# phantomzone-org/fhe-ram

Hardware: AMD Instinct MI355X
Metric: encrypted RAM read ops/s + write ops/s at 2^18 entries; achieved HBM GB/s vs peak (higher is better)
Workload: dtype f64

## Files before the change

fhe-ram_amd/csrc/bank.hpp:

```cpp
#pragma once
#include "path.hpp"

struct fheram_regs;
struct fheram_table;

enum LastKind { LAST_LIST, LAST_SELECT, LAST_REGS, LAST_TABLE, LAST_PEEK, LAST_KINDS };
struct LastOutputs {
    int n = 0;
    ResHome home;
};

struct fheram_bank {
    fheram_ctx* c = nullptr;
    int M = 0, mws = 0;
    RamState ram[FHERAM_BANK_MAX];
    double* d_prep = nullptr;
    double* d_prep_inv = nullptr;
    DenseBufs list;
    LastOutputs last[LAST_KINDS];
    DenseBufs wl;
    int kept_alone = 0, kept_n = 0;
    unsigned kept_map = 0;
    bool wl_holds[FHERAM_BANK_MAX] = {};
    SelectBufs sel;
    SelectLaneTable lanes;
    int sel_fail_alloc = 0;
    bool has_res[FHERAM_BANK_MAX] = {};
    int wl_fail_alloc = 0;
    OneRowSet regs;
    std::vector<fheram_regs*> regfiles;
    const int32_t* regs_old = nullptr;
    const fheram_regs* regs_old_owner = nullptr;
    OneRowSet tabs;
    std::vector<fheram_table*> tables;
    MixBufs mix;
    PublicBufs pub;
    int pub_fail_alloc = 0;
};

namespace {

void regs_keys_changed(fheram_bank* b);
void regs_bank_release(fheram_bank* b);
void table_bank_release(fheram_bank* b);

static_assert(FHERAM_READ_LIST_MAX >= FHERAM_BANK_MAX && FHERAM_READ_LIST_MAX * 4 <= 32, "a member set has four bits of the map per entry");
struct MemberSet {
    int n = 0;
    int m[FHERAM_READ_LIST_MAX];
    static MemberSet range(int first, int n) { MemberSet s; s.n = n; for (int k = 0; k < n; k++) s.m[k] = first + k; return s; }
    static MemberSet list(const int* members, int n) { MemberSet s; s.n = n; for (int k = 0; k < n; k++) s.m[k] = members[k]; return s; }
    bool is_range() const { for (int k = 1; k < n; k++) if (m[k] != m[0] + k) return false; return true; }
    unsigned map() const { unsigned v = 0; for (int k = 0; k < n; k++) v |= (unsigned)m[k] << (4 * k); return v; }
};

RamView bank_view(const fheram_bank* b, int first) {
    RamView v = ctx_view(b->c);
    const size_t o1 = (size_t)first * b->mws * fheram_ctx::GLWE, oR = o1 * b->c->rows;
    for (int32_t** p : {&v.rows, &v.A, &v.B, &v.C, &v.D}) *p += oR;
    for (int32_t** p : {&v.part, &v.tmp, &v.tmp2, &v.res, &v.tree, &v.w, &v.trtop}) *p += o1;
    return v;
}
GlweRef member_slot(const fheram_bank* b, int32_t* buf, int m) { return ref(buf + (size_t)m * b->mws * fheram_ctx::GLWE, (long)fheram_ctx::GLWE, 0); }

int check_addrs(fheram_ctx* c, const fheram_addr* const* addrs, int n) {
    for (int k = 0; k < n; k++) {
        if (!addrs[k] || addrs[k]->ctx != c) return fail(c, FHERAM_ERR_INVALID_ARG, "address " + std::to_string(k) + " is null or does not belong to this bank (layout mismatch, ram.rs:404)");
        if (addrs[k]->empty) return fail(c, FHERAM_ERR_INVALID_ARG, "address " + std::to_string(k) + " is an empty address: fheram_bank_address_alloc without fheram_bank_address_derive");
    }
    return FHERAM_OK;
}
int members_ready(fheram_bank* b, const MemberSet& s, const fheram_addr* const* addrs, int want_state) {
    fheram_ctx* c = b->c;
    if (addrs) { const int rc = check_addrs(c, addrs, s.n); if (rc != FHERAM_OK) return rc; }
    for (int k = 0; k < s.n; k++)
        if (!b->ram[s.m[k]].initialized) return fail(c, FHERAM_ERR_UNINITIALIZED, "unitialized memory: self.data.len()=0 (member " + std::to_string(s.m[k]) + ")");
    if (want_state < 0) return FHERAM_OK;
    if (!c->keys_loaded) return fail(c, FHERAM_ERR_KEYS, "evaluation keys not loaded");
    for (int k = 0; k < s.n; k++) {
        if (want_state == 0 && b->ram[s.m[k]].state)
            return fail(c, FHERAM_ERR_STATE, "invalid call to Memory.read: internal state is true -> requires calling Memory.write (member " + std::to_string(s.m[k]) + ")");
        if (want_state == 1 && !b->ram[s.m[k]].state)
            return fail(c, FHERAM_ERR_STATE, "invalid call to Memory.write: internal state is false -> requires calling Memory.read_prepare_write (member " + std::to_string(s.m[k]) + ")");
    }
    return FHERAM_OK;
}
int range_check(fheram_bank* b, int first, int n, const fheram_addr* const* addrs, const char* null_args, int want_state, MemberSet* s) {
    if (!b) return FHERAM_ERR_INVALID_ARG;
    fheram_ctx* c = b->c;
    if (null_args) return fail(c, FHERAM_ERR_INVALID_ARG, null_args);
    mid_rearm(c);
    if (first < 0 || n < 1 || first > b->M - n)
        return fail(c, FHERAM_ERR_INVALID_ARG, "member range [" + std::to_string(first) + ", " + std::to_string(first) + " + " + std::to_string(n) + ") is empty or outside the bank's " + std::to_string(b->M) + " members");
    *s = MemberSet::range(first, n);
    return members_ready(b, *s, addrs, want_state);
}
int read_list_check(fheram_bank* b, const int* members, const fheram_addr* const* addrs, int n, MemberSet* s) {
    if (!b) return FHERAM_ERR_INVALID_ARG;
    fheram_ctx* c = b->c;
    mid_rearm(c);
    if (!members || !addrs) return fail(c, FHERAM_ERR_INVALID_ARG, "null member list or null address list");
    if (n < 1 || n > FHERAM_READ_LIST_MAX)
        return fail(c, FHERAM_ERR_INVALID_ARG, "n = " + std::to_string(n) + " is outside [1, FHERAM_READ_LIST_MAX = " + std::to_string(FHERAM_READ_LIST_MAX) + "]");
    if ((long)n * b->mws > 64)
        return fail(c, FHERAM_ERR_INVALID_ARG, "n * word_size = " + std::to_string((long)n * b->mws) + " exceeds 64, the ciphertext limit of the single-launch chains (k_chain_mid)");
    for (int k = 0; k < n; k++)
        if (members[k] < 0 || members[k] >= b->M)
            return fail(c, FHERAM_ERR_INVALID_ARG, "entry " + std::to_string(k) + " names member " + std::to_string(members[k]) + ", outside the bank's " + std::to_string(b->M) + " members");
    *s = MemberSet::list(members, n);
    return members_ready(b, *s, addrs, 0);
}
int write_list_members(fheram_bank* b, const int* members, const fheram_addr* const* addrs, int n, int want_state, MemberSet* s) {
    fheram_ctx* c = b->c;
    if (n < 1 || n > b->M)
        return fail(c, FHERAM_ERR_INVALID_ARG, "n = " + std::to_string(n) + " is outside [1, the bank's " + std::to_string(b->M) + " members]");
    unsigned seen = 0;
    for (int k = 0; k < n; k++) {
        if (members[k] < 0 || members[k] >= b->M)
            return fail(c, FHERAM_ERR_INVALID_ARG, "entry " + std::to_string(k) + " names member " + std::to_string(members[k]) + ", outside the bank's " + std::to_string(b->M) + " members");
        if (seen & (1u << members[k]))
            return fail(c, FHERAM_ERR_INVALID_ARG, "entry " + std::to_string(k) + " names member " + std::to_string(members[k]) + " a second time: a RAM has one pending write (ram.rs:196-294), so the members of a write list are distinct");
        seen |= 1u << members[k];
    }
    *s = MemberSet::list(members, n);
    return members_ready(b, *s, addrs, want_state);
}
int write_list_check(fheram_bank* b, const int* members, const fheram_addr* const* addrs, int n, bool null_words, int want_state, MemberSet* s) {
    if (!b) return FHERAM_ERR_INVALID_ARG;
    fheram_ctx* c = b->c;
    mid_rearm(c);
    if (!members || !addrs || null_words) return fail(c, FHERAM_ERR_INVALID_ARG, want_state ? "null member list, null address list or null words" : "null member list or null address list");
    return write_list_members(b, members, addrs, n, want_state, s);
}

RamState set_state(const fheram_bank* b, const MemberSet& s, bool dense, bool write) {
    RamState st{true, write, true, dense ? 0 : b->ram[s.m[0]].memo_alone, false};
    bool holds = dense && write && b->kept_alone > 0 && b->kept_n == s.n && b->kept_map == s.map();
    for (int k = 0; k < s.n; k++) {
        const RamState& r = b->ram[s.m[k]];
        st.memo_top = st.memo_top && r.memo_top;
        if (!dense && r.memo_alone != st.memo_alone) st.memo_alone = 0;
        holds = holds && b->wl_holds[s.m[k]];
    }
    if (holds) st.memo_alone = b->kept_alone;
    return st;
}
struct SetPlan {
    const bool dense;
    RamState st;
    const RamView v;
    const Opnds o;
    SetPlan(fheram_bank* b, const MemberSet& s, const fheram_addr* const* addrs, bool write)
        : dense(!s.is_range()), st(set_state(b, s, dense, write)), v(dense ? dense_view(b->c, b->wl) : bank_view(b, s.m[0])),
          o(s.n == 1 ? one_addr(b->c, addrs, b->mws, &st)
                     : table_opnds(b->c, &st, addrs, s.n, b->mws, b->d_prep, b->d_prep_inv, dense ? s.map() : MEMBER_MAP_IDENTITY, true)) {}
    SetPlan(const SetPlan&) = delete;
};
void set_assign(fheram_bank* b, const MemberSet& s, const RamState& st, bool dense, bool state, bool new_result) {
    for (int k = 0; k < s.n; k++) {
        RamState& r = b->ram[s.m[k]];
        r.state = state; r.memo_top = st.memo_top; r.memo_alone = dense ? 0 : st.memo_alone;
        if (new_result) { r.res_in_trtop = st.res_in_trtop; b->has_res[s.m[k]] = true; }
        b->wl_holds[s.m[k]] = dense && st.memo_alone > 0;
    }
}
int set_result(fheram_bank* b, const MemberSet& s, bool dense, int64_t* out) {
    fheram_ctx* c = b->c;
    const size_t per = (size_t)b->mws * fheram_ctx::GLWE;
    ResRun runs[FHERAM_BANK_MAX];
    int n_runs = 0;
    for (int k = 0; k < s.n; k++) {
        const int32_t* src = (b->ram[s.m[k]].res_in_trtop ? c->d_trtop : c->d_res) + (size_t)s.m[k] * per;
        if (!dense && n_runs && runs[n_runs - 1].src + runs[n_runs - 1].n == src) runs[n_runs - 1].n += per;
        else runs[n_runs++] = ResRun{src, per};
    }
    return result_export(c, runs, n_runs, c->h_res, c->d_h_res, out);
}
int bank_read_set(fheram_bank* b, const MemberSet& s, const fheram_addr* const* addrs, bool prepare_write, int64_t* out) {
    fheram_ctx* c = b->c;
    HIPCHK(c, hipSetDevice(c->device));
    if (!s.is_range()) {
        const int rc = dense_reserve(c, b->wl, s.n, b->mws, true, &b->wl_fail_alloc);
        if (rc != FHERAM_OK) return rc;
        b->kept_alone = 0;
    }
    SetPlan p(b, s, addrs, false);
    const int rc = read_impl(p.o, p.v, prepare_write);
    if (rc == FHERAM_OK && p.dense) {
        const long G = (long)fheram_ctx::GLWE;
        for (int k = 0; k < s.n; k++) {
            if (c->n2 == 2) launch_copy(c, p.o.slice(ref(p.v.tree, G, 0), k), member_slot(b, c->d_tree, s.m[k]), 1, b->mws);
            launch_copy(c, p.o.slice(ref(p.st.res_in_trtop ? p.v.trtop : p.v.res, G, 0), k), member_slot(b, p.st.res_in_trtop ? c->d_trtop : c->d_res, s.m[k]), 1, b->mws);
        }
        b->kept_alone = p.st.memo_alone; b->kept_n = s.n; b->kept_map = p.o.member_map;
    }
    set_assign(b, s, p.st, p.dense, rc == FHERAM_OK && prepare_write, true);
    if (rc != FHERAM_OK) return rc;
    HIPCHK(c, hipGetLastError());
    return out ? set_result(b, s, p.dense, out) : FHERAM_OK;
}
template <typename S>
int bank_write_set(fheram_bank* b, const MemberSet& s, const fheram_addr* const* addrs, S&& stage) {
    fheram_ctx* c = b->c;
    HIPCHK(c, hipSetDevice(c->device));
    if (!s.is_range()) {
        const int rc = dense_reserve(c, b->wl, s.n, b->mws, true, &b->wl_fail_alloc);
        if (rc != FHERAM_OK) return rc;
    }
    SetPlan p(b, s, addrs, true);
    const long G = (long)fheram_ctx::GLWE;
    if (p.dense) {
        const bool holds = p.st.memo_alone > 0;
        b->kept_alone = 0;
        if (!holds) {
            main_enqueued(c);
            for (int k = 0; k < s.n; k++) {
                if (c->n2 == 2) launch_copy(c, member_slot(b, c->d_tree, s.m[k]), p.o.slice(ref(p.v.tree, G, 0), k), 1, b->mws);
                if (p.st.memo_top) launch_copy(c, member_slot(b, c->d_trtop, s.m[k]), p.o.slice(ref(p.v.trtop, G, 0), k), 1, b->mws);
            }
        }
    }
    const int rc = write_all(p.o, p.v, stage);
    if (rc == FHERAM_OK && p.dense && c->n2 == 2)
        for (int k = 0; k < s.n; k++) launch_copy(c, p.o.slice(ref(p.v.tree, G, 0), k), member_slot(b, c->d_tree, s.m[k]), 1, b->mws);
    set_assign(b, s, p.st, p.dense, rc != FHERAM_OK, false);
    if (rc != FHERAM_OK) return rc;
    HIPCHK(c, hipGetLastError());
    return FHERAM_OK;
}
struct LastKindText {
    int src;
    const char *unit, *units;
    const char *last, *of_last;
    const char* none;
};
const LastKindText LAST_TEXT[LAST_KINDS] = {
    {FHERAM_SRC_LIST_RESULT, "entry", "entries", "read list", "list", "no read list has run"},
    {FHERAM_SRC_SELECT_RESULT, "output", "outputs", "select", "select", "no select has run"},
    {FHERAM_SRC_REGS_RESULT, "output", "outputs", "register read", "register read", "no fheram_bank_regs_read has run"},
    {FHERAM_SRC_TABLE_RESULT, "output", "outputs", "table read", "table read", "no fheram_bank_table_read has run"},
    {FHERAM_SRC_PEEK_RESULT, "output", "outputs", "peek", "peek", "no fheram_bank_peek or fheram_bank_poke has run"},
};
int last_result(fheram_bank* b, LastKind kind, int first, int n, int64_t* out) {
    fheram_ctx* c = b->c;
    const LastOutputs& L = b->last[kind];
    const LastKindText& t = LAST_TEXT[kind];
    if (!out) return fail(c, FHERAM_ERR_INVALID_ARG, "null output");
    if (!L.n) return fail(c, FHERAM_ERR_STATE, std::string(t.none) + " on this bank");
    if (first < 0 || n < 1 || first > L.n - n)
        return fail(c, FHERAM_ERR_INVALID_ARG, std::string(t.units) + " [" + std::to_string(first) + ", " + std::to_string(first) + " + " + std::to_string(n) + ") are empty or outside the last " + t.of_last + "'s " + std::to_string(L.n) + " " + t.units);
    HIPCHK(c, hipSetDevice(c->device));
    const size_t per = (size_t)b->mws * fheram_ctx::GLWE;
    const ResRun run{L.home.res + (size_t)first * per, (size_t)n * per};
    return result_export(c, &run, 1, L.home.h, L.home.d_h, out);
}
void list_done(fheram_bank* b, int n) { b->last[LAST_LIST] = LastOutputs{n, ResHome{b->list.res, b->list.h_res, b->list.d_h_res, -1}}; }

}

extern "C" {

int fheram_bank_create(const fheram_params* p, int device, int n_members, const fheram_config* cfg, fheram_bank** out) {
    if (!p || !out) return fail(nullptr, FHERAM_ERR_INVALID_ARG, "null argument");
    *out = nullptr;
    if (n_members < 1 || n_members > FHERAM_BANK_MAX)
        return fail(nullptr, FHERAM_ERR_INVALID_ARG, "n_members = " + std::to_string(n_members) + " is outside [1, FHERAM_BANK_MAX = " + std::to_string(FHERAM_BANK_MAX) + "]");
    if ((uint64_t)n_members * p->word_size > 64)
        return fail(nullptr, FHERAM_ERR_INVALID_ARG, "n_members * word_size = " + std::to_string((uint64_t)n_members * p->word_size) + " exceeds 64, the ciphertext limit of the single-launch chains (k_chain_mid)");
    fheram_params wide = *p;
    wide.word_size = (uint32_t)n_members * p->word_size;
    fheram_config asked;
    if (cfg) asked = *cfg; else fheram_config_default(&asked);
    if (n_members > 1) asked.pre_inv = 0;
    fheram_ctx* c = nullptr;
    const int rc = fheram_ctx_create_cfg(&wide, device, 0, 1, &asked, &c);
    if (rc != FHERAM_OK) return rc;
    fheram_bank* b = new fheram_bank();
    b->c = c; b->M = n_members; b->mws = (int)p->word_size;
    c->ram.initialized = true;
    if (n_members > 1) {
        const size_t bytes = (size_t)n_members * c->n_digits * fheram_ctx::GGSW * sizeof(double);
        hipError_t e = c->res.device(&b->d_prep, bytes);
        if (e == hipSuccess) e = c->res.device(&b->d_prep_inv, bytes);
        if (e != hipSuccess) {
            (void)hipGetLastError();
            fheram_bank_destroy(b);
            return fail(nullptr, FHERAM_ERR_DEVICE, std::string("operand tables of the bank: ") + hipGetErrorString(e));
        }
    }
    *out = b;
    return FHERAM_OK;
}
void fheram_bank_destroy(fheram_bank* b) {
    if (!b) return;
    if (b->c) { hipSetDevice(b->c->device); for (hipStream_t s : {b->c->stream, b->c->stream2}) if (s) hipStreamSynchronize(s); }
    dense_free(b->list);
    dense_free(b->wl);
    select_free(b->sel);
    lane_table_free(b->lanes);
    regs_bank_release(b);
    table_bank_release(b);
    mix_bufs_free(b->mix);
    public_bufs_free(b->pub);
    fheram_ctx_destroy(b->c);
    delete b;
}
const char* fheram_bank_last_error(const fheram_bank* b) { return fheram_last_error(b ? b->c : nullptr); }
int fheram_bank_size(const fheram_bank* b) { return b ? b->M : 0; }

int fheram_bank_keys_load(fheram_bank* b, const int64_t* gal_els, int n_gal, const int64_t* const* atk_glwe,
                          const int64_t* atk_ggsw_inv, int64_t atk_ggsw_inv_p, const int64_t* tsk) {
    if (!b) return FHERAM_ERR_INVALID_ARG;
    const int rc = fheram_keys_load(b->c, gal_els, n_gal, atk_glwe, atk_ggsw_inv, atk_ggsw_inv_p, tsk);
    if (rc != FHERAM_OK) return rc;
    for (int m = 0; m < b->M; m++) { b->ram[m].memo_top = false; b->ram[m].memo_alone = 0; b->wl_holds[m] = false; }
    regs_keys_changed(b);
    return FHERAM_OK;
}
int fheram_bank_ram_upload(fheram_bank* b, int member, const int64_t* rows) {
    if (!b) return FHERAM_ERR_INVALID_ARG;
    fheram_ctx* c = b->c;
    if (member < 0 || member >= b->M) return fail(c, FHERAM_ERR_INVALID_ARG, "no such member");
    if (!rows) return fail(c, FHERAM_ERR_INVALID_ARG, "null rows");
    HIPCHK(c, hipSetDevice(c->device));
    const size_t n = (size_t)b->mws * c->rows * fheram_ctx::GLWE;
    const int rc = upload_i64(c, c->d_data + (size_t)member * n, rows, n);
    if (rc != FHERAM_OK) return rc;
    RamState& r = b->ram[member];
    r.initialized = true; r.state = false; r.memo_top = false; r.memo_alone = 0;
    b->wl_holds[member] = false;
    return FHERAM_OK;
}
int fheram_bank_ram_download(fheram_bank* b, int member, int64_t* rows) {
    if (!b) return FHERAM_ERR_INVALID_ARG;
    fheram_ctx* c = b->c;
    if (member < 0 || member >= b->M || !rows) return fail(c, FHERAM_ERR_INVALID_ARG, "no such member, or null rows");
    if (!b->ram[member].initialized) return fail(c, FHERAM_ERR_UNINITIALIZED, "unitialized memory: self.data.len()=0");
    HIPCHK(c, hipSetDevice(c->device));
    const size_t n = (size_t)b->mws * c->rows * fheram_ctx::GLWE;
    const int rc = download_i64(c, rows, c->d_data + (size_t)member * n, n);
    return rc == FHERAM_OK ? check_precision(c) : rc;
}
int fheram_bank_ram_tree_download(fheram_bank* b, int member, int level, int64_t* out) {
    if (!b) return FHERAM_ERR_INVALID_ARG;
    fheram_ctx* c = b->c;
    if (member < 0 || member >= b->M || !out) return fail(c, FHERAM_ERR_INVALID_ARG, "no such member, or null output");
    if (level != 0 || c->n2 < 2) return fail(c, FHERAM_ERR_INVALID_ARG, "tree level does not exist (ram.rs:315-324)");
    HIPCHK(c, hipSetDevice(c->device));
    const size_t n = (size_t)b->mws * fheram_ctx::GLWE;
    return download_i64(c, out, c->d_tree + (size_t)member * n, n);
}
int fheram_bank_ram_state(const fheram_bank* b, int member) { return (b && member >= 0 && member < b->M) ? (int)b->ram[member].state : 0; }

int fheram_bank_address_create(fheram_bank* b, const int64_t* const* ggsw, int n_ggsw, fheram_addr** out) {
    if (!b) return FHERAM_ERR_INVALID_ARG;
    return fheram_address_create(b->c, ggsw, n_ggsw, out);
}

int fheram_bank_fheuint_create(fheram_bank* b, const int64_t* bits, int n_bits, fheram_fheuint** out) {
    if (!b) return FHERAM_ERR_INVALID_ARG;
    return fheram_fheuint_create(b->c, bits, n_bits, out);
}
int fheram_bank_address_alloc(fheram_bank* b, fheram_addr** out) {
    if (!b) return FHERAM_ERR_INVALID_ARG;
    return fheram_address_alloc(b->c, out);
}
int fheram_bank_address_derive(fheram_bank* b, const fheram_fheuint* const* fus, int n, int sign, fheram_addr* const* addrs) {
    if (!b) return FHERAM_ERR_INVALID_ARG;
    return fheram_address_derive(b->c, fus, n, sign, addrs);
}
int fheram_bank_address_derive_at(fheram_bank* b, const fheram_fheuint* const* fus, const int* first_bit, int n, int sign, fheram_addr* const* addrs) {
    if (!b) return FHERAM_ERR_INVALID_ARG;
    return fheram_address_derive_at(b->c, fus, first_bit, n, sign, addrs);
}

int fheram_bank_read(fheram_bank* b, int first, int n, const fheram_addr* const* addrs, int64_t* out) {
    MemberSet s;
    const int rc = range_check(b, first, n, addrs, addrs ? nullptr : "null address list", 0, &s);
    return rc == FHERAM_OK ? bank_read_set(b, s, addrs, false, out) : rc;
}
int fheram_bank_read_prepare_write(fheram_bank* b, int first, int n, const fheram_addr* const* addrs, int64_t* out) {
    MemberSet s;
    const int rc = range_check(b, first, n, addrs, addrs ? nullptr : "null address list", 0, &s);
    return rc == FHERAM_OK ? bank_read_set(b, s, addrs, true, out) : rc;
}
int fheram_bank_write(fheram_bank* b, int first, int n, const int64_t* w, const fheram_addr* const* addrs) {
    MemberSet s;
    const int rc = range_check(b, first, n, addrs, (addrs && w) ? nullptr : "null address list or null words", 1, &s);
    return rc == FHERAM_OK ? bank_write_set(b, s, addrs, [&](int32_t* d_w, int n_ct) { return stage_words(b->c, d_w, w, n_ct); }) : rc;
}
int fheram_bank_result_download(fheram_bank* b, int first, int n, int64_t* out) {
    if (!b) return FHERAM_ERR_INVALID_ARG;
    if (!out) return fail(b->c, FHERAM_ERR_INVALID_ARG, "null output");
    MemberSet s;
    const int rc = range_check(b, first, n, nullptr, nullptr, -1, &s);
    if (rc != FHERAM_OK) return rc;
    HIPCHK(b->c, hipSetDevice(b->c->device));
    return set_result(b, s, false, out);
}
int fheram_bank_read_list(fheram_bank* b, const int* members, const fheram_addr* const* addrs, int n, int64_t* out) {
    MemberSet s;
    int rc = read_list_check(b, members, addrs, n, &s);
    if (rc != FHERAM_OK) return rc;
    fheram_ctx* c = b->c;
    HIPCHK(c, hipSetDevice(c->device));
    const long G = (long)fheram_ctx::GLWE;
    b->last[LAST_LIST].n = 0;
    if (n == 1) {
        rc = dense_reserve(c, b->list, 1, b->mws);
        if (rc == FHERAM_OK) rc = bank_read_set(b, s, addrs, false, nullptr);
        if (rc != FHERAM_OK) return rc;
        launch_copy(c, member_slot(b, c->d_res, s.m[0]), ref(b->list.res, G, 0), 1, b->mws);
        list_done(b, 1);
        HIPCHK(c, hipGetLastError());
        return out ? last_result(b, LAST_LIST, 0, 1, out) : FHERAM_OK;
    }
    RamState st{true, false, false, 0, false};
    return read_many(c, b->list, &st, addrs, n, b->mws, s.map(), b->M > 1, out, [&](const Opnds& o) {
        set_assign(b, s, st, false, false, true);
        for (int m = 0; m < b->M; m++) {
            int last = -1;
            for (int k = 0; k < n; k++) if (s.m[k] == m) last = k;
            if (last >= 0) launch_copy(c, o.slice(ref(b->list.res, G, 0), last), member_slot(b, c->d_res, m), 1, b->mws);
        }
        list_done(b, n);
    });
}
int fheram_bank_read_prepare_write_list(fheram_bank* b, const int* members, const fheram_addr* const* addrs, int n, int64_t* out) {
    MemberSet s;
    const int rc = write_list_check(b, members, addrs, n, false, 0, &s);
    return rc == FHERAM_OK ? bank_read_set(b, s, addrs, true, out) : rc;
}
int fheram_bank_write_list(fheram_bank* b, const int* members, const fheram_addr* const* addrs, int n, const int64_t* w) {
    MemberSet s;
    const int rc = write_list_check(b, members, addrs, n, !w, 1, &s);
    return rc == FHERAM_OK ? bank_write_set(b, s, addrs, [&](int32_t* d_w, int n_ct) { return stage_words(b->c, d_w, w, n_ct); }) : rc;
}
int fheram_bank_selftest_fail_list_alloc(fheram_bank* b, int nth) {
    if (!b || nth < 0) return FHERAM_ERR_INVALID_ARG;
    b->wl_fail_alloc = nth;
    return FHERAM_OK;
}
int fheram_bank_read_list_result(fheram_bank* b, int first, int n, int64_t* out) {
    return b ? last_result(b, LAST_LIST, first, n, out) : FHERAM_ERR_INVALID_ARG;
}
int fheram_bank_sync(fheram_bank* b) { return b ? fheram_sync(b->c) : FHERAM_ERR_INVALID_ARG; }
int fheram_bank_roundoff_max(fheram_bank* b, double* max_out) { return b ? fheram_roundoff_max(b->c, max_out) : FHERAM_ERR_INVALID_ARG; }
int fheram_bank_roundoff_reset(fheram_bank* b) { return b ? fheram_roundoff_reset(b->c) : FHERAM_ERR_INVALID_ARG; }
int fheram_bank_tail_stats(fheram_bank* b, uint64_t* launches, uint64_t* fallbacks) { return b ? fheram_tail_stats(b->c, launches, fallbacks) : FHERAM_ERR_INVALID_ARG; }
int fheram_bank_mid_stats(fheram_bank* b, uint64_t* launches, uint64_t* fallbacks) { return b ? fheram_mid_stats(b->c, launches, fallbacks) : FHERAM_ERR_INVALID_ARG; }
int fheram_bank_profile_enable(fheram_bank* b, int on) { return b ? fheram_profile_enable(b->c, on) : FHERAM_ERR_INVALID_ARG; }
int fheram_bank_profile_get(fheram_bank* b, const char* cls, uint64_t* launches, uint64_t* blocks, double* total_ms) {
    return b ? fheram_profile_get(b->c, cls, launches, blocks, total_ms) : FHERAM_ERR_INVALID_ARG;
}
int fheram_bank_profile_reset(fheram_bank* b) { return b ? fheram_profile_reset(b->c) : FHERAM_ERR_INVALID_ARG; }

}
```

fhe-ram_amd/csrc/ctx.hpp:

```cpp
#pragma once
#include "../../include/fheram.h"
#include "kernels.hpp"
#include "cmux_chain.hpp"
#include "cmux_jobs.hpp"
#include "mapped_chains.hpp"
#include "tail_wait.hpp"

#include <algorithm>
#include <atomic>
#include <cstdio>
#include <cstdlib>
#include <cstring>
#include <map>
#include <string>
#include <vector>

using namespace fk;

namespace {

thread_local std::string g_create_err;


struct ProfCls {
    uint64_t launches = 0, blocks = 0;
    double ms = 0.0;
    std::vector<std::pair<hipEvent_t, hipEvent_t>> pending;
};

}

inline uint64_t next_addr_id() { static std::atomic<uint64_t> n{0}; return ++n; }

struct RamState {
    bool initialized = false, state = false;
    bool memo_top = false;
    int memo_alone = 0;
    bool res_in_trtop = false;
};

struct DenseBufs {
    int cap = 0;
    int32_t *A = nullptr, *B = nullptr, *C = nullptr, *D = nullptr;
    int32_t *part = nullptr, *tmp = nullptr, *tmp2 = nullptr, *res = nullptr, *tree = nullptr, *w = nullptr, *trtop = nullptr;
    double* prep = nullptr;
    int64_t *h_res = nullptr, *d_h_res = nullptr;
};

inline fheram_config config_builtin() {
    fheram_config d{};
    d.limb_split = 1; d.fine_split = 1; d.memo = 1; d.pre_inv = 1; d.tail = 1; d.tail_test = 0; d.mid = 2; d.mid_test = 0;
    d.chain = 1; d.chain_y = 3; d.pair_z = 1; d.fuse = 1; d.graph = 0; d.safe = 0; d.nco = 0; d.tail_ep = 1; d.monitor = 1; d.reserved = 0;
    return d;
}
inline fheram_config config_in_effect(const fheram_config& in) {
    using C = fheram_config;
    fheram_config e{};
    for (int32_t C::*on_off : {&C::limb_split, &C::fine_split, &C::memo, &C::tail, &C::tail_ep, &C::mid_test, &C::chain, &C::pair_z, &C::fuse, &C::graph, &C::safe})
        e.*on_off = in.*on_off ? 1 : 0;
    for (int32_t C::*upto2 : {&C::tail_test, &C::mid, &C::monitor}) e.*upto2 = in.*upto2 < 0 ? 0 : (in.*upto2 > 2 ? 2 : in.*upto2);
    e.chain_y = in.chain_y ? 3 : 0;
    e.nco = in.nco == 2 ? 2 : (in.nco == 1 ? 1 : 0);
    e.pre_inv = e.memo ? (in.pre_inv == 2 ? 2 : (in.pre_inv ? 1 : 0)) : 0;
    if (e.graph) e.pre_inv = 0;
    if (e.safe) { e.tail = 0; e.tail_test = 0; e.mid = 0; e.mid_test = 0; if (e.pre_inv == 1) e.pre_inv = 2; }
    if (e.safe && e.monitor == 1) e.monitor = 2;
    return e;
}

struct CtxResources {
    std::vector<void*> dev, pinned;
    std::vector<hipEvent_t> events;
    template <typename T> hipError_t device(T** p, size_t bytes) { const hipError_t e = hipMalloc((void**)p, bytes); if (e == hipSuccess) dev.push_back(*p); return e; }
    template <typename T> hipError_t host(T** p, size_t bytes, unsigned flags) { const hipError_t e = hipHostMalloc((void**)p, bytes, flags); if (e == hipSuccess) pinned.push_back(*p); return e; }
    hipError_t event(hipEvent_t* ev, bool timing = false) {
        const hipError_t e = timing ? hipEventCreate(ev) : hipEventCreateWithFlags(ev, hipEventDisableTiming);
        if (e == hipSuccess) events.push_back(*ev);
        return e;
    }
    void release() {
        for (hipEvent_t e : events) hipEventDestroy(e);
        for (void* p : dev) hipFree(p);
        for (void* p : pinned) hipHostFree(p);
        events.clear(); dev.clear(); pinned.clear();
    }
};

struct fheram_ctx {
    fheram_params p;
    int device = 0;
    int ws = 0, n2 = 0, n_digits = 0, max_digits = 0;
    size_t rows = 0;
    size_t rows_glob = 0;
    int shard = 0, n_shards = 1;
    std::vector<std::vector<int>> base2d;
    static constexpr int S_CT = 3, S_ADDR = 4, S_INV = 5, DNUM_CT = 3, DNUM_GGSW = 4;
    int s_evk = 4;
    size_t atk = 0;
    static constexpr size_t GLWE = (size_t)S_CT * 2 * N;
    static constexpr size_t GLWE4 = (size_t)S_ADDR * 2 * N;
    static constexpr size_t GGSW = (size_t)DNUM_CT * 2 * GLWE4;
    static constexpr size_t EVK5 = (size_t)DNUM_GGSW * S_INV * 2 * N;
    static constexpr size_t GGSW5 = (size_t)DNUM_GGSW * 2 * S_INV * 2 * N;
    int cus = 256;
    CtxResources res;
    hipStream_t stream = nullptr;
    hipStream_t stream2 = nullptr;
    hipStream_t cur = nullptr;
    hipEvent_t ev_fork = nullptr, ev_join = nullptr;
    hipEvent_t ev_xout = nullptr, ev_xin = nullptr;
    fheram_config cfg = config_builtin();
    bool wide = false;
    double* d_tw = nullptr;
    double ninv = 0.0;
    double* d_atk = nullptr;
    double* d_atk_inv = nullptr;
    double* d_tsk = nullptr;
    int64_t gal[LOGN];
    bool keys_loaded = false;
    unsigned* h_ro_flag = nullptr;
    int32_t* d_data = nullptr;
    int32_t* d_tree = nullptr;
    int32_t* d_scrA = nullptr;
    int32_t* d_scrB = nullptr;
    int32_t* d_scrC = nullptr;
    int32_t* d_scrD = nullptr;
    int32_t* d_res = nullptr;
    int32_t* d_tmp = nullptr;
    int32_t* d_tmp2 = nullptr;
    int32_t* d_w = nullptr;
    int32_t* d_trtop = nullptr;
    int32_t* d_part = nullptr;
    int32_t* d_gat[3] = {nullptr, nullptr, nullptr};
    RamState ram;
    DenseBufs batch;
    double* d_big = nullptr;
    double* d_big2 = nullptr;
    double* d_prep = nullptr;
    bool prep1_ready = false;
    int32_t* d_ggsw_tmp = nullptr;
    int32_t* d_ggsw_tmp2 = nullptr;
    unsigned tail_seq = 0;
    int tail_xoff = 0;
    uint64_t tail_launches = 0;
    unsigned* h_tail_fb = nullptr;
    unsigned tail_fb_mark = 0;
    uint64_t tail_launch_mark = 0;
    unsigned* d_tail_sync = nullptr;
    unsigned* h_tail_done = nullptr;
    unsigned* d_h_tail_done = nullptr;
    TailWait tail_wait;
    unsigned mid_seq = 0;
    uint64_t mid_launches = 0, mid_launch_mark = 0;
    unsigned mid_fb_mark = 0;
    int mid_bad_windows = 0, mid_saved = 0;
    uint64_t mid_window_cts = 0, mid_disabled_count = 0;
    unsigned mid_off_ops = 0;
    unsigned* h_mid_fb = nullptr;
    unsigned* d_mid_sync[2] = {nullptr, nullptr};
    double* d_mid_big[2] = {nullptr, nullptr};
    double* d_mid_y[2] = {nullptr, nullptr};
    uint64_t inv_id[2] = {0, 0};
    double* d_prep_inv = nullptr;
    int32_t* d_ggsw_inv = nullptr;
    hipEvent_t ev_inv[2] = {nullptr, nullptr};
    bool inv_pending[2] = {false, false};
    hipEvent_t ev_wdone = nullptr;
    bool wdone_pending = false;
    hipEvent_t ev_opstart = nullptr;
    bool opstart_valid = false;
    bool wide_unsynced = false;
    bool derive_unsynced = false;
    bool main_idle = false;
    int32_t* h_pin[2] = {nullptr, nullptr};
    hipEvent_t ev_pin[2] = {nullptr, nullptr};
    int64_t* h_res = nullptr;
    int64_t* d_h_res = nullptr;
    int32_t* h_w = nullptr;
    hipEvent_t ev_w = nullptr;
    bool w_busy = false;
    bool side_begun = false;
    bool trhi_in_C = false;
    bool tree_rotate_pending = false;
    bool words_staged = false;
    int profile = 0;
    std::map<std::string, ProfCls> prof;
    std::vector<hipEvent_t> ev_pool;
    hipEvent_t t0 = nullptr, t1 = nullptr;
    std::string err;
};

struct fheram_addr {
    fheram_ctx* ctx;
    int32_t* d_ggsw;
    int n_digits;
    int device;
    uint64_t id = next_addr_id();
    hipGraphExec_t graph[3] = {nullptr, nullptr, nullptr};
    unsigned graph_sig[3] = {0, 0, 0};
    bool empty = false;
};

struct fheram_fheuint {
    fheram_ctx* ctx;
    int device, n_bits;
    int32_t* d_std;
    double* d_prep;
};

struct fheram_secret {
    fheram_ctx* ctx;
    int device;
    std::vector<int32_t> sk;
    double* d_hat;
};

namespace {

int fail(fheram_ctx* c, int code, const std::string& msg) {
    if (c) c->err = msg; else g_create_err = msg;
    return code;
}
int check_precision(fheram_ctx* c) {
    if (c->h_ro_flag && __atomic_load_n(c->h_ro_flag, __ATOMIC_RELAXED))
        return fail(c, FHERAM_ERR_PRECISION, "FP64 round-off of an inverse transform exceeded 3/8 (fheram_roundoff_max): the rounded integers are no longer trustworthy");
    return FHERAM_OK;
}
#define HIPCHK(c, call)                                                                     \
    do {                                                                                    \
        hipError_t e_ = (call);                                                             \
        if (e_ != hipSuccess)                                                               \
            return fail((c), FHERAM_ERR_DEVICE, std::string(#call) + ": " + hipGetErrorString(e_)); \
    } while (0)

GlweRef ref(int32_t* p, long sy, long sx) { return GlweRef{p, sy, sx}; }

void main_waited(fheram_ctx* c) { c->wide_unsynced = c->derive_unsynced = false; c->main_idle = true; c->tail_wait.waited(); }
void main_enqueued(fheram_ctx* c) { c->main_idle = false; c->tail_wait.enqueued(); }

hipEvent_t get_event(fheram_ctx* c) {
    if (!c->ev_pool.empty()) { hipEvent_t e = c->ev_pool.back(); c->ev_pool.pop_back(); return e; }
    hipEvent_t e = nullptr; c->res.event(&e, true); return e;
}
struct ProfScope {
    fheram_ctx* c; ProfCls* cls = nullptr; hipEvent_t a = nullptr;
    ProfScope(fheram_ctx* c_, const char* name, uint64_t blocks, int steps = 1) : c(c_) {
        if (!c->profile) return;
        if (c->profile == 2 && !strstr(name, "chain_launch")) return;
        cls = &c->prof[name];
        cls->launches += steps; cls->blocks += blocks * steps;
        a = get_event(c);
        hipEventRecord(a, c->cur);
    }
    ~ProfScope() {
        if (!cls) return;
        hipEvent_t b = get_event(c);
        hipEventRecord(b, c->cur);
        cls->pending.emplace_back(a, b);
    }
};
void prof_collect(fheram_ctx* c) {
    for (auto& kv : c->prof) {
        for (auto& pr : kv.second.pending) {
            hipEventSynchronize(pr.second);
            float ms = 0.f;
            hipEventElapsedTime(&ms, pr.first, pr.second);
            kv.second.ms += ms;
            c->ev_pool.push_back(pr.first); c->ev_pool.push_back(pr.second);
        }
        kv.second.pending.clear();
    }
}

std::vector<std::vector<int>> base_2d(uint64_t max_addr, const fheram_params& p) {
    std::vector<std::vector<int>> plan;
    uint32_t x = (uint32_t)(max_addr - 1), bits = 0;
    while (x) { bits++; x >>= 1; }
    while (bits != 0) {
        std::vector<int> v;
        for (uint32_t i = 0; i < p.n_decomp; i++) {
            const uint32_t b = p.decomp_n[i];
            if (b <= bits) { v.push_back((int)b); bits -= b; }
            else { if (bits != 0) { v.push_back((int)bits); bits = 0; } break; }
        }
        plan.push_back(v);
    }
    return plan;
}
int ilog2_ceil(size_t x) { int k = 0; while (((size_t)1 << k) < x) k++; return k; }
int galois_mod(int64_t g) { const int64_t m = 2 * N; return (int)(((g % m) + m) % m); }
int galois_inv_mod(int g) {
    int64_t r = 1, b = g, e = N - 1, m = 2 * N;
    while (e) { if (e & 1) r = r * b % m; b = b * b % m; e >>= 1; }
    return (int)r;
}
int64_t galois_element(int i) {
    if (i == 0) return -1;
    int64_t g = 5, e = (int64_t)1 << (i - 1), r = 1, m = 2 * N;
    while (e) { if (e & 1) r = r * g % m; g = g * g % m; e >>= 1; }
    return r;
}

bool narrow(const int64_t* src, int32_t* dst, size_t n) {
    int64_t bad = 0;
    for (size_t i = 0; i < n; i++) {
        const int64_t v = src[i];
        bad |= (v > 65536) | (v < -65536);
        dst[i] = (int32_t)v;
    }
    return bad == 0;
}
void widen(const int32_t* src, int64_t* dst, size_t n) { for (size_t i = 0; i < n; i++) dst[i] = src[i]; }

constexpr size_t PIN_CHUNK = (size_t)1 << 21;
int pin_init(fheram_ctx* c) {
    if (c->h_pin[0]) return FHERAM_OK;
    for (int b = 0; b < 2; b++) {
        HIPCHK(c, c->res.host(&c->h_pin[b], PIN_CHUNK * sizeof(int32_t), hipHostMallocDefault));
        HIPCHK(c, c->res.event(&c->ev_pin[b]));
    }
    return FHERAM_OK;
}
int upload_i64(fheram_ctx* c, int32_t* dst, const int64_t* src, size_t n) {
    int rc = pin_init(c);
    if (rc != FHERAM_OK) return rc;
    bool ok = true;
    int k = 0;
    for (size_t off = 0; off < n && ok; off += PIN_CHUNK, k++) {
        const int b = k & 1;
        const size_t m = std::min(PIN_CHUNK, n - off);
        if (k >= 2) HIPCHK(c, hipEventSynchronize(c->ev_pin[b]));
        ok = narrow(src + off, c->h_pin[b], m);
        if (!ok) break;
        HIPCHK(c, hipMemcpyAsync(dst + off, c->h_pin[b], m * sizeof(int32_t), hipMemcpyHostToDevice, c->stream));
        HIPCHK(c, hipEventRecord(c->ev_pin[b], c->stream));
    }
    HIPCHK(c, hipStreamSynchronize(c->stream));
    if (!ok) return fail(c, FHERAM_ERR_RANGE, "limb out of the normalised range [-2^16, 2^16]");
    return FHERAM_OK;
}
int download_i64(fheram_ctx* c, int64_t* dst, const int32_t* src, size_t n) {
    int rc = pin_init(c);
    if (rc != FHERAM_OK) return rc;
    const size_t n_chunks = (n + PIN_CHUNK - 1) / PIN_CHUNK;
    for (size_t k = 0; k <= n_chunks; k++) {
        if (k < n_chunks) {
            const size_t off = k * PIN_CHUNK, m = std::min(PIN_CHUNK, n - off);
            HIPCHK(c, hipMemcpyAsync(c->h_pin[k & 1], src + off, m * sizeof(int32_t), hipMemcpyDeviceToHost, c->stream));
            HIPCHK(c, hipEventRecord(c->ev_pin[k & 1], c->stream));
        }
        if (k > 0) {
            const size_t off = (k - 1) * PIN_CHUNK, m = std::min(PIN_CHUNK, n - off);
            HIPCHK(c, hipEventSynchronize(c->ev_pin[(k - 1) & 1]));
            widen(c->h_pin[(k - 1) & 1], dst + off, m);
        }
    }
    return FHERAM_OK;
}
int stage_words(fheram_ctx* c, int32_t* d_w, const int64_t* w, int n_ct) {
    if (c->w_busy) { HIPCHK(c, hipEventSynchronize(c->ev_w)); c->w_busy = false; }
    const size_t n = (size_t)n_ct * fheram_ctx::GLWE;
    if (!narrow(w, c->h_w, n)) return fail(c, FHERAM_ERR_RANGE, "limb out of the normalised range [-2^16, 2^16]");
    main_enqueued(c);
    HIPCHK(c, hipMemcpyAsync(d_w, c->h_w, n * sizeof(int32_t), hipMemcpyHostToDevice, c->stream));
    HIPCHK(c, hipEventRecord(c->ev_w, c->stream));
    c->w_busy = true;
    return FHERAM_OK;
}

}
```

fhe-ram_amd/csrc/fheram.hip:

```cpp
#include <unistd.h>
#include <atomic>
#include "path.hpp"

extern "C" {

int fheram_params_default(fheram_params* p) {
    if (!p) return FHERAM_ERR_INVALID_ARG;
    std::memset(p, 0, sizeof(*p));
    p->log_n = 12; p->base2k = 17; p->rank = 1;
    p->k_glwe_pt = 3; p->k_glwe_ct = 51; p->k_ggsw_addr = 68; p->k_evk_trace = 68; p->k_evk_ggsw_inv = 85;
    p->word_size = 4; p->n_decomp = 4;
    p->decomp_n[0] = p->decomp_n[1] = p->decomp_n[2] = p->decomp_n[3] = 3;
    p->max_addr = (uint64_t)1 << 14;
    return FHERAM_OK;
}

const char* fheram_last_error(const fheram_ctx* c) { return c ? c->err.c_str() : g_create_err.c_str(); }

void fheram_config_default(fheram_config* cfg) {
    if (!cfg) return;
    fheram_config d = config_builtin();
    auto env = [](const char* n) { const char* v = getenv(n); return (v && v[0]) ? v[0] : '\0'; };
    if (env("FHERAM_LIMB_SPLIT") == '0') d.limb_split = 0;
    if (env("FHERAM_FINE_SPLIT") == '0') d.fine_split = 0;
    if (env("FHERAM_MEMO") == '0') d.memo = 0;
    if (env("FHERAM_PRE_INV") == '0') d.pre_inv = 0; else if (env("FHERAM_PRE_INV") == '2') d.pre_inv = 2;
    const char tl = env("FHERAM_TAIL");
    if (tl == '0') d.tail = 0;
    d.tail_test = tl == '2' ? 1 : (tl == '3' ? 2 : 0);
    const char md = env("FHERAM_MID");
    d.mid = md == '0' ? 0 : (md == '1' ? 1 : 2);
    d.mid_test = md == '2' ? 1 : 0;
    if (env("FHERAM_CHAIN") == '0') d.chain = 0;
    if (env("FHERAM_CHAIN_Y") == '0') d.chain_y = 0;
    if (env("FHERAM_PAIR_Z") == '0') d.pair_z = 0;
    if (env("FHERAM_FUSE") == '0') d.fuse = 0;
    if (env("FHERAM_GRAPH") == '1') d.graph = 1;
    if (env("FHERAM_SAFE") == '1') d.safe = 1;
    const char nc = env("FHERAM_NCO");
    d.nco = nc == '2' ? 2 : (nc == '1' ? 1 : 0);
    if (env("FHERAM_TAIL_EP") == '0') d.tail_ep = 0;
    const char mo = env("FHERAM_MONITOR");
    if (mo == '0') d.monitor = 0; else if (mo == '2') d.monitor = 2;
    *cfg = d;
}

int fheram_ctx_create(const fheram_params* p, int device, fheram_ctx** out) {
    return fheram_ctx_create_cfg(p, device, 0, 1, nullptr, out);
}

int fheram_ctx_create_sharded(const fheram_params* p, int device, int shard, int n_shards, fheram_ctx** out) {
    return fheram_ctx_create_cfg(p, device, shard, n_shards, nullptr, out);
}

int fheram_ctx_create_cfg(const fheram_params* p, int device, int shard, int n_shards, const fheram_config* user_cfg, fheram_ctx** out) {
    if (!p || !out) return fail(nullptr, FHERAM_ERR_INVALID_ARG, "null argument");
    *out = nullptr;
    if (n_shards < 1 || shard < 0 || shard >= n_shards || (n_shards & (n_shards - 1)) != 0)
        return fail(nullptr, FHERAM_ERR_INVALID_ARG, "n_shards must be a power of two and 0 <= shard < n_shards");
    auto limbs = [&](uint32_t k) { return (k + p->base2k - 1) / (p->base2k ? p->base2k : 1); };
    if (p->log_n != 12 || p->base2k != 17 || p->rank != 1 || p->k_glwe_ct == 0 || limbs(p->k_glwe_ct) != 3 || limbs(p->k_ggsw_addr) != 4 ||
        (limbs(p->k_evk_trace) != 4 && limbs(p->k_evk_trace) != 5) || limbs(p->k_evk_ggsw_inv) != 5)
        return fail(nullptr, FHERAM_ERR_UNSUPPORTED, "kernels are built for LOG_N=12, BASE2K=17, RANK=1 and limb counts K_CT: 3, K_ADDR: 4, K_EVK_TRACE: 4 or 5, K_EVK_GGSW_INV: 5");
    if (p->k_glwe_pt == 0 || p->k_glwe_pt > p->k_glwe_ct)
        return fail(nullptr, FHERAM_ERR_INVALID_ARG, "k_glwe_pt must be in [1, k_glwe_ct]");
    if (p->word_size == 0 || p->word_size > 64 || p->n_decomp == 0 || p->n_decomp > 16 || p->max_addr < 2)
        return fail(nullptr, FHERAM_ERR_INVALID_ARG, "bad word_size / decomp_n / max_addr");
    unsigned sum = 0;
    for (uint32_t i = 0; i < p->n_decomp; i++) { if (p->decomp_n[i] == 0) return fail(nullptr, FHERAM_ERR_INVALID_ARG, "zero digit width"); sum += p->decomp_n[i]; }
    if (sum != p->log_n) return fail(nullptr, FHERAM_ERR_INVALID_ARG, "DECOMP_N must sum to LOG_N (parameters.rs:168)");
    if (p->max_addr > ((uint64_t)N * N)) return fail(nullptr, FHERAM_ERR_UNSUPPORTED, "max_addr > N^2 is not supported by the reference either (SURVEY.md 3.1)");
    if (user_cfg && user_cfg->reserved != 0)
        return fail(nullptr, FHERAM_ERR_INVALID_ARG, "fheram_config.reserved must be 0 (start from fheram_config_default())");

    int ndev = 0;
    if (hipGetDeviceCount(&ndev) != hipSuccess || ndev <= 0)
        return fail(nullptr, FHERAM_ERR_DEVICE, "no HIP device: the FHE-RAM evaluator has no CPU path");
    if (device < 0 || device >= ndev) return fail(nullptr, FHERAM_ERR_INVALID_ARG, "bad device index");

    fheram_ctx* c = new fheram_ctx();
    c->p = *p; c->device = device; c->ws = (int)p->word_size;
    c->s_evk = (int)limbs(p->k_evk_trace);
    c->atk = (size_t)fheram_ctx::DNUM_CT * c->s_evk * 2 * N;
    c->rows_glob = (size_t)((p->max_addr + N - 1) / N);
    c->shard = shard; c->n_shards = n_shards;
    if (n_shards > 1 && ((c->rows_glob & (c->rows_glob - 1)) != 0 || c->rows_glob < (size_t)n_shards)) {
        delete c;
        return fail(nullptr, FHERAM_ERR_INVALID_ARG, "row sharding needs a power-of-two number of rows >= n_shards (else: replicas only)");
    }
    c->rows = c->rows_glob / (size_t)n_shards;
    c->base2d = base_2d(p->max_addr, *p);
    c->n2 = (int)c->base2d.size();
    for (auto& v : c->base2d) { c->n_digits += (int)v.size(); c->max_digits = std::max(c->max_digits, (int)v.size()); }
    for (int i = 0; i < LOGN; i++) c->gal[i] = galois_element(i);

#define CCHK(call)                                                                  \
    do {                                                                            \
        hipError_t e_ = (call);                                                     \
        if (e_ != hipSuccess) {                                                     \
            g_create_err = std::string(#call) + ": " + hipGetErrorString(e_);       \
            fheram_ctx_destroy(c);                                                  \
            return FHERAM_ERR_DEVICE;                                               \
        }                                                                           \
    } while (0)
    CCHK(hipSetDevice(device));
    CCHK(hipStreamCreateWithFlags(&c->stream, hipStreamNonBlocking));
    {
        int lo = 0, hi = 0;
        CCHK(hipDeviceGetStreamPriorityRange(&lo, &hi));
        CCHK(hipStreamCreateWithPriority(&c->stream2, hipStreamNonBlocking, lo));
    }
    c->cur = c->stream;
    for (hipEvent_t* ev : {&c->ev_fork, &c->ev_join, &c->ev_xout, &c->ev_xin}) CCHK(c->res.event(ev));
    for (hipEvent_t* ev : {&c->t0, &c->t1}) CCHK(c->res.event(ev, true));
    fheram_config asked;
    if (user_cfg) asked = *user_cfg; else fheram_config_default(&asked);
    c->cfg = config_in_effect(asked);
    static std::atomic<int> serial{0};
    c->tail_xoff = ((serial++ + (int)getpid()) & 1) * (TAIL_GROUPS / 2);
    hipDeviceProp_t prop;
    if (hipGetDeviceProperties(&prop, device) == hipSuccess && prop.multiProcessorCount > 0) c->cus = prop.multiProcessorCount;
#define LDSATTR(k) CCHK(hipFuncSetAttribute(reinterpret_cast<const void*>(k), hipFuncAttributeMaxDynamicSharedMemorySize, (int)LDS_BYTES))
    LDSATTR(k_prepare);
    LDSATTR((&k_ext_product<3, 4, 1>));
    LDSATTR((&k_ext_product<3, 4, 2>));
    LDSATTR((&k_ext_product<3, 4, 1, 1>));
    LDSATTR((&k_ext_product_fine<3, 4>));
    LDSATTR((&k_ext_product_fine<4, 5>));
    LDSATTR((&k_ext_product_chain<3, 4>));
    LDSATTR((&k_ext_product_chain_r<4>));
    LDSATTR((&k_pair_z<4>)); LDSATTR((&k_pair_z<5>));
    LDSATTR((&k_read_chain<4, 4>)); LDSATTR((&k_read_chain<5, 4>)); LDSATTR((&k_write_chain<4, 4>)); LDSATTR((&k_write_chain<5, 4>));
    LDSATTR((&k_write_chain_t<4, 4>)); LDSATTR((&k_write_chain_t<5, 4>));
    LDSATTR((&k_read_chain_w<4, 4>)); LDSATTR((&k_read_chain_w<5, 4>));
    LDSATTR((&k_read_chain_t<4, 4>)); LDSATTR((&k_read_chain_t<5, 4>));
    LDSATTR((&k_trace_tail_t<3, 4, 3>)); LDSATTR((&k_trace_tail_t<3, 5, 3>));
    LDSATTR((&k_keyswitch_chain_w<3, 4, 3, 3>)); LDSATTR((&k_keyswitch_chain_w<3, 5, 3, 3>));
    LDSATTR((&k_keyswitch_chain<3, 4, 3>));
    LDSATTR((&k_keyswitch_chain<3, 4, 3, 3>));
    LDSATTR((&k_keyswitch_chain<3, 5, 3, 3>));
    LDSATTR((&k_trace_tail<3, 4, 3>));
    LDSATTR((&k_chain_mid<false, 4, 3, 2>)); LDSATTR((&k_chain_mid<false, 5, 3, 2>)); LDSATTR((&k_chain_mid<true, 4, 3, 2>));
    LDSATTR((&k_chain_mid<false, 4, 1, 1>)); LDSATTR((&k_chain_mid<false, 5, 1, 1>));
    LDSATTR((&k_chain_mid<false, 4, 1, 2>)); LDSATTR((&k_chain_mid<false, 5, 1, 2>));
#define LDSATTR_KS4(M, SX, SK, SO) LDSATTR((&k_keyswitch<M, SX, SK, SO, 1>)); LDSATTR((&k_keyswitch<M, SX, SK, SO, 1, 1>)); LDSATTR((&k_keyswitch_fine<M, SX, SK>))
#define LDSATTR_KS(M, SX, SK, SO) LDSATTR_KS4(M, SX, SK, SO); LDSATTR((&k_keyswitch<M, SX, SK, SO, 2>))
    LDSATTR_KS(KS_AUTO, 3, 4, 3);
    LDSATTR_KS(KS_TRACE, 3, 4, 3);
    LDSATTR_KS4(KS_PAIR, 3, 4, 3);
    LDSATTR_KS(KS_ADD, 3, 4, 3);
    LDSATTR_KS(KS_SUBNEG, 3, 4, 3);
    LDSATTR((&k_keyswitch_chain<3, 5, 3>));
    LDSATTR((&k_trace_tail<3, 5, 3>));
    LDSATTR_KS(KS_AUTO, 3, 5, 3);
    LDSATTR_KS(KS_TRACE, 3, 5, 3);
    LDSATTR_KS4(KS_PAIR, 3, 5, 3);
    LDSATTR_KS(KS_ADD, 3, 5, 3);
    LDSATTR_KS(KS_SUBNEG, 3, 5, 3);
    LDSATTR_KS4(KS_AUTO, 4, 5, 4);
    LDSATTR_KS4(KS_TENSOR, 4, 5, 4);
    LDSATTR((&k_encrypt_sk<1, 1>));
    LDSATTR((&k_encrypt_sk<3, 0>)); LDSATTR((&k_encrypt_sk<3, 1>));
    LDSATTR((&k_encrypt_sk<4, 0>)); LDSATTR((&k_encrypt_sk<4, 1>));
    LDSATTR((&k_encrypt_sk<5, 0>)); LDSATTR((&k_encrypt_sk<5, 1>));
    CCHK(cmux_chain_register());
    CCHK(cmux_jobs_register());
    CCHK(mapped_chains_register());
#undef LDSATTR_KS
#undef LDSATTR_KS4
#undef LDSATTR

    std::vector<double> tw = make_fft_twiddles();
    c->ninv = 1.0 / (double)NC;
    {
        CCHK(c->res.host(&c->h_ro_flag, 64, hipHostMallocDefault));
        *c->h_ro_flag = 0;
        const uint64_t mode = (uint64_t)c->cfg.monitor, flag_addr = (uint64_t)(size_t)c->h_ro_flag;
        std::memcpy(&tw[0], &mode, 8);
        std::memcpy(&tw[N + 1], &flag_addr, 8);
    }
    CCHK(c->res.device(&c->d_tw, TW_GLOBAL * sizeof(double)));
    CCHK(hipMemcpy(c->d_tw, tw.data(), TW_GLOBAL * sizeof(double), hipMemcpyHostToDevice));
    const size_t G = fheram_ctx::GLWE, nrow = (size_t)c->ws * c->rows;
    CCHK(c->res.device(&c->d_atk, (size_t)LOGN * c->atk * sizeof(double)));
    for (double** key : {&c->d_atk_inv, &c->d_tsk}) CCHK(c->res.device(key, fheram_ctx::EVK5 * sizeof(double)));
    for (int32_t** arena : {&c->d_data, &c->d_scrA, &c->d_scrB, &c->d_scrC, &c->d_scrD}) CCHK(c->res.device(arena, nrow * G * sizeof(int32_t)));
    CCHK(c->res.device(&c->d_ggsw_tmp2, (size_t)c->max_digits * fheram_ctx::GGSW * sizeof(int32_t)));
    for (int32_t** ct : {&c->d_tmp2, &c->d_part}) CCHK(c->res.device(ct, (size_t)c->ws * G * sizeof(int32_t)));
    for (double** big : {&c->d_big, &c->d_big2}) CCHK(c->res.device(big, (size_t)LIMB_SPLIT_MAX * BIG_STRIDE * sizeof(double)));
    if (n_shards > 1) for (int i = 0; i < 3; i++) CCHK(c->res.device(&c->d_gat[i], (size_t)n_shards * c->ws * G * sizeof(int32_t)));
    for (int32_t** ct : {&c->d_tree, &c->d_res, &c->d_tmp, &c->d_w, &c->d_trtop}) CCHK(c->res.device(ct, (size_t)c->ws * G * sizeof(int32_t)));
    CCHK(c->res.device(&c->d_prep, (size_t)std::max(c->n_digits, c->max_digits) * fheram_ctx::GGSW * sizeof(double)));
    CCHK(c->res.device(&c->d_ggsw_tmp, (size_t)c->max_digits * fheram_ctx::GGSW * sizeof(int32_t)));
    CCHK(hipMemset(c->d_tree, 0, (size_t)c->ws * G * sizeof(int32_t)));
    CCHK(c->res.device(&c->d_prep_inv, (size_t)c->n_digits * fheram_ctx::GGSW * sizeof(double)));
    CCHK(c->res.device(&c->d_ggsw_inv, (size_t)c->n_digits * fheram_ctx::GGSW * sizeof(int32_t)));
    for (hipEvent_t* ev : {&c->ev_inv[0], &c->ev_inv[1], &c->ev_wdone, &c->ev_opstart}) CCHK(c->res.event(ev));
    CCHK(c->res.device(&c->d_tail_sync, (size_t)(TAIL_GROUPS + 1) * 32 * sizeof(unsigned)));
    CCHK(hipMemset(c->d_tail_sync, 0, (size_t)(TAIL_GROUPS + 1) * 32 * sizeof(unsigned)));
    for (int i = 0; i < 2; i++) {
        CCHK(c->res.device(&c->d_mid_sync[i], (size_t)(MID_GROUPS_MAX + 1) * 32 * sizeof(unsigned)));
        CCHK(hipMemset(c->d_mid_sync[i], 0, (size_t)(MID_GROUPS_MAX + 1) * 32 * sizeof(unsigned)));
        CCHK(c->res.device(&c->d_mid_y[i], (size_t)2 * MID_GROUPS_MAX * 2 * N * sizeof(double)));
        CCHK(c->res.device(&c->d_mid_big[i], (size_t)2 * MID_GROUPS_MAX * BIG_STRIDE * sizeof(double)));
    }
    CCHK(c->res.host(&c->h_tail_fb, 64, hipHostMallocDefault));
    *c->h_tail_fb = 0;
    CCHK(c->res.host(&c->h_tail_done, 128, hipHostMallocMapped));
    memset(c->h_tail_done, 0, 128);
    CCHK(hipHostGetDevicePointer((void**)&c->d_h_tail_done, c->h_tail_done, 0));
    c->tail_wait.done = c->h_tail_done; c->tail_wait.gave_up = c->h_tail_done + 16;
    if (const char* e = std::getenv("FHERAM_TAIL_POLL_US")) c->tail_wait.bound_us = std::atol(e);
    CCHK(c->res.host(&c->h_mid_fb, 128, hipHostMallocDefault));
    memset(c->h_mid_fb, 0, 128);
    CCHK(c->res.host(&c->h_res, ((size_t)c->ws * G + 1) * sizeof(int64_t), hipHostMallocMapped));
    CCHK(hipHostGetDevicePointer((void**)&c->d_h_res, c->h_res, 0));
    CCHK(c->res.host(&c->h_w, (size_t)c->ws * G * sizeof(int32_t), hipHostMallocDefault));
    CCHK(c->res.event(&c->ev_w));
#undef CCHK
    *out = c;
    return FHERAM_OK;
}

void fheram_ctx_destroy(fheram_ctx* c) {
    if (!c) return;
    hipSetDevice(c->device);
    for (hipStream_t s : {c->stream, c->stream2}) if (s) hipStreamSynchronize(s);
    prof_collect(c);
    dense_free(c->batch);
    c->res.release();
    for (hipStream_t s : {c->stream2, c->stream}) if (s) hipStreamDestroy(s);
    delete c;
}

int fheram_ctx_config(const fheram_ctx* c, fheram_config* out) {
    if (!c || !out) return FHERAM_ERR_INVALID_ARG;
    *out = c->cfg;
    out->reserved = 0;
    return FHERAM_OK;
}

size_t fheram_glwe_len(const fheram_ctx*) { return fheram_ctx::GLWE; }
size_t fheram_ggsw_len(const fheram_ctx*) { return fheram_ctx::GGSW; }
size_t fheram_atk_len(const fheram_ctx* c) { return c ? c->atk : 0; }
size_t fheram_evk_inv_len(const fheram_ctx*) { return fheram_ctx::EVK5; }
size_t fheram_rows(const fheram_ctx* c) { return c ? c->rows : 0; }
int fheram_n_digits(const fheram_ctx* c) { return c ? c->n_digits : 0; }
int fheram_n_coordinates(const fheram_ctx* c) { return c ? c->n2 : 0; }

int fheram_keys_load(fheram_ctx* c, const int64_t* gal_els, int n_gal, const int64_t* const* atk_glwe,
                     const int64_t* atk_ggsw_inv, int64_t atk_ggsw_inv_p, const int64_t* tsk) {
    if (!c) return FHERAM_ERR_INVALID_ARG;
    if (!gal_els || !atk_glwe || !atk_ggsw_inv || !tsk) return fail(c, FHERAM_ERR_INVALID_ARG, "null key pointer");
    if (n_gal != LOGN) return fail(c, FHERAM_ERR_KEYS, "expected log2(N) trace keys (keys.rs:39)");
    if (atk_ggsw_inv_p != -1) return fail(c, FHERAM_ERR_KEYS, "auto_key.p() != -1 (coordinate_prepared.rs:134)");
    HIPCHK(c, hipSetDevice(c->device));
    HIPCHK(c, hipStreamSynchronize(c->stream));
    HIPCHK(c, hipStreamSynchronize(c->stream2));
    int order[LOGN];
    for (int i = 0; i < LOGN; i++) {
        order[i] = -1;
        for (int j = 0; j < n_gal; j++) if (gal_els[j] == c->gal[i]) order[i] = j;
        if (order[i] < 0) return fail(c, FHERAM_ERR_KEYS, "missing trace key for a Galois element of GLWE::trace_galois_elements");
    }
    int32_t* d_stage = nullptr;
    const size_t stage_n = std::max(c->atk, fheram_ctx::EVK5);
    HIPCHK(c, hipMalloc(&d_stage, stage_n * sizeof(int32_t)));
    int rc = FHERAM_OK;
    for (int i = 0; i < LOGN && rc == FHERAM_OK; i++) {
        rc = upload_i64(c, d_stage, atk_glwe[order[i]], c->atk);
        if (rc == FHERAM_OK) launch_prepare(c, d_stage, c->d_atk + (size_t)i * c->atk, (int)(c->atk / N), c->gal[i]);
        hipStreamSynchronize(c->stream);
    }
    if (rc == FHERAM_OK) rc = upload_i64(c, d_stage, atk_ggsw_inv, fheram_ctx::EVK5);
    if (rc == FHERAM_OK) { launch_prepare(c, d_stage, c->d_atk_inv, (int)(fheram_ctx::EVK5 / N), -1); hipStreamSynchronize(c->stream); }
    if (rc == FHERAM_OK) rc = upload_i64(c, d_stage, tsk, fheram_ctx::EVK5);
    if (rc == FHERAM_OK) { launch_prepare(c, d_stage, c->d_tsk, (int)(fheram_ctx::EVK5 / N)); hipStreamSynchronize(c->stream); }
    hipFree(d_stage);
    if (rc != FHERAM_OK) return rc;
    HIPCHK(c, hipGetLastError());
    c->keys_loaded = true;
    c->inv_id[0] = c->inv_id[1] = 0;
    c->inv_pending[0] = c->inv_pending[1] = false;
    c->ram.memo_top = false; c->ram.memo_alone = 0;
    return FHERAM_OK;
}

int fheram_ram_upload(fheram_ctx* c, const int64_t* rows) {
    if (!c) return FHERAM_ERR_INVALID_ARG;
    if (!rows) return fail(c, FHERAM_ERR_INVALID_ARG, "null rows");
    HIPCHK(c, hipSetDevice(c->device));
    int rc = upload_i64(c, c->d_data, rows, (size_t)c->ws * c->rows * fheram_ctx::GLWE);
    if (rc != FHERAM_OK) return rc;
    c->ram.initialized = true; c->ram.state = false; c->ram.memo_top = false; c->ram.memo_alone = 0;
    return FHERAM_OK;
}
int fheram_ram_download(fheram_ctx* c, int64_t* rows) {
    if (!c || !rows) return FHERAM_ERR_INVALID_ARG;
    if (!c->ram.initialized) return fail(c, FHERAM_ERR_UNINITIALIZED, "unitialized memory: self.data.len()=0");
    HIPCHK(c, hipSetDevice(c->device));
    const int rc = download_i64(c, rows, c->d_data, (size_t)c->ws * c->rows * fheram_ctx::GLWE);
    return rc == FHERAM_OK ? check_precision(c) : rc;
}
int fheram_ram_tree_download(fheram_ctx* c, int level, int64_t* out) {
    if (!c || !out) return FHERAM_ERR_INVALID_ARG;
    if (level != 0 || c->n2 < 2) return fail(c, FHERAM_ERR_INVALID_ARG, "tree level does not exist (ram.rs:315-324)");
    HIPCHK(c, hipSetDevice(c->device));
    return download_i64(c, out, c->d_tree, (size_t)c->ws * fheram_ctx::GLWE);
}
int fheram_ram_state(const fheram_ctx* c) { return c ? (int)c->ram.state : 0; }

int fheram_address_create(fheram_ctx* c, const int64_t* const* ggsw, int n_ggsw, fheram_addr** out) {
    if (!c || !out) return FHERAM_ERR_INVALID_ARG;
    *out = nullptr;
    if (!ggsw) return fail(c, FHERAM_ERR_INVALID_ARG, "null ggsw");
    if (n_ggsw != c->n_digits) return fail(c, FHERAM_ERR_INVALID_ARG, "address digit count does not match the context's Base2D (ram.rs:404)");
    HIPCHK(c, hipSetDevice(c->device));
    fheram_addr* a = new fheram_addr{c, nullptr, n_ggsw, c->device};
    hipError_t e = hipMalloc(&a->d_ggsw, (size_t)n_ggsw * fheram_ctx::GGSW * sizeof(int32_t));
    if (e != hipSuccess) { delete a; return fail(c, FHERAM_ERR_DEVICE, std::string("hipMalloc: ") + hipGetErrorString(e)); }
    for (int i = 0; i < n_ggsw; i++) {
        if (!ggsw[i]) { fheram_address_destroy(a); return fail(c, FHERAM_ERR_INVALID_ARG, "null ggsw digit"); }
        int rc = upload_i64(c, a->d_ggsw + (size_t)i * fheram_ctx::GGSW, ggsw[i], fheram_ctx::GGSW);
        if (rc != FHERAM_OK) { fheram_address_destroy(a); return rc; }
    }
    *out = a;
    return FHERAM_OK;
}
void fheram_address_destroy(fheram_addr* a) {
    if (!a) return;
    hipSetDevice(a->device);
    for (auto& g : a->graph) if (g) { hipGraphExecDestroy(g); g = nullptr; }
    if (a->d_ggsw) hipFree(a->d_ggsw);
    delete a;
}

int fheram_result_map(fheram_ctx* c, const int64_t** out) {
    if (!c || !out) return FHERAM_ERR_INVALID_ARG;
    HIPCHK(c, hipSetDevice(c->device));
    const ResRun run{c->ram.res_in_trtop ? c->d_trtop : c->d_res, (size_t)c->ws * fheram_ctx::GLWE};
    *out = c->h_res;
    return result_export(c, &run, 1, c->h_res, c->d_h_res, nullptr);
}
int fheram_result_download(fheram_ctx* c, int64_t* out) {
    if (!c || !out) return FHERAM_ERR_INVALID_ARG;
    const int64_t* src = nullptr;
    const int rc = fheram_result_map(c, &src);
    if (rc != FHERAM_OK) return rc;
    std::memcpy(out, src, (size_t)c->ws * fheram_ctx::GLWE * sizeof(int64_t));
    return FHERAM_OK;
}
int fheram_sync(fheram_ctx* c) {
    if (!c) return FHERAM_ERR_INVALID_ARG;
    HIPCHK(c, hipSetDevice(c->device));
    if (!c->tail_wait.poll()) HIPCHK(c, hipStreamSynchronize(c->stream));
    HIPCHK(c, hipGetLastError());
    main_waited(c);
    return check_precision(c);
}
int fheram_roundoff_max(fheram_ctx* c, double* max_out) {
    if (!c || !max_out) return FHERAM_ERR_INVALID_ARG;
    HIPCHK(c, hipSetDevice(c->device));
    HIPCHK(c, hipStreamSynchronize(c->stream));
    HIPCHK(c, hipStreamSynchronize(c->stream2));
    double m = 0.0;
    HIPCHK(c, hipMemcpy(&m, c->d_tw + N, sizeof(double), hipMemcpyDeviceToHost));
    *max_out = m;
    if (c->cfg.monitor && m > MON_LIMIT) __atomic_store_n(c->h_ro_flag, 1u, __ATOMIC_RELAXED);
    return check_precision(c);
}
int fheram_roundoff_reset(fheram_ctx* c) {
    if (!c) return FHERAM_ERR_INVALID_ARG;
    HIPCHK(c, hipSetDevice(c->device));
    HIPCHK(c, hipStreamSynchronize(c->stream));
    HIPCHK(c, hipStreamSynchronize(c->stream2));
    HIPCHK(c, hipMemset(c->d_tw + N, 0, sizeof(double)));
    __atomic_store_n(c->h_ro_flag, 0u, __ATOMIC_RELAXED);
    return FHERAM_OK;
}

int fheram_read(fheram_ctx* c, const fheram_addr* addr, int64_t* out) {
    int rc = check_common(c, addr);
    if (rc != FHERAM_OK) return rc;
    if (c->n_shards != 1) return fail(c, FHERAM_ERR_INVALID_ARG, "row-sharded context: use fheram_read_partial / fheram_read_finish");
    if (c->ram.state) return fail(c, FHERAM_ERR_STATE, "invalid call to Memory.read: internal state is true -> requires calling Memory.write");
    HIPCHK(c, hipSetDevice(c->device));
    rc = run_op(c, addr, 0, [&] { return read_impl(one_addr(c, &addr), ctx_view(c), false); });
    if (rc != FHERAM_OK) return rc;
    HIPCHK(c, hipGetLastError());
    if (out) return fheram_result_download(c, out);
    c->tail_wait.arm();
    return FHERAM_OK;
}
int fheram_read_batch(fheram_ctx* c, const fheram_addr* const* addrs, int n_addr, int64_t* out) {
    if (!c) return FHERAM_ERR_INVALID_ARG;
    if (!addrs) return fail(c, FHERAM_ERR_INVALID_ARG, "null address list");
    if (n_addr < 1 || n_addr > FHERAM_READ_BATCH_MAX)
        return fail(c, FHERAM_ERR_INVALID_ARG, "n_addr = " + std::to_string(n_addr) + " is outside [1, FHERAM_READ_BATCH_MAX = " + std::to_string(FHERAM_READ_BATCH_MAX) + "]");
    for (int k = 0; k < n_addr; k++) {
        const int rc = check_common(c, addrs[k]);
        if (rc != FHERAM_OK) return rc;
    }
    if (c->n_shards != 1) return fail(c, FHERAM_ERR_INVALID_ARG, "row-sharded context: use fheram_read_partial / fheram_read_finish");
    if (c->ram.state) return fail(c, FHERAM_ERR_STATE, "invalid call to Memory.read: internal state is true -> requires calling Memory.write");
    HIPCHK(c, hipSetDevice(c->device));
    int rc;
    if (n_addr == 1) {
        rc = run_op(c, addrs[0], 0, [&] { return read_impl(one_addr(c, addrs), ctx_view(c), false); });
        if (rc != FHERAM_OK) return rc;
        HIPCHK(c, hipGetLastError());
        if (out) return fheram_result_download(c, out);
        c->tail_wait.arm();
        return FHERAM_OK;
    }
    return read_many(c, c->batch, &c->ram, addrs, n_addr, c->ws, 0, false, out, [&](const Opnds& o) {
        launch_copy(c, o.slice(ref(c->batch.res, (long)fheram_ctx::GLWE, 0), n_addr - 1), ref(c->d_res, (long)fheram_ctx::GLWE, 0), 1, c->ws);
    });
}
int fheram_read_prepare_write(fheram_ctx* c, const fheram_addr* addr, int64_t* out) {
    int rc = check_common(c, addr);
    if (rc != FHERAM_OK) return rc;
    if (c->n_shards != 1) return fail(c, FHERAM_ERR_INVALID_ARG, "row-sharded context: use fheram_read_partial / fheram_read_finish");
    if (c->ram.state) return fail(c, FHERAM_ERR_STATE, "invalid call to Memory.read: internal state is true -> requires calling Memory.write");
    HIPCHK(c, hipSetDevice(c->device));
    rc = run_op(c, addr, 1, [&] { return read_impl(one_addr(c, &addr), ctx_view(c), true); });
    if (rc != FHERAM_OK) return rc;
    c->ram.state = true;
    HIPCHK(c, hipGetLastError());
    if (out) return fheram_result_download(c, out);
    c->tail_wait.arm();
    return FHERAM_OK;
}
int fheram_word_stage(fheram_ctx* c, const int64_t* w, int n_w) {
    if (!c || !w) return FHERAM_ERR_INVALID_ARG;
    if (n_w != c->ws) return fail(c, FHERAM_ERR_INVALID_ARG, "w.len() != subrams.len() (ram.rs:243)");
    HIPCHK(c, hipSetDevice(c->device));
    const int rc = stage_words(c, c->d_w, w, c->ws);
    if (rc == FHERAM_OK) c->words_staged = true;
    return rc;
}
int fheram_write(fheram_ctx* c, const int64_t* w, int n_w, const fheram_addr* addr) {
    int rc = check_common(c, addr);
    if (rc != FHERAM_OK) return rc;
    if (n_w != c->ws) return fail(c, FHERAM_ERR_INVALID_ARG, "w.len() != subrams.len() (ram.rs:243)");
    if (!c->ram.state) return fail(c, FHERAM_ERR_STATE, "invalid call to Memory.write: internal state is false -> requires calling Memory.read_prepare_write");
    HIPCHK(c, hipSetDevice(c->device));
    if (c->n_shards != 1) return fail(c, FHERAM_ERR_INVALID_ARG, "row-sharded context: use fheram_write_root / fheram_write_shard");
    if (!w && !c->words_staged) return fail(c, FHERAM_ERR_INVALID_ARG, "w == NULL and no staged words");
    const Opnds o = one_addr(c, &addr);
    if (w && !c->side_begun && !capturing(c)) write_side_begin(o, ctx_view(c));
    if (w) { rc = fheram_word_stage(c, w, n_w); if (rc != FHERAM_OK) { write_side_abort(c); return rc; } }
    rc = run_op(c, addr, 2, [&] {
        if (!c->side_begun) write_side_begin(o, ctx_view(c));
        int r2 = write_top(o, ctx_view(c));
        return r2 == FHERAM_OK ? write_rows(o, ctx_view(c)) : r2;
    });
    if (rc != FHERAM_OK) return rc;
    c->ram.state = false;
    HIPCHK(c, hipGetLastError());
    return FHERAM_OK;
}

namespace {
int export_glwes(fheram_ctx* c, const int32_t* src, void* dst, int on_device, size_t n_glwe) {
    const size_t n = n_glwe * fheram_ctx::GLWE;
    if (on_device) { main_enqueued(c); HIPCHK(c, hipMemcpyAsync(dst, src, n * 4, hipMemcpyDeviceToDevice, c->stream)); return FHERAM_OK; }
    return download_i64(c, (int64_t*)dst, src, n);
}
int import_glwes(fheram_ctx* c, int32_t* dst, const void* src, int on_device, size_t n_glwe) {
    const size_t n = n_glwe * fheram_ctx::GLWE;
    if (on_device) { main_enqueued(c); HIPCHK(c, hipMemcpyAsync(dst, src, n * 4, hipMemcpyDeviceToDevice, c->stream)); return FHERAM_OK; }
    return upload_i64(c, dst, (const int64_t*)src, n);
}
}

int fheram_shard_info(const fheram_ctx* c, int* shard, int* n_shards, size_t* local_rows) {
    if (!c) return FHERAM_ERR_INVALID_ARG;
    if (shard) *shard = c->shard;
    if (n_shards) *n_shards = c->n_shards;
    if (local_rows) *local_rows = c->rows;
    return FHERAM_OK;
}
int fheram_read_partial(fheram_ctx* c, const fheram_addr* addr, int prepare_write, void* out, int out_on_device) {
    int rc = check_common(c, addr);
    if (rc != FHERAM_OK) return rc;
    if (!out) return fail(c, FHERAM_ERR_INVALID_ARG, "null output");
    if (c->ram.state) return fail(c, FHERAM_ERR_STATE, "invalid call to Memory.read: internal state is true -> requires calling Memory.write");
    HIPCHK(c, hipSetDevice(c->device));
    GlweRef packed;
    rc = read_local(one_addr(c, &addr), ctx_view(c), prepare_write != 0, &packed, true);
    if (rc != FHERAM_OK) return rc;
    HIPCHK(c, hipGetLastError());
    if (prepare_write) c->ram.state = true;
    return export_glwes(c, c->d_part, out, out_on_device, (size_t)c->ws);
}
int fheram_stream_signal(fheram_ctx* c, void* hip_stream) {
    if (!c) return FHERAM_ERR_INVALID_ARG;
    HIPCHK(c, hipSetDevice(c->device));
    main_enqueued(c);
    HIPCHK(c, hipEventRecord(c->ev_xout, c->stream));
    HIPCHK(c, hipStreamWaitEvent((hipStream_t)hip_stream, c->ev_xout, 0));
    return FHERAM_OK;
}
int fheram_stream_wait(fheram_ctx* c, void* hip_stream) {
    if (!c) return FHERAM_ERR_INVALID_ARG;
    HIPCHK(c, hipSetDevice(c->device));
    HIPCHK(c, hipEventRecord(c->ev_xin, (hipStream_t)hip_stream));
    main_enqueued(c);
    HIPCHK(c, hipStreamWaitEvent(c->stream, c->ev_xin, 0));
    return FHERAM_OK;
}
int fheram_device_malloc(fheram_ctx* c, size_t bytes, void** out) {
    if (!c || !out || bytes == 0) return fail(c, FHERAM_ERR_INVALID_ARG, "bad argument");
    HIPCHK(c, hipSetDevice(c->device));
    HIPCHK(c, hipMalloc(out, bytes));
    return FHERAM_OK;
}
int fheram_device_free(fheram_ctx* c, void* ptr) {
    if (!c) return FHERAM_ERR_INVALID_ARG;
    HIPCHK(c, hipSetDevice(c->device));
    HIPCHK(c, hipFree(ptr));
    return FHERAM_OK;
}
int fheram_write_begin(fheram_ctx* c, const fheram_addr* addr) {
    int rc = check_common(c, addr);
    if (rc != FHERAM_OK) return rc;
    if (!c->ram.state) return fail(c, FHERAM_ERR_STATE, "invalid call to Memory.write: internal state is false -> requires calling Memory.read_prepare_write");
    HIPCHK(c, hipSetDevice(c->device));
    if (!c->side_begun) write_side_begin(one_addr(c, &addr), ctx_view(c));
    HIPCHK(c, hipGetLastError());
    return FHERAM_OK;
}
int fheram_read_finish(fheram_ctx* c, const fheram_addr* addr, int prepare_write, const void* partials, int partials_on_device, int64_t* out) {
    int rc = check_common(c, addr);
    if (rc != FHERAM_OK) return rc;
    if (!partials) return fail(c, FHERAM_ERR_INVALID_ARG, "null partials");
    HIPCHK(c, hipSetDevice(c->device));
    int32_t* gathered = nullptr;
    if (c->n_shards > 1) {
        rc = import_glwes(c, c->d_gat[0], partials, partials_on_device, (size_t)c->n_shards * c->ws);
        gathered = c->d_gat[0];
    } else {
        rc = import_glwes(c, c->d_part, partials, partials_on_device, (size_t)c->ws);
    }
    if (rc != FHERAM_OK) return rc;
    rc = read_top(one_addr(c, &addr), ctx_view(c), prepare_write != 0, gathered, ref(c->d_part, (long)fheram_ctx::GLWE, 0));
    if (rc != FHERAM_OK) return rc;
    HIPCHK(c, hipGetLastError());
    return out ? fheram_result_download(c, out) : fheram_sync(c);
}
int fheram_write_root(fheram_ctx* c, const int64_t* w, int n_w, const fheram_addr* addr, void* ct_lo_out, int out_on_device) {
    int rc = check_common(c, addr);
    if (rc != FHERAM_OK) return rc;
    if (n_w != c->ws) return fail(c, FHERAM_ERR_INVALID_ARG, "w.len() != subrams.len() (ram.rs:243)");
    if (c->n2 != 2) return fail(c, FHERAM_ERR_INVALID_ARG, "a row-sharded RAM has two coordinates");
    if (!c->ram.state) return fail(c, FHERAM_ERR_STATE, "invalid call to Memory.write: internal state is false -> requires calling Memory.read_prepare_write");
    if (!ct_lo_out) return fail(c, FHERAM_ERR_INVALID_ARG, "null output");
    HIPCHK(c, hipSetDevice(c->device));
    if (w) { rc = fheram_word_stage(c, w, n_w); if (rc != FHERAM_OK) return rc; }
    else if (!c->words_staged) return fail(c, FHERAM_ERR_INVALID_ARG, "w == NULL and no staged words");
    if (!c->side_begun) write_side_begin(one_addr(c, &addr), ctx_view(c));
    rc = write_top(one_addr(c, &addr), ctx_view(c));
    if (rc != FHERAM_OK) return rc;
    HIPCHK(c, hipGetLastError());
    return export_glwes(c, c->d_part, ct_lo_out, out_on_device, (size_t)c->ws);
}
int fheram_write_shard(fheram_ctx* c, const fheram_addr* addr, const void* ct_lo, int on_device) {
    int rc = check_common(c, addr);
    if (rc != FHERAM_OK) return rc;
    if (!ct_lo) return fail(c, FHERAM_ERR_INVALID_ARG, "null ct_lo");
    if (!c->ram.state) return fail(c, FHERAM_ERR_STATE, "invalid call to Memory.write: internal state is false -> requires calling Memory.read_prepare_write");
    HIPCHK(c, hipSetDevice(c->device));
    if (!c->side_begun) write_side_begin(one_addr(c, &addr), ctx_view(c));
    rc = import_glwes(c, c->d_part, ct_lo, on_device, (size_t)c->ws);
    if (rc != FHERAM_OK) { write_side_abort(c); return rc; }
    rc = write_rows(one_addr(c, &addr), ctx_view(c));
    if (rc != FHERAM_OK) return rc;
    HIPCHK(c, hipGetLastError());
    return FHERAM_OK;
}

namespace {
struct DevBuf {
    int32_t* p = nullptr;
    ~DevBuf() { if (p) hipFree(p); }
};
}

int fheram_glwe_external_product(fheram_ctx* c, const int64_t* a, int batch, const int64_t* ggsw, int64_t* res) {
    if (!c || !a || !ggsw || !res || batch <= 0) return fail(c, FHERAM_ERR_INVALID_ARG, "bad argument");
    HIPCHK(c, hipSetDevice(c->device));
    const size_t G = fheram_ctx::GLWE;
    DevBuf da, dg;
    HIPCHK(c, hipMalloc(&da.p, (size_t)batch * G * 4));
    HIPCHK(c, hipMalloc(&dg.p, fheram_ctx::GGSW * 4));
    int rc = upload_i64(c, da.p, a, (size_t)batch * G);
    if (rc == FHERAM_OK) rc = upload_i64(c, dg.p, ggsw, fheram_ctx::GGSW);
    if (rc != FHERAM_OK) return rc;
    DevBuf dout;
    HIPCHK(c, hipMalloc(&dout.p, (size_t)batch * G * 4));
    launch_prepare(c, dg.p, c->d_prep, (int)(fheram_ctx::GGSW / N));
    launch_ep(c, ref(da.p, 0, (long)G), ref(dout.p, 0, (long)G), c->d_prep, batch, 1);
    HIPCHK(c, hipGetLastError());
    return download_i64(c, res, dout.p, (size_t)batch * G);
}
int fheram_glwe_automorphism(fheram_ctx* c, int mode, int64_t gal_el, const int64_t* a, int batch, int64_t* res) {
    if (!c || !a || !res || batch <= 0 || mode < 0 || mode > 2) return fail(c, FHERAM_ERR_INVALID_ARG, "bad argument");
    if (!c->keys_loaded) return fail(c, FHERAM_ERR_KEYS, "evaluation keys not loaded");
    int ki = -1;
    for (int i = 0; i < LOGN; i++) if (c->gal[i] == gal_el) ki = i;
    if (ki < 0) return fail(c, FHERAM_ERR_KEYS, "no key for this Galois element");
    HIPCHK(c, hipSetDevice(c->device));
    const size_t G = fheram_ctx::GLWE;
    DevBuf da, dout;
    HIPCHK(c, hipMalloc(&da.p, (size_t)batch * G * 4));
    HIPCHK(c, hipMalloc(&dout.p, (size_t)batch * G * 4));
    int rc = upload_i64(c, da.p, a, (size_t)batch * G);
    if (rc != FHERAM_OK) return rc;
    KsArgs ka = ks_args(c, ref(da.p, 0, (long)G), ref(da.p, 0, 0), ref(dout.p, 0, (long)G), trace_key(c, ki), gal_el);
    if (mode == 0) launch_ks_tr<KS_AUTO>(c, ka, batch, 1);
    else if (mode == 1) launch_ks_tr<KS_ADD>(c, ka, batch, 1);
    else launch_ks_tr<KS_SUBNEG>(c, ka, batch, 1);
    HIPCHK(c, hipGetLastError());
    return download_i64(c, res, dout.p, (size_t)batch * G);
}
int fheram_glwe_trace(fheram_ctx* c, int start, int end, const int64_t* a, int batch, int64_t* res) {
    if (!c || !a || !res || batch <= 0 || start < 0 || end > LOGN || start > end) return fail(c, FHERAM_ERR_INVALID_ARG, "bad argument");
    if (!c->keys_loaded) return fail(c, FHERAM_ERR_KEYS, "evaluation keys not loaded");
    HIPCHK(c, hipSetDevice(c->device));
    const size_t G = fheram_ctx::GLWE;
    DevBuf da, db, dc;
    HIPCHK(c, hipMalloc(&da.p, (size_t)batch * G * 4));
    HIPCHK(c, hipMalloc(&db.p, (size_t)batch * G * 4));
    HIPCHK(c, hipMalloc(&dc.p, (size_t)batch * G * 4));
    int rc = upload_i64(c, da.p, a, (size_t)batch * G);
    if (rc != FHERAM_OK) return rc;
    trace_steps(c, ref(da.p, 0, (long)G), ref(db.p, 0, (long)G), ref(dc.p, 0, (long)G), start, end, batch, 1);
    HIPCHK(c, hipGetLastError());
    return download_i64(c, res, db.p, (size_t)batch * G);
}
int fheram_glwe_pack(fheram_ctx* c, const int64_t* cts, int count, int64_t* out) {
    if (!c || !cts || !out || count <= 0 || count > N) return fail(c, FHERAM_ERR_INVALID_ARG, "bad argument");
    if (!c->keys_loaded) return fail(c, FHERAM_ERR_KEYS, "evaluation keys not loaded");
    HIPCHK(c, hipSetDevice(c->device));
    const size_t G = fheram_ctx::GLWE;
    DevBuf src, A, B;
    HIPCHK(c, hipMalloc(&src.p, (size_t)count * G * 4));
    HIPCHK(c, hipMalloc(&A.p, (size_t)count * G * 4));
    HIPCHK(c, hipMalloc(&B.p, (size_t)count * G * 4));
    int rc = upload_i64(c, src.p, cts, (size_t)count * G);
    if (rc != FHERAM_OK) return rc;
    const int L0p = LOGN - ilog2_ceil((size_t)count);
    int32_t* packed = pack_levels(c, src.p, A.p, B.p, 0, (long)G, (size_t)count, 1, L0p, L0p);
    HIPCHK(c, hipGetLastError());
    return download_i64(c, out, packed, G);
}
int fheram_ggsw_automorphism_inv(fheram_ctx* c, const int64_t* ggsw_in, int64_t* ggsw_out) {
    if (!c || !ggsw_in || !ggsw_out) return fail(c, FHERAM_ERR_INVALID_ARG, "bad argument");
    if (!c->keys_loaded) return fail(c, FHERAM_ERR_KEYS, "evaluation keys not loaded");
    HIPCHK(c, hipSetDevice(c->device));
    DevBuf din;
    HIPCHK(c, hipMalloc(&din.p, fheram_ctx::GGSW * 4));
    int rc = upload_i64(c, din.p, ggsw_in, fheram_ctx::GGSW);
    if (rc != FHERAM_OK) return rc;
    ggsw_inverse(c, din.p, c->d_ggsw_tmp, 1);
    HIPCHK(c, hipGetLastError());
    return download_i64(c, ggsw_out, c->d_ggsw_tmp, fheram_ctx::GGSW);
}

int fheram_timer_begin(fheram_ctx* c) {
    if (!c) return FHERAM_ERR_INVALID_ARG;
    HIPCHK(c, hipSetDevice(c->device));
    HIPCHK(c, hipEventRecord(c->t0, c->stream));
    return FHERAM_OK;
}
int fheram_timer_end(fheram_ctx* c, float* ms) {
    if (!c || !ms) return FHERAM_ERR_INVALID_ARG;
    HIPCHK(c, hipSetDevice(c->device));
// ... 159 lines not shown
```

fhe-ram_amd/csrc/launch.hpp:

```cpp
#pragma once
#include "ctx.hpp"

namespace {

template <typename F>
void with_evk(const fheram_ctx* c, F&& f) {
    if (c->s_evk == 5) f(std::integral_constant<int, 5>{});
    else f(std::integral_constant<int, 4>{});
}
template <typename F>
void with_evk_wide(fheram_ctx* c, bool wide, F&& f) {
    if (wide) c->wide_unsynced = true;
    with_evk(c, [&](auto sk) { if (wide) f(sk, std::true_type{}); else f(sk, std::false_type{}); });
}
bool capturing(const fheram_ctx* c) { return c->cfg.graph && !c->profile; }

constexpr int LIMB_SPLIT_MAX = 64;
constexpr int EW_SLICES = 8;
int pick_nco(const fheram_ctx* c, int gx, int gy, bool one_wg = false) {
    if (c->cfg.nco != 0) return c->cfg.nco;
    if (one_wg) return 2;
    return ((long)gx * gy * 2 <= c->cus) ? 1 : 2;
}
void launch_prepare(fheram_ctx* c, const int32_t* in, double* out, int npoly, int64_t gal = 0) {
    ProfScope ps(c, "prepare", npoly);
    const int ginv = gal == 0 ? 0 : galois_inv_mod(galois_mod(gal));
    hipLaunchKernelGGL(k_prepare, dim3((npoly + 1) / 2), dim3(T), LDS_PREPARE_BYTES, c->cur, in, out, c->d_tw, c->ninv, ginv, npoly);
}
double* big_of(const fheram_ctx* c) { return c->cur == c->stream2 ? c->d_big2 : c->d_big; }
bool use_limb_split(const fheram_ctx* c, int gx, int gy, int sk) {
    return c->cfg.limb_split && (long)gx * gy <= LIMB_SPLIT_MAX && (long)gx * gy * 2 * sk <= c->cus;
}
bool use_fine_split(const fheram_ctx* c, int gx, int gy, int wgs) {
    return c->cfg.limb_split && c->cfg.fine_split && (long)gx * gy * wgs <= c->cus && (long)gx * gy * wgs * N * 8 <= (long)LIMB_SPLIT_MAX * BIG_STRIDE * 8;
}
void launch_ep(fheram_ctx* c, GlweRef a, GlweRef res, const double* ggsw, int gx, int gy) {
    if (gx <= 0 || gy <= 0) return;
    ProfScope ps(c, "ext_product", (uint64_t)gx * gy);
    if (use_fine_split(c, gx, gy, 2 * 4 * 2 * 3)) {
        hipLaunchKernelGGL((k_ext_product_fine<3, 4>), dim3(gx, gy, 2 * 4 * 2 * 3), dim3(T), LDS_BYTES, c->cur, a, ggsw, c->d_tw, big_of(c));
        hipLaunchKernelGGL((k_ext_product_fine_norm<3, 4>), dim3(gx, gy, 2 * (N / 256)), dim3(256), 0, c->cur, res, big_of(c));
        return;
    }
    if (use_limb_split(c, gx, gy, 4)) {
        hipLaunchKernelGGL((k_ext_product<3, 4, 1, 1>), dim3(gx, gy, 8), dim3(T), LDS_BYTES, c->cur, a, res, ggsw, c->d_tw, big_of(c));
        hipLaunchKernelGGL((k_ext_product<3, 4, 1, 2>), dim3(gx, gy, 2), dim3(T), 0, c->cur, a, res, ggsw, c->d_tw, big_of(c));
        return;
    }
    if (pick_nco(c, gx, gy) == 1) hipLaunchKernelGGL((k_ext_product<3, 4, 1>), dim3(gx, gy, 2), dim3(T), LDS_BYTES, c->cur, a, res, ggsw, c->d_tw, big_of(c));
    else {
        ProfScope pf(c, "ext_product_fused", (uint64_t)gx * gy);
        hipLaunchKernelGGL((k_ext_product<3, 4, 2>), dim3(gx, gy, 1), dim3(T), LDS_BYTES, c->cur, a, res, ggsw, c->d_tw, big_of(c));
    }
}
template <int MODE, int SX, int SK, int SO>
void launch_ks(fheram_ctx* c, const KsArgs& ka, int gx, int gy, bool beside = false) {
    if (gx <= 0 || gy <= 0) return;
    ProfScope ps(c, "keyswitch", (uint64_t)gx * gy);
    if (!beside && use_fine_split(c, gx, gy, 2 * SK * SX)) {
        KsArgs kb = ka;
        kb.big = big_of(c);
        hipLaunchKernelGGL((k_keyswitch_fine<MODE, SX, SK>), dim3(gx, gy, 2 * SK * SX), dim3(T), LDS_BYTES, c->cur, kb);
        hipLaunchKernelGGL((k_keyswitch_norm<MODE, SX, SK, SO, SX>), dim3(gx, gy, 2 * (N / 256)), dim3(256), 0, c->cur, kb);
        return;
    }
    if (!beside && use_limb_split(c, gx, gy, SK)) {
        KsArgs kb = ka;
        kb.big = big_of(c);
        hipLaunchKernelGGL((k_keyswitch<MODE, SX, SK, SO, 1, 1>), dim3(gx, gy, 2 * SK), dim3(T), LDS_BYTES, c->cur, kb);
        hipLaunchKernelGGL((k_keyswitch_norm<MODE, SX, SK, SO>), dim3(gx, gy, 2 * (N / 256)), dim3(256), 0, c->cur, kb);
        return;
    }
    constexpr bool FUSABLE = (SX == 3) && (MODE != KS_PAIR);
    if constexpr (MODE == KS_PAIR && SX == 3 && SO == 3) {
        if (c->cfg.pair_z) {
            hipLaunchKernelGGL((k_pair_z<SK>), dim3(gx, gy, 2), dim3(T), LDS_BYTES, c->cur, ka);
            return;
        }
    }
    if (!FUSABLE || pick_nco(c, gx, gy) == 1) {
        hipLaunchKernelGGL((k_keyswitch<MODE, SX, SK, SO, 1>), dim3(gx, gy, 2), dim3(T), LDS_BYTES, c->cur, ka);
    } else if constexpr (FUSABLE) {
        ProfScope pf(c, "keyswitch_fused", (uint64_t)gx * gy);
        hipLaunchKernelGGL((k_keyswitch<MODE, SX, SK, SO, 2>), dim3(gx, gy, 1), dim3(T), LDS_BYTES, c->cur, ka);
    }
}
void launch_copy(fheram_ctx* c, GlweRef src, GlweRef dst, int gx, int gy) {
    if (gx <= 0 || gy <= 0) return;
    ProfScope ps(c, "elementwise", (uint64_t)gx * gy);
    hipLaunchKernelGGL((k_copy<3>), dim3(gx, gy, EW_SLICES), dim3(256), 0, c->cur, src, dst);
}
KsArgs ks_args(fheram_ctx* c, GlweRef a, GlweRef b, GlweRef out, const double* key, int64_t gal, int t = 0, int rot_mul = 0, int rot_base = 0) {
    KsArgs ka;
    ka.a = a; ka.b = b; ka.out = out; ka.key = key; ka.tw = c->d_tw;
    ka.g = galois_mod(gal); ka.ginv = galois_inv_mod(ka.g); ka.t = t; ka.rot_mul = rot_mul; ka.rot_base = rot_base; ka.big = c->d_big;
    return ka;
}
const double* trace_key(fheram_ctx* c, int i) { return c->d_atk + (size_t)i * c->atk; }
template <int MODE>
void launch_ks_tr(fheram_ctx* c, const KsArgs& ka, int gx, int gy) {
    with_evk(c, [&](auto sk) { launch_ks<MODE, 3, decltype(sk)::value, 3>(c, ka, gx, gy); });
}
bool same(const GlweRef& a, const GlweRef& b) { return a.p == b.p; }

template <typename F>
void run_chain(fheram_ctx* c, int n, GlweRef src, GlweRef dst, GlweRef tmp, int gx, int gy, F&& step) {
    if (n <= 0) { if (!same(src, dst)) launch_copy(c, src, dst, gx, gy); return; }
    if (same(src, dst) && (n % 2 == 1)) {
        run_chain(c, n, src, tmp, dst, gx, gy, step);
        launch_copy(c, tmp, dst, gx, gy);
        return;
    }
    GlweRef cur = src;
    for (int i = 0; i < n; i++) {
        GlweRef out = ((n - 1 - i) % 2 == 0) ? dst : tmp;
        step(i, cur, out);
        cur = out;
    }
}
enum class ChainForm { Tail, Mid, Chain, Steps };
struct ChainPlan {
    ChainForm form;
    int split;
};
struct ChainQuery {
    bool ep;
    int n, gx, gy;
    bool rotated = false;
    bool one_wg = false;
    bool handoff = true;
};
ChainPlan chain_form(const fheram_ctx* c, const ChainQuery& q) {
    const long batch = (long)q.gx * q.gy;
    const int sk = q.ep ? 4 : c->s_evk;
    const bool len = q.n >= 2 && q.n <= CHAIN_MAX;
    const bool handoff = q.handoff && len && c->cfg.limb_split &&
                         c->cus >= TAIL_GROUPS * 32 &&
                         !capturing(c);
    if (handoff && !q.ep && !q.rotated && c->cfg.tail && c->cfg.fine_split && batch <= TAIL_GROUPS &&
        c->cur == c->stream &&
        2 * sk * 3 <= 32)
        return {ChainForm::Tail, 0};
    if (handoff && c->cfg.mid && batch > TAIL_GROUPS) {
        if (batch <= 16) return {ChainForm::Mid, 1};
        if (!q.ep && c->cfg.mid >= 2) {
            if (batch <= 8 * (32 / (2 * sk))) return {ChainForm::Mid, 2};
            if (batch <= 8 * (32 / sk)) return {ChainForm::Mid, 3};
        }
    }
    if (len && c->cfg.chain && pick_nco(c, q.gx, q.gy, q.one_wg) == 2 && !use_limb_split(c, q.gx, q.gy, sk) &&
        !use_fine_split(c, q.gx, q.gy, q.ep ? 2 * 4 * 2 * 3 : 2 * sk * 3))
        return {ChainForm::Chain, 0};
    return {ChainForm::Steps, 0};
}
bool chain_bufs(int n, GlweRef src, GlweRef dst, GlweRef tmp, GlweRef (&b)[2]) {
    if (n % 2 == 1) { if (same(src, dst)) return false; b[0] = dst; b[1] = tmp; }
    else { b[0] = tmp; b[1] = dst; }
    return !same(b[0], src);
}
ChainPlan plan_chain(const fheram_ctx* c, ChainQuery q, GlweRef src, GlweRef dst, GlweRef tmp, GlweRef (&b)[2], bool& fits) {
    fits = chain_bufs(q.n, src, dst, tmp, b);
    ChainPlan p = chain_form(c, q);
    if ((p.form == ChainForm::Tail && !(fits && !same(b[1], src))) || (p.form == ChainForm::Mid && !fits)) {
        q.handoff = false;
        p = chain_form(c, q);
    }
    return p;
}
void mid_rearm(fheram_ctx* c) {
    if (!c->cfg.mid && c->mid_saved && ++c->mid_off_ops >= 256) { c->cfg.mid = c->mid_saved; c->mid_saved = 0; c->mid_bad_windows = 0; c->mid_off_ops = 0; }
}
template <bool EP>
void fill_mid(fheram_ctx* c, MidArgs& ma, GlweRef src, GlweRef dst, int n, int gx, int gy) {
    const int side = c->cur == c->stream2 ? 1 : 0;
    ma.src = src; ma.dst = dst; ma.tw = c->d_tw; ma.big = c->d_mid_big[side]; ma.sync = c->d_mid_sync[side]; ma.y = c->d_mid_y[side];
    if (++c->mid_seq == 0) ++c->mid_seq;
    c->mid_launches++;
    c->mid_window_cts += (uint64_t)(gx * gy);
    if (!c->cfg.mid_test && c->mid_launches - c->mid_launch_mark >= 64) {
        const unsigned fb = __atomic_load_n(c->h_mid_fb, __ATOMIC_RELAXED) + __atomic_load_n(c->h_mid_fb + 16, __ATOMIC_RELAXED);
        const unsigned redone = fb - c->mid_fb_mark;
        const bool bad = (uint64_t)redone * 4u > c->mid_window_cts;
        c->mid_bad_windows = bad ? c->mid_bad_windows + 1 : 0;
        if (c->cfg.mid && c->mid_bad_windows >= 2) { c->mid_saved = c->cfg.mid; c->cfg.mid = 0; c->mid_disabled_count++; }
        c->mid_fb_mark = fb;
        c->mid_launch_mark = c->mid_launches;
        c->mid_window_cts = 0;
    }
    ma.seq = c->mid_seq; ma.n = n; ma.n_ct = gx * gy; ma.gx = gx; ma.rot_mul = 0; ma.rot_base = 0;
    ma.give_up_at = c->cfg.mid_test ? n - 2 : -1;
}
template <int SK, int RS, int LPM>
void launch_k_mid_trace(fheram_ctx* c, const MidArgs& ma) {
    constexpr int members = RS * 2 * SK / LPM;
    hipLaunchKernelGGL((k_chain_mid<false, SK, RS, LPM>), dim3(8 * (32 / members) * members), dim3(T), LDS_BYTES, c->cur, ma);
}
void launch_mid_trace(fheram_ctx* c, GlweRef src, const GlweRef (&b)[2], int start, int n, int gx, int gy, int rot_mul, int rot_base, int split) {
    ProfScope ps(c, "keyswitch", (uint64_t)gx * gy, n);
    ProfScope pm(c, "keyswitch_mid_launch", (uint64_t)gx * gy * n, 1);
    MidArgs ma;
    fill_mid<false>(c, ma, src, b[(n - 1) & 1], n, gx, gy);
    ma.rot_mul = rot_mul; ma.rot_base = rot_base;
    KsChainArgs ca;
    ca.base = ks_args(c, src, src, b[0], trace_key(c, start), c->gal[start], 0, rot_mul, rot_base);
    ca.buf[0] = b[0]; ca.buf[1] = b[1]; ca.n = n;
    ca.done = ma.sync; ca.done_seq = ma.seq; ca.host_count = c->h_mid_fb + (c->cur == c->stream2 ? 16 : 0);
    for (int i = 0; i < n; i++) { ma.opnd[i] = ca.key[i] = trace_key(c, start + i); ma.ginv[i] = ca.ginv[i] = galois_inv_mod(galois_mod(c->gal[start + i])); }
    with_evk(c, [&](auto sk) {
        constexpr int SK = decltype(sk)::value;
        if (split == 1) launch_k_mid_trace<SK, 3, 2>(c, ma); else if (split == 2) launch_k_mid_trace<SK, 1, 1>(c, ma); else launch_k_mid_trace<SK, 1, 2>(c, ma);
        hipLaunchKernelGGL((k_keyswitch_chain<3, SK, 3>), dim3(gx, gy, 1), dim3(T), LDS_BYTES, c->cur, ca);
    });
}
void launch_mid_ep(fheram_ctx* c, GlweRef src, const GlweRef (&b)[2], const double* prep, int d, int gx, int gy) {
    ProfScope ps(c, "ext_product", (uint64_t)gx * gy, d);
    ProfScope pm(c, "ext_product_mid_launch", (uint64_t)gx * gy * d, 1);
    MidArgs ma;
    fill_mid<true>(c, ma, src, b[(d - 1) & 1], d, gx, gy);
    EpChainArgs ca;
    ca.src = src; ca.buf[0] = b[0]; ca.buf[1] = b[1]; ca.tw = c->d_tw; ca.n = d;
    ca.done = ma.sync; ca.done_seq = ma.seq; ca.host_count = c->h_mid_fb + (c->cur == c->stream2 ? 16 : 0);
    for (int i = 0; i < d; i++) { ma.opnd[i] = ca.ggsw[i] = prep + (size_t)i * fheram_ctx::GGSW; ma.ginv[i] = 1; }
    hipLaunchKernelGGL((k_chain_mid<true, 4, 3, 2>), dim3(8 * 2 * 12), dim3(T), LDS_BYTES, c->cur, ma);
    hipLaunchKernelGGL((k_ext_product_chain<3, 4>), dim3(gx, gy, 1), dim3(T), LDS_BYTES, c->cur, ca);
}
void launch_ep_chain(fheram_ctx* c, GlweRef src, const GlweRef (&b)[2], const double* prep, int d, int gx, int gy) {
    ProfScope ps(c, "ext_product", (uint64_t)gx * gy, d);
    ProfScope pf(c, "ext_product_fused", (uint64_t)gx * gy, d);
    EpChainArgs ca;
    ca.src = src; ca.buf[0] = b[0]; ca.buf[1] = b[1]; ca.tw = c->d_tw; ca.n = d;
    for (int i = 0; i < d; i++) ca.ggsw[i] = prep + (size_t)i * fheram_ctx::GGSW;
    if (d >= 2) hipLaunchKernelGGL((k_ext_product_chain_r<4>), dim3(gx, gy, 1), dim3(T), LDS_BYTES, c->cur, ca);
    else hipLaunchKernelGGL((k_ext_product_chain<3, 4>), dim3(gx, gy, 1), dim3(T), LDS_BYTES, c->cur, ca);
}
void ep_chain(fheram_ctx* c, GlweRef src, GlweRef dst, GlweRef tmp, const double* prep, int d, int gx, int gy) {
    if (gx <= 0 || gy <= 0) return;
    GlweRef b[2];
    bool fits;
    switch (plan_chain(c, ChainQuery{true, d, gx, gy}, src, dst, tmp, b, fits).form) {
    case ChainForm::Mid: launch_mid_ep(c, src, b, prep, d, gx, gy); return;
    case ChainForm::Chain:
        if (!fits && !chain_bufs(d, src, tmp, dst, b)) break;
        launch_ep_chain(c, src, b, prep, d, gx, gy);
        if (!fits) launch_copy(c, tmp, dst, gx, gy);
        return;
    default: break;
    }
    run_chain(c, d, src, dst, tmp, gx, gy, [&](int i, GlweRef in, GlweRef out) { launch_ep(c, in, out, prep + (size_t)i * fheram_ctx::GGSW, gx, gy); });
}
void launch_trace_chain(fheram_ctx* c, GlweRef src, const GlweRef (&b)[2], int start, int n, int gx, int gy, int rot_mul, int rot_base) {
    ProfScope ps(c, "keyswitch", (uint64_t)gx * gy, n);
    ProfScope pf(c, "keyswitch_fused", (uint64_t)gx * gy, n);
    ProfScope pl(c, "keyswitch_chain_launch", (uint64_t)gx * gy * n, 1);
    KsChainArgs ca;
    ca.base = ks_args(c, src, src, b[0], trace_key(c, start), c->gal[start], 0, rot_mul, rot_base);
    ca.buf[0] = b[0]; ca.buf[1] = b[1]; ca.n = n;
    for (int i = 0; i < n; i++) { ca.key[i] = trace_key(c, start + i); ca.ginv[i] = galois_inv_mod(galois_mod(c->gal[start + i])); }
    const int yf = n >= 2 ? c->cfg.chain_y : 0;
    with_evk_wide(c, yf && c->wide, [&](auto sk, auto w) {
        constexpr int SK = decltype(sk)::value;
        if (!yf) hipLaunchKernelGGL((k_keyswitch_chain<3, SK, 3>), dim3(gx, gy, 1), dim3(T), LDS_BYTES, c->cur, ca);
        else if constexpr (decltype(w)::value) hipLaunchKernelGGL((k_keyswitch_chain_w<3, SK, 3, 3>), dim3(gx, gy, 1), dim3(T), LDS_BYTES, c->cur, ca);
        else hipLaunchKernelGGL((k_keyswitch_chain<3, SK, 3, 3>), dim3(gx, gy, 1), dim3(T), LDS_BYTES, c->cur, ca);
    });
}
struct OpndTable { int ws = 0; long stride = 0; unsigned member_map = 0; bool store_mapped = false; };
constexpr unsigned MEMBER_MAP_IDENTITY = 0x76543210u;
bool map_is_identity(unsigned map, int n) { for (int k = 0; k < n; k++) if (((map >> (4 * k)) & 15u) != (unsigned)k) return false; return true; }
bool use_row_fuse(const fheram_ctx* c, int d, int n_tr, int gx, int gy, bool one_wg = false) {
    return c->cfg.fuse && c->cfg.chain_y == 3 && !capturing(c) &&
           chain_form(c, ChainQuery{true, d, gx, gy, false, one_wg}).form == ChainForm::Chain &&
           chain_form(c, ChainQuery{false, n_tr, gx, gy, false, one_wg}).form == ChainForm::Chain;
}
RowChainTableArgs with_table(const RowChainArgs& ra, const OpndTable& t) {
    RowChainTableArgs rt;
    static_cast<RowChainArgs&>(rt) = ra;
    rt.opnd_stride = t.stride; rt.ws = t.ws; rt.member_map = t.member_map;
    return rt;
}
void fill_row_chain(fheram_ctx* c, RowChainArgs& ra, const double* prep, int d, int start, int n_tr) {
    ra.ep.tw = c->d_tw; ra.ep.n = d;
    for (int i = 0; i < d; i++) ra.ep.ggsw[i] = prep + (size_t)i * fheram_ctx::GGSW;
    ra.ks.n = n_tr;
    for (int i = 0; i < n_tr; i++) { ra.ks.key[i] = trace_key(c, start + i); ra.ks.ginv[i] = galois_inv_mod(galois_mod(c->gal[start + i])); }
}
void launch_read_chain(fheram_ctx* c, GlweRef src, const GlweRef* ep_store, GlweRef dst, const double* prep, int d, int n_tr, int gx, int gy, const OpndTable& t) {
    ProfScope ps(c, "read_chain_launch", (uint64_t)gx * gy, 1);
    RowChainArgs ra;
    fill_row_chain(c, ra, prep, d, 0, n_tr);
    ra.ep.src = src;
    ra.ep.buf[0] = ra.ep.buf[1] = ep_store ? *ep_store : dst;
    ra.store_ep = ep_store ? 1 : 0;
    ra.ks.base = ks_args(c, dst, dst, dst, trace_key(c, 0), c->gal[0]);
    ra.ks.buf[0] = ra.ks.buf[1] = dst;
    ra.hi = dst; ra.trhi = dst;
    if (t.ws > 0) {
        c->wide_unsynced = true;
        if (ep_store && t.store_mapped) {
            read_chain_m_launch(c->s_evk, dim3(gx, gy, 1), c->cur, with_table(ra, t));
            return;
        }
        with_evk(c, [&](auto sk) {
            constexpr int SK = decltype(sk)::value;
            hipLaunchKernelGGL((k_read_chain_t<SK, 4>), dim3(gx, gy, 1), dim3(T), LDS_BYTES, c->cur, with_table(ra, t));
        });
        return;
    }
    with_evk_wide(c, c->wide, [&](auto sk, auto w) {
        constexpr int SK = decltype(sk)::value;
        if constexpr (decltype(w)::value) hipLaunchKernelGGL((k_read_chain_w<SK, 4>), dim3(gx, gy, 1), dim3(T), LDS_BYTES, c->cur, ra);
        else hipLaunchKernelGGL((k_read_chain<SK, 4>), dim3(gx, gy, 1), dim3(T), LDS_BYTES, c->cur, ra);
    });
}
void launch_write_chain(fheram_ctx* c, GlweRef src, int rot_mul, int rot_base, GlweRef data, GlweRef trhi, const double* prep, int d, int n_tr, int gx, int gy, const OpndTable& t,
                        const GlweRef* tree = nullptr, int tree_rho = 0) {
    ProfScope ps(c, "write_chain_launch", (uint64_t)gx * gy, 1);
    RowChainArgs ra;
    fill_row_chain(c, ra, prep, d, 0, n_tr);
    ra.ks.base = ks_args(c, src, src, data, trace_key(c, 0), c->gal[0], 0, rot_mul, rot_base);
    ra.ks.buf[0] = ra.ks.buf[1] = data;
    ra.hi = data; ra.trhi = trhi;
    ra.ep.src = data; ra.ep.buf[0] = ra.ep.buf[1] = data;
    if (tree) { ra.tree = *tree; ra.tree_rho = tree_rho; }
    c->wide_unsynced = true;
    if (t.ws > 0 && t.store_mapped) {
        write_chain_m_launch(c->s_evk, dim3(gx, gy, 1), c->cur, with_table(ra, t));
        return;
    }
    with_evk(c, [&](auto sk) {
        constexpr int SK = decltype(sk)::value;
        if (t.ws > 0) hipLaunchKernelGGL((k_write_chain_t<SK, 4>), dim3(gx, gy, 1), dim3(T), LDS_BYTES, c->cur, with_table(ra, t));
        else hipLaunchKernelGGL((k_write_chain<SK, 4>), dim3(gx, gy, 1), dim3(T), LDS_BYTES, c->cur, ra);
    });
}
void launch_trace_tail(fheram_ctx* c, GlweRef src, const GlweRef (&b)[2], int start, int n, int gx, int gy,
                       const double* prep = nullptr, int d = 0, GlweRef ep_out = GlweRef{nullptr, 0, 0}, bool store_ep = false, const OpndTable& t = {}) {
    ProfScope ps(c, "keyswitch", (uint64_t)gx * gy, n);
    ProfScope pt(c, "keyswitch_tail_launch", (uint64_t)gx * gy * n, 1);
    TailArgs ta;
    ta.src = src; ta.buf[0] = b[0]; ta.buf[1] = b[1]; ta.tw = c->d_tw; ta.big = big_of(c); ta.sync = c->d_tail_sync;
    ta.n_ep = prep ? d : 0; ta.ep_out = ep_out;
    ta.host_done = c->d_h_tail_done;
    for (int i = 0; i < TAIL_EP_MAX; i++) ta.ggsw[i] = (prep && i < d) ? prep + (size_t)i * fheram_ctx::GGSW : nullptr;
    if (++c->tail_seq == 0) ++c->tail_seq;
    c->tail_launches++;
    if (c->cfg.tail_test != 1 && c->tail_launches - c->tail_launch_mark >= 64) {
        const unsigned fb = *(volatile unsigned*)c->h_tail_fb;
        if (fb - c->tail_fb_mark > 16) c->cfg.tail = 0;
        c->tail_fb_mark = fb;
        c->tail_launch_mark = c->tail_launches;
    }
    ta.seq = c->tail_seq; ta.n = n; ta.n_ct = gx * gy; ta.gx = gx; ta.xoff = c->tail_xoff; ta.give_up_at = c->cfg.tail_test ? ta.n_ep + n - 2 : -1;
    KsChainArgs ca;
    ca.base = ks_args(c, src, src, b[0], trace_key(c, start), c->gal[start], 0, 0, 0);
    ca.buf[0] = b[0]; ca.buf[1] = b[1]; ca.n = n;
    ca.pred = c->d_tail_sync + TAIL_GROUPS * 32; ca.pred_seq = ta.seq; ca.host_count = c->h_tail_fb;
    for (int i = 0; i < n; i++) { ta.key[i] = ca.key[i] = trace_key(c, start + i); ta.ginv[i] = ca.ginv[i] = galois_inv_mod(galois_mod(c->gal[start + i])); }
    RowChainArgs ra;
    if (ta.n_ep) {
        fill_row_chain(c, ra, prep, d, start, n);
        ra.ep.src = src; ra.ep.buf[0] = ra.ep.buf[1] = ep_out; ra.store_ep = store_ep ? 1 : 0;
        ra.ks.base = ks_args(c, b[(n - 1) & 1], b[(n - 1) & 1], b[(n - 1) & 1], trace_key(c, start), c->gal[start]);
        ra.ks.buf[0] = ra.ks.buf[1] = b[(n - 1) & 1];
        ra.hi = ra.trhi = b[(n - 1) & 1];
        ra.ks.pred = ca.pred; ra.ks.pred_seq = ca.pred_seq; ra.ks.host_count = ca.host_count;
    }
    with_evk(c, [&](auto sk) {
        constexpr int SK = decltype(sk)::value;
        const dim3 groups(TAIL_GROUPS * 2 * SK * 3);
        if (t.ws > 0 && ta.n_ep) {
            TailTableArgs tt;
            static_cast<TailArgs&>(tt) = ta;
            tt.opnd_stride = t.stride; tt.ws = t.ws;
            hipLaunchKernelGGL((k_trace_tail_t<3, SK, 3>), groups, dim3(T), LDS_BYTES, c->cur, tt);
            c->wide_unsynced = true;
            hipLaunchKernelGGL((k_read_chain_t<SK, 4>), dim3(gx, gy, 1), dim3(T), LDS_BYTES, c->cur, with_table(ra, OpndTable{t.ws, t.stride, MEMBER_MAP_IDENTITY}));
            return;
        }
        hipLaunchKernelGGL((k_trace_tail<3, SK, 3>), groups, dim3(T), LDS_BYTES, c->cur, ta);
        if (ta.n_ep) hipLaunchKernelGGL((k_read_chain<SK, 4>), dim3(gx, gy, 1), dim3(T), LDS_BYTES, c->cur, ra);
        else hipLaunchKernelGGL((k_keyswitch_chain<3, SK, 3>), dim3(gx, gy, 1), dim3(T), LDS_BYTES, c->cur, ca);
    });
}
void trace_steps(fheram_ctx* c, GlweRef src, GlweRef dst, GlweRef tmp, int start, int end, int gx, int gy, int rot_mul = 0, int rot_base = 0) {
    if (gx <= 0 || gy <= 0) return;
    const int n = end - start;
    GlweRef b[2];
    bool fits;
    const ChainPlan p = plan_chain(c, ChainQuery{false, n, gx, gy, rot_mul != 0 || rot_base != 0}, src, dst, tmp, b, fits);
    switch (p.form) {
    case ChainForm::Tail: launch_trace_tail(c, src, b, start, n, gx, gy); return;
    case ChainForm::Mid: launch_mid_trace(c, src, b, start, n, gx, gy, rot_mul, rot_base, p.split); return;
    case ChainForm::Chain:
        if (!fits && !chain_bufs(n, src, tmp, dst, b)) break;
        launch_trace_chain(c, src, b, start, n, gx, gy, rot_mul, rot_base);
        if (!fits) launch_copy(c, tmp, dst, gx, gy);
        return;
    case ChainForm::Steps: break;
    }
    run_chain(c, n, src, dst, tmp, gx, gy, [&](int i, GlweRef in, GlweRef out) {
        KsArgs ka = ks_args(c, in, in, out, trace_key(c, start + i), c->gal[start + i], 0, i == 0 ? rot_mul : 0, i == 0 ? rot_base : 0);
        launch_ks_tr<KS_TRACE>(c, ka, gx, gy);
    });
}
int32_t* pack_levels(fheram_ctx* c, int32_t* src, int32_t* A, int32_t* B, long sy, long sx, size_t count, int gy,
                     int n_alone, int first_pair, bool keep_alone = false, int32_t* P0 = nullptr, int32_t* P1 = nullptr) {
    const int k = ilog2_ceil(count);
    int32_t* cur = src;
    auto other = [&](int32_t* x) { return x == A ? B : A; };
    if (n_alone > 0 && count > 0) {
        int32_t* b0 = other(src);
        int32_t* b1 = other(b0);
        if (b1 == src && P0 && P0 != src && chain_form(c, ChainQuery{false, n_alone, (int)count, gy}).form == ChainForm::Tail) b1 = P0;
        cur = keep_alone ? A : ((n_alone - 1) & 1) ? b1 : b0;
        trace_steps(c, ref(src, sy, sx), ref(cur, sy, sx), ref(cur == b0 ? b1 : b0, sy, sx), 0, n_alone, (int)count, gy);
    }
    size_t live = count;
    for (int m = 0; m < k; m++) {
        const int i = first_pair + m;
        const long h = (long)1 << (k - 1 - m);
        int32_t* nxt = (keep_alone && P0) ? (cur == P0 ? P1 : P0) : other(cur);
        const long n_pair = std::max<long>(0, std::min<long>(h, (long)live - h));
        const long n_alone_here = std::min<long>(h, (long)live) - n_pair;
        if (n_pair > 0) {
            KsArgs ka = ks_args(c, ref(cur, sy, sx), ref(cur + h * sx, sy, sx), ref(nxt, sy, sx), trace_key(c, i), c->gal[i], N >> (i + 1));
            launch_ks_tr<KS_PAIR>(c, ka, (int)n_pair, gy);
        }
        if (n_alone_here > 0) {
            KsArgs ka = ks_args(c, ref(cur + n_pair * sx, sy, sx), ref(cur, sy, sx), ref(nxt + n_pair * sx, sy, sx), trace_key(c, i), c->gal[i]);
            launch_ks_tr<KS_TRACE>(c, ka, (int)n_alone_here, gy);
        }
        live = std::min<size_t>(live, (size_t)h);
        cur = nxt;
    }
    return cur;
}
int coord_first_digit(const fheram_ctx* c, int ci) { int s = 0; for (int i = 0; i < ci; i++) s += (int)c->base2d[i].size(); return s; }
double* digits_of(const fheram_ctx* c, double* table, int ci) { return table + (size_t)coord_first_digit(c, ci) * fheram_ctx::GGSW; }
void coordinate_prepare(fheram_ctx* c, const fheram_addr* addr, int ci, double* table) {
    const int d = (int)c->base2d[ci].size();
    launch_prepare(c, addr->d_ggsw + (size_t)coord_first_digit(c, ci) * fheram_ctx::GGSW, digits_of(c, table, ci), d * (int)(fheram_ctx::GGSW / N));
}
void coordinate_prepare_all(fheram_ctx* c, const fheram_addr* addr, double* table) {
    launch_prepare(c, addr->d_ggsw, table, c->n_digits * (int)(fheram_ctx::GGSW / N));
}
void ggsw_inverse(fheram_ctx* c, const int32_t* in, int32_t* tmp, int d, bool beside = false) {
    const long g4 = (long)fheram_ctx::GLWE4;
    int32_t* inp = const_cast<int32_t*>(in);
    KsArgs ka = ks_args(c, ref(inp, (long)fheram_ctx::GGSW, 2 * g4), ref(inp, 0, 0), ref(tmp, (long)fheram_ctx::GGSW, 2 * g4), c->d_atk_inv, -1);
    launch_ks<KS_AUTO, 4, 5, 4>(c, ka, fheram_ctx::DNUM_CT, d, beside);
    KsArgs kt = ks_args(c, ref(tmp, (long)fheram_ctx::GGSW, 2 * g4), ref(tmp, 0, 0), ref(tmp + g4, (long)fheram_ctx::GGSW, 2 * g4), c->d_tsk, 1);
    launch_ks<KS_TENSOR, 4, 5, 4>(c, kt, fheram_ctx::DNUM_CT, d, beside);
}
void coordinate_prepare_inv(fheram_ctx* c, const int32_t* digits, int d, int32_t* tmp, double* prep, bool beside = false) {
    ggsw_inverse(c, digits, tmp, d, beside);
    launch_prepare(c, tmp, prep, d * (int)(fheram_ctx::GGSW / N));
}
void coordinate_prepare_inv(fheram_ctx* c, const fheram_addr* addr, int ci, int32_t* tmp, double* prep, bool beside = false) {
    coordinate_prepare_inv(c, addr->d_ggsw + (size_t)coord_first_digit(c, ci) * fheram_ctx::GGSW, (int)c->base2d[ci].size(), tmp, prep, beside);
}

void precompute_inverse(fheram_ctx* c, const fheram_addr* addr, int ci, bool fork, unsigned gate_seq = 0) {
    if (fork && c->wdone_pending) {
        hipStreamWaitEvent(c->stream2, c->ev_wdone, 0);
        c->wdone_pending = false;
    }
    if (fork && gate_seq) {
        if (c->opstart_valid) { hipStreamWaitEvent(c->stream2, c->ev_opstart, 0); c->opstart_valid = false; }
        hipLaunchKernelGGL(k_tail_gate, dim3(1), dim3(64), 0, c->stream2, c->d_tail_sync + TAIL_GROUPS * 32 + 2, gate_seq);
    } else if (fork) {
        hipEventRecord(c->ev_fork, c->stream);
        hipStreamWaitEvent(c->stream2, c->ev_fork, 0);
    }
    hipStream_t keep = c->cur;
    c->cur = c->stream2;
    coordinate_prepare_inv(c, addr, ci, c->d_ggsw_inv + (size_t)coord_first_digit(c, ci) * fheram_ctx::GGSW, digits_of(c, c->d_prep_inv, ci), true);
    hipEventRecord(c->ev_inv[ci], c->stream2);
    c->cur = keep;
    c->inv_id[ci] = addr->id;
    c->inv_pending[ci] = true;
}
void wait_inverse(fheram_ctx* c, hipStream_t s, int ci) { if (!capturing(c)) hipStreamWaitEvent(s, c->ev_inv[ci], 0); }

}
```

fhe-ram_amd/csrc/path.hpp:

```cpp
#pragma once
#include "launch.hpp"

namespace {

struct Opnds {
    fheram_ctx* c;
    RamState* st;
    const fheram_addr* const* addrs;
    int n, ws;
    double *tab, *tab_inv;
    long stride;
    unsigned member_map;
    bool bank;
    int member(int k) const { return (int)((member_map >> (4 * k)) & 15u); }
    bool rows_dense() const { return map_is_identity(member_map, n); }
    int Y() const { return n * ws; }
    double* prep(int k, int ci) const { return digits_of(c, tab + k * stride, ci); }
    double* inv(int k, int ci) const { return digits_of(c, tab_inv + k * stride, ci); }
    GlweRef slice(GlweRef r, int k) const { r.p += (long)k * ws * r.sy; return r; }
    GlweRef rows(GlweRef r, int k) const { return slice(r, member(k)); }
    OpndTable table() const { return n == 1 ? OpndTable{} : OpndTable{ws, stride, member_map, !rows_dense()}; }
    bool row_fuse(int d, int n_tr, int gx) const { return use_row_fuse(c, d, n_tr, gx, Y(), bank); }
};
Opnds one_addr(fheram_ctx* c, const fheram_addr* const* a, int ws, RamState* st) { return Opnds{c, st, a, 1, ws, c->d_prep, c->d_prep_inv, 0, 0, false}; }
Opnds one_addr(fheram_ctx* c, const fheram_addr* const* a) { return one_addr(c, a, c->ws, &c->ram); }
Opnds table_opnds(fheram_ctx* c, RamState* st, const fheram_addr* const* addrs, int n, int ws, double* tab, double* tab_inv, unsigned member_map, bool bank) {
    return Opnds{c, st, addrs, n, ws, tab, tab_inv, (long)c->n_digits * (long)fheram_ctx::GGSW, member_map, bank};
}

struct RamView {
    int32_t *rows, *A, *B, *C, *D;
    int32_t *part, *tmp, *tmp2, *res, *tree, *w, *trtop;
};
RamView ctx_view(const fheram_ctx* c) {
    return RamView{c->d_data, c->d_scrA, c->d_scrB, c->d_scrC, c->d_scrD, c->d_part, c->d_tmp, c->d_tmp2, c->d_res, c->d_tree, c->d_w, c->d_trtop};
}

void read_local_done(const fheram_ctx* c, RamState* st, bool prepare_write) {
    if (c->n2 == 2) st->memo_alone = (prepare_write && c->cfg.memo) ? LOGN - ilog2_ceil(c->rows_glob) : 0;
}
void read_top_done(fheram_ctx* c, RamState* st, bool prepare_write) {
    st->memo_top = prepare_write && c->cfg.memo;
    st->res_in_trtop = st->memo_top;
    c->prep1_ready = false;
}
void write_done(fheram_ctx* c, RamState* st) { st->memo_top = false; st->memo_alone = 0; c->side_begun = false; c->tree_rotate_pending = false; }

template <typename F>
int run_op(fheram_ctx* c, const fheram_addr* addr, int which, F&& enqueue) {
    if (!capturing(c)) return enqueue();
    main_enqueued(c);
    fheram_addr* a = const_cast<fheram_addr*>(addr);
    const unsigned sig = 1u | (c->ram.memo_top ? 2u : 0u) | ((unsigned)c->ram.memo_alone << 2) | (c->side_begun ? 64u : 0u) |
                         (c->inv_id[0] == addr->id ? 128u : 0u) | (c->inv_id[1] == addr->id ? 256u : 0u);
    if (a->graph[which] && a->graph_sig[which] != sig) { hipGraphExecDestroy(a->graph[which]); a->graph[which] = nullptr; }
    if (!a->graph[which]) {
        hipGraph_t g = nullptr;
        HIPCHK(c, hipStreamBeginCapture(c->stream, hipStreamCaptureModeThreadLocal));
        const int rc = enqueue();
        const hipError_t e = hipStreamEndCapture(c->stream, &g);
        if (rc != FHERAM_OK || e != hipSuccess) {
            if (g) hipGraphDestroy(g);
            return rc != FHERAM_OK ? rc : fail(c, FHERAM_ERR_DEVICE, std::string("hipStreamEndCapture: ") + hipGetErrorString(e));
        }
        const hipError_t e2 = hipGraphInstantiate(&a->graph[which], g, nullptr, nullptr, 0);
        hipGraphDestroy(g);
        if (e2 != hipSuccess) { a->graph[which] = nullptr; return fail(c, FHERAM_ERR_DEVICE, std::string("hipGraphInstantiate: ") + hipGetErrorString(e2)); }
        a->graph_sig[which] = sig;
    }
    HIPCHK(c, hipGraphLaunch(a->graph[which], c->stream));
    if (which == 2) write_done(c, &c->ram);
    else { read_local_done(c, &c->ram, which == 1); read_top_done(c, &c->ram, which == 1); }
    return FHERAM_OK;
}

int check_common(fheram_ctx* c, const fheram_addr* addr) {
    if (!c) return FHERAM_ERR_INVALID_ARG;
    mid_rearm(c);
    if (!addr || addr->ctx != c) return fail(c, FHERAM_ERR_INVALID_ARG, "address does not belong to this context (layout mismatch, ram.rs:404)");
    if (addr->empty) return fail(c, FHERAM_ERR_INVALID_ARG, "empty address: fheram_address_alloc without fheram_address_derive");
    if (!c->ram.initialized) return fail(c, FHERAM_ERR_UNINITIALIZED, "unitialized memory: self.data.len()=0");
    if (!c->keys_loaded) return fail(c, FHERAM_ERR_KEYS, "evaluation keys not loaded");
    return FHERAM_OK;
}

int read_local(const Opnds& o, const RamView& a, bool prepare_write, GlweRef* packed_out, bool to_part) {
    fheram_ctx* c = o.c;
    const int n = o.n, ws = o.ws, Y = o.Y(), R = (int)c->rows;
    main_enqueued(c);
    c->wide = !prepare_write || n > 1;
    if (n == 1 && prepare_write && c->cfg.pre_inv == 1 && !capturing(c) && (c->wide_unsynced || c->derive_unsynced)) {
        hipEventRecord(c->ev_opstart, c->stream);
        c->opstart_valid = true;
    }
    const long G = (long)fheram_ctx::GLWE;
    const long sy = (long)c->rows * G;
    GlweRef data = ref(a.rows, sy, G), A = ref(a.A, sy, G), B = ref(a.B, sy, G);
    GlweRef part = ref(a.part, G, 0);
    const bool all = (c->n_shards == 1 && c->n2 == 2);
    for (int k = 0; k < n; k++)
        if (all) coordinate_prepare_all(c, o.addrs[k], o.tab + k * o.stride); else coordinate_prepare(c, o.addrs[k], 0, o.tab + k * o.stride);
    c->prep1_ready = all;
    read_local_done(c, o.st, prepare_write);
    const int d0 = (int)c->base2d[0].size();
    if (c->n2 == 1) {
        GlweRef row0 = ref(a.rows, sy, 0);
        for (int k = 0; k < n; k++)
            if (prepare_write) ep_chain(c, o.rows(row0, k), o.rows(row0, k), o.slice(ref(a.A, sy, 0), k), o.prep(k, 0), d0, 1, ws);
            else ep_chain(c, o.rows(row0, k), o.slice(part, k), o.slice(ref(a.tmp, G, 0), k), o.prep(k, 0), d0, 1, ws);
        const bool gather = prepare_write && !o.rows_dense();
        if (gather) for (int k = 0; k < n; k++) launch_copy(c, o.rows(row0, k), o.slice(part, k), 1, ws);
        *packed_out = (prepare_write && !gather) ? row0 : part;
        if (prepare_write && to_part && !gather) launch_copy(c, row0, part, 1, Y);
        return FHERAM_OK;
    }
    const int L0 = LOGN - ilog2_ceil(c->rows_glob);
    const bool keep = o.st->memo_alone > 0;
    int32_t* packed;
    if (o.row_fuse(d0, L0, R) && !(prepare_write && (d0 & 1))) {
        launch_read_chain(c, data, prepare_write ? &data : nullptr, A, o.prep(0, 0), d0, L0, R, Y, o.table());
        packed = pack_levels(c, a.A, a.A, a.B, sy, G, (size_t)R, Y, 0, L0, keep, a.C, a.D);
    } else {
        for (int k = 0; k < n; k++)
            if (prepare_write) ep_chain(c, o.rows(data, k), o.rows(data, k), o.slice(A, k), o.prep(k, 0), d0, R, ws);
            else ep_chain(c, o.rows(data, k), o.slice(A, k), o.slice(B, k), o.prep(k, 0), d0, R, ws);
        int32_t* leaves = prepare_write ? a.rows : a.A;
        if (prepare_write && !o.rows_dense()) {
            for (int k = 0; k < n; k++) launch_copy(c, o.rows(data, k), o.slice(ref(a.D, sy, G), k), R, ws);
            leaves = a.D;
        }
        packed = pack_levels(c, leaves, a.A, a.B, sy, G, (size_t)R, Y, L0, L0, keep, a.C, a.D);
    }
    *packed_out = ref(packed, sy, 0);
    if (to_part) launch_copy(c, *packed_out, part, 1, Y);
    return FHERAM_OK;
}
int read_top(const Opnds& o, const RamView& a, bool prepare_write, int32_t* gathered, GlweRef pk) {
    fheram_ctx* c = o.c;
    const int n = o.n, ws = o.ws, Y = o.Y();
    main_enqueued(c);
    c->wide = !prepare_write || n > 1;
    const long G = (long)fheram_ctx::GLWE;
    GlweRef tmp = ref(a.tmp, G, 0);
    GlweRef last = pk;
    const int d1 = c->n2 == 2 ? (int)c->base2d[1].size() : 0;
    auto tail_top = [&] { return chain_form(c, ChainQuery{false, LOGN, 1, Y}).form == ChainForm::Tail; };
    const bool fuse_ep = c->n2 == 2 && c->cfg.tail_ep && d1 >= 2 && d1 <= TAIL_EP_MAX && tail_top();
    GlweRef ep_out = ref(prepare_write ? a.tree : a.tmp2, G, 0);
    auto products1 = [&] { for (int k = 0; k < n; k++) ep_chain(c, o.slice(pk, k), o.slice(ep_out, k), o.slice(tmp, k), o.prep(k, 1), d1, 1, ws); };
    if (c->n2 == 2) {
        if (gathered) {
            const int kG = ilog2_ceil((size_t)c->n_shards);
            int32_t* a0 = c->d_gat[1];
            int32_t* a1 = c->d_gat[2];
            int32_t* packed = pack_levels(c, gathered, a0, a1, G, (long)ws * G, (size_t)c->n_shards, ws, 0, LOGN - kG);
            pk = ref(packed, G, 0);
        }
        if (!c->prep1_ready) coordinate_prepare(c, o.addrs[0], 1, o.tab);
        if (!fuse_ep) products1();
        last = ep_out;
    }
    const bool pre = n == 1 && prepare_write && c->cfg.pre_inv && (long)c->rows * Y <= c->cus;
    const bool gated = pre && c->cfg.pre_inv == 1 && !capturing(c) && tail_top();
    if (pre && !gated)
        for (int ci = c->n2 - 1; ci >= 0; ci--) precompute_inverse(c, o.addrs[0], ci, ci == c->n2 - 1);
    read_top_done(c, o.st, prepare_write);
    const GlweRef res = ref(o.st->memo_top ? a.trtop : a.res, G, 0);
    const uint64_t tl0 = c->tail_launches;
    GlweRef tb[2];
    if (fuse_ep && chain_bufs(LOGN, last, res, tmp, tb))
        launch_trace_tail(c, pk, tb, 0, LOGN, 1, Y, o.prep(0, 1), d1, ep_out, prepare_write, o.table());
    else {
        if (fuse_ep) products1();
        trace_steps(c, last, res, tmp, 0, LOGN, 1, Y);
    }
    if (gated && !c->opstart_valid && (c->wide_unsynced || c->derive_unsynced)) {
        hipEventRecord(c->ev_opstart, c->stream);
        c->opstart_valid = true;
    }
    if (gated) {
        const unsigned seq = c->tail_launches != tl0 ? c->tail_seq : 0;
        for (int ci = c->n2 - 1; ci >= 0; ci--) precompute_inverse(c, o.addrs[0], ci, ci == c->n2 - 1, seq);
    }
    c->tail_wait.note_top(c->tail_launches != tl0 ? c->tail_seq : 0);
    return FHERAM_OK;
}
int read_impl(const Opnds& o, const RamView& a, bool prepare_write) {
    fheram_ctx* c = o.c;
    GlweRef packed;
    int rc = read_local(o, a, prepare_write, &packed, false);
    if (rc != FHERAM_OK) return rc;
    rc = read_top(o, a, prepare_write, nullptr, packed);
    if (o.n == 1 && prepare_write && c->inv_id[0] == o.addrs[0]->id && capturing(c))
        for (int ci = 0; ci < c->n2; ci++) hipStreamWaitEvent(c->stream, c->ev_inv[ci], 0);
    if (rc == FHERAM_OK && prepare_write) o.st->state = true;
    return rc;
}

struct HostStage {
    unsigned char *d = nullptr, *h = nullptr;
    hipEvent_t ev = nullptr;
    bool busy = false;
    template <typename T> T* dev() const { return reinterpret_cast<T*>(d); }
    template <typename T> T* host() const { return reinterpret_cast<T*>(h); }
    hipError_t pin(size_t bytes) { return hipHostMalloc((void**)&h, bytes, hipHostMallocDefault); }
    hipError_t event() { return hipEventCreateWithFlags(&ev, hipEventDisableTiming); }
};
int stage_wait(fheram_ctx* c, HostStage& s) {
    if (s.busy) { HIPCHK(c, hipEventSynchronize(s.ev)); s.busy = false; }
    return FHERAM_OK;
}
int stage_record(fheram_ctx* c, HostStage& s) {
    HIPCHK(c, hipEventRecord(s.ev, c->stream));
    s.busy = true;
    return FHERAM_OK;
}
void bufs_free(std::initializer_list<void*> device, std::initializer_list<void*> pinned, std::initializer_list<hipEvent_t> events) {
    for (void* p : device) if (p) hipFree(p);
    for (void* p : pinned) if (p) hipHostFree(p);
    for (hipEvent_t e : events) if (e) hipEventDestroy(e);
}
hipError_t pinned_result(int64_t** h, int64_t** d_h, size_t ct) {
    const hipError_t e = hipHostMalloc((void**)h, ct * 2 + sizeof(int64_t), hipHostMallocMapped);
    return e == hipSuccess ? hipHostGetDevicePointer((void**)d_h, *h, 0) : e;
}
int reserve_failed(fheram_ctx* c, hipError_t e, const std::string& what) {
    (void)hipGetLastError();
    return fail(c, FHERAM_ERR_DEVICE, what + ": " + hipGetErrorString(e));
}

void dense_free(DenseBufs& L) {
    bufs_free({L.A, L.B, L.C, L.D, L.part, L.tmp, L.tmp2, L.res, L.tree, L.w, L.trtop, L.prep}, {L.h_res}, {});
    L = DenseBufs{};
}
bool third_arena_needed(const fheram_ctx* c, int n_ct) {
    return c->n2 == 2 && chain_form(c, ChainQuery{false, LOGN - ilog2_ceil(c->rows_glob), (int)c->rows, n_ct}).form == ChainForm::Tail;
}
int dense_reserve(fheram_ctx* c, DenseBufs& L, int n, int ws, bool all = false, int* fail_alloc = nullptr) {
    const bool work = all || n > 1, third = all || (work && third_arena_needed(c, n * ws));
    if (n <= L.cap && (!work || L.A) && (!third || L.C)) return FHERAM_OK;
    if (n < L.cap) n = L.cap;
    const bool with_work = work || L.A, with_third = third || L.C;
    if (L.cap) {
        HIPCHK(c, hipStreamSynchronize(c->stream));
        if (all) HIPCHK(c, hipStreamSynchronize(c->stream2));
        dense_free(L);
    }
    const size_t ct = (size_t)n * ws * fheram_ctx::GLWE * sizeof(int32_t), row = ct * c->rows;
    hipError_t e = hipSuccess;
    auto dev = [&](auto** p, size_t bytes) {
        if (e != hipSuccess) return;
        if (fail_alloc && *fail_alloc > 0 && --*fail_alloc == 0) e = hipErrorOutOfMemory;
        else e = hipMalloc((void**)p, bytes);
    };
    if (all) {
        for (int32_t** p : {&L.A, &L.B, &L.C, &L.D}) dev(p, row);
        for (int32_t** p : {&L.part, &L.tmp, &L.tmp2, &L.res, &L.tree, &L.w, &L.trtop}) dev(p, ct);
    } else {
        dev(&L.res, ct);
        if (with_work) {
            for (int32_t** p : {&L.A, &L.B}) dev(p, row);
            if (with_third) dev(&L.C, row);
            for (int32_t** p : {&L.tmp, &L.tmp2}) dev(p, ct);
            dev(&L.prep, (size_t)n * c->n_digits * fheram_ctx::GGSW * sizeof(double));
        }
        if (e == hipSuccess) e = pinned_result(&L.h_res, &L.d_h_res, ct);
    }
    if (e != hipSuccess) {
        dense_free(L);
        return reserve_failed(c, e, all ? "buffers of a write list of " + std::to_string(n) + " members" : "read buffers for " + std::to_string(n) + " addresses");
    }
    L.cap = n;
    return FHERAM_OK;
}
RamView dense_view(const fheram_ctx* c, const DenseBufs& L) {
    return RamView{c->d_data, L.A, L.B, L.C, L.D, L.part ? L.part : L.tmp2, L.tmp, L.tmp2, L.res, L.tree, L.w, L.trtop};
}

struct SelectBufs {
    int cap = 0, prep_cap = 0, host_cap = 0;
    int32_t *packed = nullptr, *ep = nullptr, *tmp = nullptr, *tmp2 = nullptr, *res = nullptr;
    double* prep = nullptr;
    int64_t *h_res = nullptr, *d_h_res = nullptr;
    HostStage host;
};
void select_free(SelectBufs& S) {
    bufs_free({S.packed, S.ep, S.tmp, S.tmp2, S.res, S.prep, S.host.d}, {S.h_res, S.host.h}, {S.host.ev});
    S = SelectBufs{};
}
using SelectLaneTable = HostStage;
void lane_table_free(SelectLaneTable& L) {
    bufs_free({L.d}, {L.h}, {L.ev});
    L = SelectLaneTable{};
}

struct OneRowSet {
    int cap = 0;
    int32_t *fan = nullptr, *ep = nullptr, *tmp = nullptr, *res = nullptr;
    double* prep = nullptr;
    int64_t *h_res = nullptr, *d_h_res = nullptr;
    HostStage stage;
};
void one_row_free(OneRowSet& S) {
    bufs_free({S.fan, S.ep, S.tmp, S.res, S.prep, S.stage.d}, {S.h_res, S.stage.h}, {S.stage.ev});
    S = OneRowSet{};
}
int one_row_reserve(fheram_ctx* c, OneRowSet& S, int ws, int prep_digits, size_t stage_bytes, const char* what) {
    if (S.cap) return FHERAM_OK;
    OneRowSet nw;
    nw.cap = std::min(FHERAM_SELECT_MAX * ws, 64);
    const size_t ct = (size_t)nw.cap * fheram_ctx::GLWE * sizeof(int32_t);
    hipError_t e = hipSuccess;
    for (int32_t** p : {&nw.fan, &nw.ep, &nw.tmp, &nw.res}) if (e == hipSuccess) e = hipMalloc((void**)p, ct);
    if (e == hipSuccess) e = hipMalloc((void**)&nw.prep, (size_t)FHERAM_SELECT_MAX * prep_digits * fheram_ctx::GGSW * sizeof(double));
    if (e == hipSuccess) e = hipMalloc((void**)&nw.stage.d, stage_bytes);
    if (e == hipSuccess) e = pinned_result(&nw.h_res, &nw.d_h_res, ct);
    if (e == hipSuccess) e = nw.stage.pin(stage_bytes);
    if (e == hipSuccess) e = nw.stage.event();
    if (e != hipSuccess) { one_row_free(nw); return reserve_failed(c, e, what); }
    S = nw;
    return FHERAM_OK;
}

struct PublicBufs {
    int cap = 0;
    int32_t *fan = nullptr, *tmp = nullptr, *res[2] = {nullptr, nullptr};
    int cur = 0;
    int64_t *h_res = nullptr, *d_h_res = nullptr;
    HostStage host;
    HostStage data;
};
void public_bufs_free(PublicBufs& P) {
    bufs_free({P.fan, P.tmp, P.res[0], P.res[1], P.host.d, P.data.d}, {P.h_res, P.host.h, P.data.h}, {P.host.ev, P.data.ev});
    P = PublicBufs{};
}

struct MixBufs {
    int cap = 0;
    int32_t *ep = nullptr, *tmp = nullptr, *res[3] = {nullptr, nullptr, nullptr};
    int64_t *h_res = nullptr, *d_h_res = nullptr;
    int32_t *own = nullptr, *keep = nullptr;
    double* prep = nullptr;
};
void mix_bufs_free(MixBufs& M) {
    bufs_free({M.ep, M.tmp, M.res[0], M.res[1], M.res[2], M.own, M.keep, M.prep}, {M.h_res}, {});
    M = MixBufs{};
}
struct ResHome {
    const int32_t* res = nullptr;
    int64_t *h = nullptr, *d_h = nullptr;
    int mix_slot = -1;
};

struct ResRun { const int32_t* src; size_t n; };
int result_export(fheram_ctx* c, const ResRun* runs, int n_runs, int64_t* h, int64_t* d_h, int64_t* out) {
    size_t n = 0;
    for (int i = 0; i < n_runs; i++) {
        const int n4 = (int)(runs[i].n / 4);
        hipLaunchKernelGGL(k_export_i64, dim3((n4 + 255) / 256), dim3(256), 0, c->stream, runs[i].src, reinterpret_cast<long long*>(d_h + n), n4,
                           reinterpret_cast<const long long*>(c->d_tw + N));
        n += runs[i].n;
    }
    HIPCHK(c, hipStreamSynchronize(c->stream));
    HIPCHK(c, hipGetLastError());
    main_waited(c);
    double m;
    std::memcpy(&m, h + n, 8);
    if (c->cfg.monitor && m > MON_LIMIT) __atomic_store_n(c->h_ro_flag, 1u, __ATOMIC_RELAXED);
    const int rc = check_precision(c);
    if (rc == FHERAM_OK && out) std::memcpy(out, h, n * sizeof(int64_t));
    return rc;
}

int reads_export(fheram_ctx* c, const DenseBufs& L, size_t first, size_t n_ct, int64_t* out) {
    const ResRun run{L.res + first * fheram_ctx::GLWE, n_ct * fheram_ctx::GLWE};
    return result_export(c, &run, 1, L.h_res, L.d_h_res, out);
}
template <typename F>
int read_many(fheram_ctx* c, DenseBufs& L, RamState* st, const fheram_addr* const* addrs, int n, int ws, unsigned member_map, bool bank, int64_t* out, F&& kept) {
    int rc = dense_reserve(c, L, n, ws);
    if (rc != FHERAM_OK) return rc;
    const Opnds o = table_opnds(c, st, addrs, n, ws, L.prep, nullptr, member_map, bank);
    rc = read_impl(o, dense_view(c, L), false);
    if (rc != FHERAM_OK) return rc;
    kept(o);
    HIPCHK(c, hipGetLastError());
    return out ? reads_export(c, L, 0, (size_t)n * ws, out) : FHERAM_OK;
}

int write_top(const Opnds& o, const RamView& v) {
    fheram_ctx* c = o.c;
    main_enqueued(c);
    c->wide = true;
    const long G = (long)fheram_ctx::GLWE;
    const long sy = (long)c->rows * G;
    const int n = o.n, ws = o.ws, Y = o.Y();
    GlweRef wref = ref(v.w, G, 0), tmp = ref(v.tmp, G, 0), tmp2 = ref(v.tmp2, G, 0), tree = ref(v.tree, G, 0);
    GlweRef top = (c->n2 != 1) ? tree : ref(v.rows, sy, 0);
    GlweRef tr = tmp;
    const bool by_member = c->n2 == 1 && !o.rows_dense();
    if (o.st->memo_top) tr = ref(v.trtop, G, 0);
    else if (by_member) for (int k = 0; k < n; k++) trace_steps(c, o.rows(top, k), o.slice(tmp, k), o.slice(tmp2, k), 0, LOGN, 1, ws);
    else trace_steps(c, top, tmp, tmp2, 0, LOGN, 1, Y);
    if (by_member) {
        ProfScope ps(c, "elementwise", Y);
        for (int k = 0; k < n; k++)
            hipLaunchKernelGGL((k_sub_add_norm<3>), dim3(1, ws, EW_SLICES), dim3(256), 0, c->cur, o.rows(top, k), o.slice(tr, k), o.slice(wref, k), o.rows(top, k));
    } else {
        ProfScope ps(c, "elementwise", Y);
        hipLaunchKernelGGL((k_sub_add_norm<3>), dim3(1, Y, EW_SLICES), dim3(256), 0, c->cur, top, tr, wref, top);
    }
    o.st->memo_top = false;
    if (c->n2 == 2) {
        if (n == 1 && c->inv_id[1] == o.addrs[0]->id) wait_inverse(c, c->stream, 1);
        else {
            if (n == 1 && c->inv_pending[1]) wait_inverse(c, c->stream, 1);
            for (int k = 0; k < n; k++) coordinate_prepare_inv(c, o.addrs[k], 1, c->d_ggsw_tmp, o.inv(k, 1));
        }
        if (n == 1) { c->inv_pending[1] = false; c->inv_id[1] = 0; }
        for (int k = 0; k < n; k++)
            ep_chain(c, o.slice(tree, k), o.slice(ref(v.part, G, 0), k), o.slice(tmp, k), o.inv(k, 1), (int)c->base2d[1].size(), 1, ws);
        c->tree_rotate_pending = true;
    }
    return FHERAM_OK;
}
void write_side_begin(const Opnds& o, const RamView& v) {
    fheram_ctx* c = o.c;
    c->wide = true;
    const long G = (long)fheram_ctx::GLWE;
    const long sy = (long)c->rows * G;
    if (!(c->main_idle && !capturing(c) && c->n_shards == 1)) {
        hipEventRecord(c->ev_fork, c->stream);
        hipStreamWaitEvent(c->stream2, c->ev_fork, 0);
    }
    main_enqueued(c);
    c->cur = c->stream2;
    if (c->n2 == 2) {
        const int kept = o.st->memo_alone;
        c->trhi_in_C = kept > 0 && (LOGN - kept) % 2 == 1;
        if (kept > 0) trace_steps(c, ref(v.A, sy, G), ref(c->trhi_in_C ? v.C : v.A, sy, G), ref(c->trhi_in_C ? v.A : v.C, sy, G), kept, LOGN, (int)c->rows, o.Y());
        else if (!o.rows_dense())
            for (int k = 0; k < o.n; k++) trace_steps(c, o.rows(ref(v.rows, sy, G), k), o.slice(ref(v.A, sy, G), k), o.slice(ref(v.C, sy, G), k), 0, LOGN, (int)c->rows, o.ws);
        else trace_steps(c, ref(v.rows, sy, G), ref(v.A, sy, G), ref(v.C, sy, G), 0, LOGN, (int)c->rows, o.Y());
        o.st->memo_alone = 0;
    }
    if (o.n == 1 && c->inv_id[0] == o.addrs[0]->id) wait_inverse(c, c->stream2, 0);
    else for (int k = 0; k < o.n; k++) coordinate_prepare_inv(c, o.addrs[k], 0, c->d_ggsw_tmp2, o.inv(k, 0));
    if (o.n == 1) { c->inv_id[0] = 0; c->inv_pending[0] = false; }
    hipEventRecord(c->ev_join, c->stream2);
    c->cur = c->stream;
    c->side_begun = true;
}
void write_side_abort(fheram_ctx* c) {
    if (!c->side_begun) return;
    hipStreamWaitEvent(c->stream, c->ev_join, 0);
    c->side_begun = false;
}
int write_rows(const Opnds& o, const RamView& v) {
    fheram_ctx* c = o.c;
    main_enqueued(c);
    c->wide = true;
    const long G = (long)fheram_ctx::GLWE;
    const long sy = (long)c->rows * G;
    const int n = o.n, ws = o.ws, Y = o.Y(), R = (int)c->rows;
    GlweRef data = ref(v.rows, sy, G), A = ref(v.A, sy, G), B = ref(v.B, sy, G), D = ref(v.D, sy, G);
    GlweRef trhi = ref(c->trhi_in_C ? v.C : v.A, sy, G), part = ref(v.part, G, 0);
    const int d0 = (int)c->base2d[0].size();
    const bool fuse = c->n2 == 2 && o.row_fuse(d0, LOGN, R);
    const bool rot_in_chain = fuse && c->tree_rotate_pending && c->n_shards == 1;
    const GlweRef tree = ref(v.tree, G, 0);
    if (fuse) {
        hipStreamWaitEvent(c->stream, c->ev_join, 0);
        launch_write_chain(c, part, c->n_shards, c->shard, data, trhi, o.inv(0, 0), d0, LOGN, R, Y, o.table(), rot_in_chain ? &tree : nullptr, -(int)c->rows_glob);
    } else if (c->n2 == 2)
        trace_steps(c, part, B, D, 0, LOGN, R, Y, c->n_shards, c->shard);
    if (c->tree_rotate_pending && !rot_in_chain) {
        ProfScope ps(c, "elementwise", Y);
        hipLaunchKernelGGL((k_rotate<3>), dim3(1, Y, EW_SLICES), dim3(256), 0, c->cur, part, ref(v.tree, G, 0), -(int)c->rows_glob);
    }
    if (!fuse) {
        hipStreamWaitEvent(c->stream, c->ev_join, 0);
        if (c->n2 == 2) {
            ProfScope ps(c, "elementwise", (uint64_t)R * Y);
            if (o.rows_dense()) hipLaunchKernelGGL((k_sub_add_norm<3>), dim3(R, Y, EW_SLICES), dim3(256), 0, c->cur, data, trhi, B, data);
            else for (int k = 0; k < n; k++)
                hipLaunchKernelGGL((k_sub_add_norm<3>), dim3(R, ws, EW_SLICES), dim3(256), 0, c->cur, o.rows(data, k), o.slice(trhi, k), o.slice(B, k), o.rows(data, k));
        }
        for (int k = 0; k < n; k++) ep_chain(c, o.rows(data, k), o.rows(data, k), o.slice(A, k), o.inv(k, 0), d0, R, ws);
    }
    if (n == 1 && !capturing(c)) { hipEventRecord(c->ev_wdone, c->stream); c->wdone_pending = true; }
    write_done(c, o.st);
    o.st->state = false;
    return FHERAM_OK;
}

template <typename S>
int write_all(const Opnds& o, const RamView& v, S&& stage) {
    write_side_begin(o, v);
    int rc = stage(v.w, o.Y());
    if (rc != FHERAM_OK) { write_side_abort(o.c); return rc; }
    rc = write_top(o, v);
    return rc == FHERAM_OK ? write_rows(o, v) : rc;
}

}
```

fhe-ram_amd/csrc/setup.hpp:

```cpp
#pragma once
#include "launch.hpp"

namespace {
void wipe_free(hipStream_t st, void* d, size_t bytes) {
    if (!d) return;
    if (hipMemsetAsync(d, 0, bytes, st) == hipSuccess) hipStreamSynchronize(st);
    hipFree(d);
}
void wipe_host(void* p, size_t bytes) {
    volatile unsigned char* v = static_cast<volatile unsigned char*>(p);
    for (size_t i = 0; i < bytes; i++) v[i] = 0;
}
}

namespace {

constexpr int64_t NOISE_LIM = (int64_t)1 << 30;
int noise_limb(int k) { return (k + BASE2K - 1) / BASE2K - 1; }

template <int S, int DEC>
void launch_enc(fheram_ctx* c, int32_t* cts, const double* s_hat, const int32_t* pt1, int n) {
    ProfScope ps(c, "encrypt", (uint64_t)n);
    hipLaunchKernelGGL((k_encrypt_sk<S, DEC>), dim3(n), dim3(T), LDS_BYTES, c->cur, cts, s_hat, c->d_tw, pt1);
}
bool launch_enc_dyn(fheram_ctx* c, int S, int dec, int32_t* cts, const double* s_hat, const int32_t* pt1, int n) {
    if (n <= 0) return true;
    switch (S * 2 + dec) {
        case 3: launch_enc<1, 1>(c, cts, s_hat, pt1, n); return true;
        case 6: launch_enc<3, 0>(c, cts, s_hat, pt1, n); return true;
        case 7: launch_enc<3, 1>(c, cts, s_hat, pt1, n); return true;
        case 8: launch_enc<4, 0>(c, cts, s_hat, pt1, n); return true;
        case 9: launch_enc<4, 1>(c, cts, s_hat, pt1, n); return true;
        case 10: launch_enc<5, 0>(c, cts, s_hat, pt1, n); return true;
        case 11: launch_enc<5, 1>(c, cts, s_hat, pt1, n); return true;
    }
    return false;
}
bool stage_random(int32_t* pre, int S, int k, const int64_t* mask, const int64_t* noise) {
    int64_t bad = 0;
    for (int j = 0; j < S; j++) {
        int32_t* m = pre + (size_t)(j * 2 + 1) * N;
        const int64_t* src = mask + (size_t)j * N;
        for (int i = 0; i < N; i++) { const int64_t v = src[i]; bad |= (v > 65535) | (v < -65536); m[i] = (int32_t)v; }
    }
    int32_t* b = pre + (size_t)(noise_limb(k) * 2) * N;
    for (int i = 0; i < N; i++) { const int64_t e = noise[i]; bad |= (e >= NOISE_LIM) | (e <= -NOISE_LIM); b[i] += (int32_t)e; }
    return bad == 0;
}
int check_setup_args(fheram_ctx* c, const fheram_secret* sk, int S, int k) {
    if (!sk || sk->ctx != c) return fail(c, FHERAM_ERR_INVALID_ARG, "secret belongs to another context");
    if (k <= 0 || noise_limb(k) >= S) return fail(c, FHERAM_ERR_INVALID_ARG, "precision k does not fit the ciphertext's limbs");
    return FHERAM_OK;
}
int encrypt_staged(fheram_ctx* c, const double* s_hat, int32_t* d_dst, const std::vector<int32_t>& pre,
                   const std::vector<int32_t>* pt1, int n, int S) {
    int32_t* d_pt1 = nullptr;
    HIPCHK(c, hipMemcpyAsync(d_dst, pre.data(), (size_t)n * S * 2 * N * sizeof(int32_t), hipMemcpyHostToDevice, c->stream));
    if (pt1) {
        HIPCHK(c, hipMalloc(&d_pt1, (size_t)n * S * N * sizeof(int32_t)));
        hipError_t e = hipMemcpyAsync(d_pt1, pt1->data(), (size_t)n * S * N * sizeof(int32_t), hipMemcpyHostToDevice, c->stream);
        if (e != hipSuccess) { hipFree(d_pt1); return fail(c, FHERAM_ERR_DEVICE, std::string("hipMemcpyAsync: ") + hipGetErrorString(e)); }
    }
    c->cur = c->stream;
    const bool ok = launch_enc_dyn(c, S, 0, d_dst, s_hat, d_pt1, n);
    hipError_t e = hipStreamSynchronize(c->stream);
    if (d_pt1) hipFree(d_pt1);
    if (!ok) return fail(c, FHERAM_ERR_UNSUPPORTED, "ciphertext size must be 3, 4 or 5 limbs");
    if (e != hipSuccess) return fail(c, FHERAM_ERR_DEVICE, std::string("k_encrypt_sk: ") + hipGetErrorString(e));
    HIPCHK(c, hipGetLastError());
    return FHERAM_OK;
}
void host_automorphism(int64_t g, const int32_t* a, int32_t* res) {
    const int64_t m = 2 * N, gg = ((g % m) + m) % m;
    for (int i = 0; i < N; i++) {
        const int64_t j = (int64_t)i * gg % m;
        if (j >= N) res[j - N] = -a[i]; else res[j] = a[i];
    }
}
void encode_value(int64_t v, int k_pt, int size_pt, int32_t* limbs ) {
    int64_t x = (int64_t)((uint64_t)v << (size_pt * BASE2K - k_pt)), carry = 0;
    for (int j = size_pt - 1; j >= 0; j--) {
        const int64_t t = (j == size_pt - 1 ? x : 0) + carry;
        const int64_t d = (int64_t)((uint64_t)t << (64 - BASE2K)) >> (64 - BASE2K);
        limbs[j] = (int32_t)d;
        carry = (t - d) >> BASE2K;
    }
}

}

extern "C" {

int fheram_secret_create(fheram_ctx* c, const int64_t* sk, fheram_secret** out) {
    if (!c || !out) return FHERAM_ERR_INVALID_ARG;
    *out = nullptr;
    if (!sk) return fail(c, FHERAM_ERR_INVALID_ARG, "null secret");
    HIPCHK(c, hipSetDevice(c->device));
    fheram_secret* s = new fheram_secret{c, c->device, std::vector<int32_t>(N), nullptr};
    for (int i = 0; i < N; i++) {
        if (sk[i] < -1 || sk[i] > 1) { delete s; return fail(c, FHERAM_ERR_RANGE, "secret coefficients must be in {-1, 0, 1}"); }
        s->sk[i] = (int32_t)sk[i];
    }
    int32_t* d_in = nullptr;
    hipError_t e = hipMalloc(&d_in, N * sizeof(int32_t));
    if (e == hipSuccess) e = hipMalloc(&s->d_hat, N * sizeof(double));
    if (e == hipSuccess) e = hipMemcpyAsync(d_in, s->sk.data(), N * sizeof(int32_t), hipMemcpyHostToDevice, c->stream);
    if (e == hipSuccess) { c->cur = c->stream; launch_prepare(c, d_in, s->d_hat, 1); e = hipStreamSynchronize(c->stream); }
    wipe_free(c->stream, d_in, N * sizeof(int32_t));
    if (e != hipSuccess) { fheram_secret_destroy(s); return fail(c, FHERAM_ERR_DEVICE, std::string("secret prepare: ") + hipGetErrorString(e)); }
    *out = s;
    return FHERAM_OK;
}
void fheram_secret_destroy(fheram_secret* s) {
    if (!s) return;
    hipSetDevice(s->device);
    wipe_free(nullptr, s->d_hat, N * sizeof(double));
    wipe_host(s->sk.data(), s->sk.size() * sizeof(int32_t));
    delete s;
}

int fheram_glwe_encrypt_sk(fheram_ctx* c, const fheram_secret* sk, int n_glwe, int size, int k, const int64_t* pt,
                           int pt_size, int pt_col, const int64_t* mask, const int64_t* noise, int64_t* out) {
    if (!c) return FHERAM_ERR_INVALID_ARG;
    if (!mask || !noise || !out || n_glwe <= 0) return fail(c, FHERAM_ERR_INVALID_ARG, "null argument / empty batch");
    if (size < 3 || size > 5) return fail(c, FHERAM_ERR_UNSUPPORTED, "ciphertext size must be 3, 4 or 5 limbs");
    if (pt && (pt_size <= 0 || (pt_col != 0 && pt_col != 1))) return fail(c, FHERAM_ERR_INVALID_ARG, "bad plaintext shape");
    int rc = check_setup_args(c, sk, size, k);
    if (rc != FHERAM_OK) return rc;
    HIPCHK(c, hipSetDevice(c->device));
    const size_t glen = (size_t)size * 2 * N;
    std::vector<int32_t> pre((size_t)n_glwe * glen, 0), pt1;
    if (pt && pt_col == 1) pt1.assign((size_t)n_glwe * size * N, 0);
    const int np = pt ? std::min(pt_size, size) : 0;
    for (int g = 0; g < n_glwe; g++) {
        int32_t* pg = pre.data() + (size_t)g * glen;
        for (int j = 0; j < np; j++) {
            const int64_t* src = pt + ((size_t)g * pt_size + j) * N;
            int32_t* dst = pt_col == 0 ? pg + (size_t)(j * 2) * N : pt1.data() + ((size_t)g * size + j) * N;
            for (int i = 0; i < N; i++) {
                if (src[i] > 65536 || src[i] < -65536) return fail(c, FHERAM_ERR_RANGE, "plaintext limb out of the normalised range [-2^16, 2^16]");
                dst[i] = (int32_t)src[i];
            }
        }
        if (!stage_random(pg, size, k, mask + (size_t)g * size * N, noise + (size_t)g * N))
            return fail(c, FHERAM_ERR_RANGE, "mask limb outside [-2^16, 2^16) or |noise| >= 2^30");
    }
    int32_t* d_ct = nullptr;
    HIPCHK(c, hipMalloc(&d_ct, pre.size() * sizeof(int32_t)));
    rc = encrypt_staged(c, sk->d_hat, d_ct, pre, pt1.empty() ? nullptr : &pt1, n_glwe, size);
    if (rc == FHERAM_OK) rc = download_i64(c, out, d_ct, pre.size());
    hipFree(d_ct);
    return rc;
}

int fheram_glwe_decrypt(fheram_ctx* c, const fheram_secret* sk, int n_glwe, int size, const int64_t* ct, int64_t* pt) {
    if (!c) return FHERAM_ERR_INVALID_ARG;
    if (!ct || !pt || n_glwe <= 0) return fail(c, FHERAM_ERR_INVALID_ARG, "null argument / empty batch");
    if (size < 3 || size > 5) return fail(c, FHERAM_ERR_UNSUPPORTED, "ciphertext size must be 3, 4 or 5 limbs");
    if (!sk || sk->ctx != c) return fail(c, FHERAM_ERR_INVALID_ARG, "secret belongs to another context");
    HIPCHK(c, hipSetDevice(c->device));
    const size_t glen = (size_t)size * 2 * N, total = (size_t)n_glwe * glen;
    int32_t* d_ct = nullptr;
    HIPCHK(c, hipMalloc(&d_ct, total * sizeof(int32_t)));
    int rc = upload_i64(c, d_ct, ct, total);
    if (rc == FHERAM_OK) {
        c->cur = c->stream;
        launch_enc_dyn(c, size, 1, d_ct, sk->d_hat, nullptr, n_glwe);
        std::vector<int32_t> h_i32(total);
        hipError_t e = hipMemcpyAsync(h_i32.data(), d_ct, total * sizeof(int32_t), hipMemcpyDeviceToHost, c->stream);
        if (e == hipSuccess) e = hipStreamSynchronize(c->stream);
        if (e != hipSuccess) rc = fail(c, FHERAM_ERR_DEVICE, std::string("decrypt: ") + hipGetErrorString(e));
        else
            for (int g = 0; g < n_glwe; g++)
                for (int j = 0; j < size; j++)
                    widen(h_i32.data() + (size_t)g * glen + (size_t)(j * 2) * N, pt + ((size_t)g * size + j) * N, N);
    }
    hipFree(d_ct);
    return rc;
}

}
namespace {
struct RamShape { size_t ws, rows, max_addr; int shard, n_shards; };
int ram_encrypt_body(fheram_ctx* c, const fheram_secret* sk, const uint8_t* data, size_t data_len, const int64_t* mask, const int64_t* noise,
                     const RamShape& sh, int32_t* d_rows, bool check_draws) {
    if (!data || !mask || !noise) return fail(c, FHERAM_ERR_INVALID_ARG, "null argument");
    const size_t ws = sh.ws;
    if (data_len % ws != 0) return fail(c, FHERAM_ERR_INVALID_ARG, "invalid data: data.len()%ram_chunks != 0");
    if (data_len / ws != sh.max_addr) return fail(c, FHERAM_ERR_INVALID_ARG, "invalid data: data.len()/ram_chunks != max_addr");
    const int k = (int)c->p.k_glwe_ct, S = fheram_ctx::S_CT;
    int rc = check_setup_args(c, sk, S, k);
    if (rc != FHERAM_OK) return rc;
    const int k_pt = (int)c->p.k_glwe_pt, size_pt = (k_pt + BASE2K - 1) / BASE2K;
    if (k_pt <= 0 || k_pt > 8 + BASE2K || size_pt > S) return fail(c, FHERAM_ERR_UNSUPPORTED, "k_glwe_pt out of range");
    if (check_draws) {
        int64_t bad = 0;
        const size_t n_noise = ws * sh.rows * N, n_mask = n_noise * S;
        for (size_t i = 0; i < n_mask; i++) bad |= (mask[i] > 65535) | (mask[i] < -65536);
        for (size_t i = 0; i < n_noise; i++) bad |= (noise[i] >= NOISE_LIM) | (noise[i] <= -NOISE_LIM);
        if (bad) return fail(c, FHERAM_ERR_RANGE, "mask limb outside [-2^16, 2^16) or |noise| >= 2^30");
    }
    HIPCHK(c, hipSetDevice(c->device));
    const size_t G = fheram_ctx::GLWE, max_addr = sh.max_addr;
    const size_t CH = 256;
    std::vector<int32_t> pre(std::min(CH, sh.rows) * G);
    int32_t limbs[4];
    for (size_t w = 0; w < ws; w++)
        for (size_t x0 = 0; x0 < sh.rows; x0 += CH) {
            const size_t nx = std::min(CH, sh.rows - x0);
            std::fill(pre.begin(), pre.begin() + nx * G, 0);
            for (size_t x = 0; x < nx; x++) {
                const size_t r = (size_t)sh.shard + (x0 + x) * (size_t)sh.n_shards;
                int32_t* pg = pre.data() + x * G;
                for (size_t q = 0; q < (size_t)N; q++) {
                    const size_t a = r * N + q;
                    if (a >= max_addr) break;
                    encode_value((int64_t)(int8_t)data[a * ws + w], k_pt, size_pt, limbs);
                    for (int j = 0; j < size_pt; j++) pg[(size_t)(j * 2) * N + q] = limbs[j];
                }
                const size_t gi = w * sh.rows + x0 + x;
                if (!stage_random(pg, S, k, mask + gi * S * N, noise + gi * N))
                    return fail(c, FHERAM_ERR_RANGE, "mask limb outside [-2^16, 2^16) or |noise| >= 2^30");
            }
            rc = encrypt_staged(c, sk->d_hat, d_rows + (w * sh.rows + x0) * G, pre, nullptr, (int)nx, S);
            if (rc != FHERAM_OK) return rc;
        }
    return FHERAM_OK;
}

struct DigitPlan {
    int n_digits = 0;
    unsigned char rsh[32] = {}, width[32] = {}, lsh[32] = {};
    unsigned char coord_rsh[32] = {}, coord_bits[32] = {};
};
int digits_encrypt_body(fheram_ctx* c, const fheram_secret* sk, uint32_t value, const DigitPlan& pl, const int64_t* mask, const int64_t* noise,
                        int32_t* d_ggsw) {
    const int S = fheram_ctx::S_ADDR, k = (int)c->p.k_ggsw_addr, D = fheram_ctx::DNUM_CT;
    const size_t glen = fheram_ctx::GLWE4;
    const int n = pl.n_digits * D * 2;
    std::vector<int32_t> pre((size_t)n * glen, 0), pt1((size_t)n * S * N, 0);
    int gi = 0;
    for (int d = 0; d < pl.n_digits; d++) {
        const size_t rem_c = ((size_t)value >> pl.coord_rsh[d]) & (((size_t)1 << pl.coord_bits[d]) - 1);
        const bool neg = rem_c != 0;
        const size_t chunk = (((size_t)value >> pl.rsh[d]) & (((size_t)1 << pl.width[d]) - 1)) << pl.lsh[d];
        const size_t pos = (neg && chunk != 0) ? (size_t)N - chunk : chunk;
        const int32_t sgn = (neg && chunk != 0) ? -1 : 1;
        for (int r = 0; r < D; r++)
            for (int ci = 0; ci < 2; ci++, gi++) {
                int32_t* pg = pre.data() + (size_t)gi * glen;
                if (ci == 0) pg[(size_t)(r * 2) * N + pos] = sgn;
                else pt1[((size_t)gi * S + r) * N + pos] = sgn;
                if (!stage_random(pg, S, k, mask + (size_t)gi * S * N, noise + (size_t)gi * N))
                    return fail(c, FHERAM_ERR_RANGE, "mask limb outside [-2^16, 2^16) or |noise| >= 2^30");
            }
    }
    return encrypt_staged(c, sk->d_hat, d_ggsw, pre, &pt1, n, S);
}
}
extern "C" {

int fheram_ram_encrypt_sk(fheram_ctx* c, const fheram_secret* sk, const uint8_t* data, size_t data_len,
                          const int64_t* mask, const int64_t* noise) {
    if (!c) return FHERAM_ERR_INVALID_ARG;
    const int rc = ram_encrypt_body(c, sk, data, data_len, mask, noise, RamShape{(size_t)c->ws, c->rows, (size_t)c->p.max_addr, c->shard, c->n_shards}, c->d_data, false);
    if (rc != FHERAM_OK) return rc;
    c->ram.initialized = true; c->ram.state = false;
    return FHERAM_OK;
}

int fheram_address_encrypt_sk(fheram_ctx* c, const fheram_secret* sk, uint32_t value, const int64_t* mask,
                              const int64_t* noise, fheram_addr** out) {
    if (!c || !out) return FHERAM_ERR_INVALID_ARG;
    *out = nullptr;
    if (!mask || !noise) return fail(c, FHERAM_ERR_INVALID_ARG, "null argument");
    int rc = check_setup_args(c, sk, fheram_ctx::S_ADDR, (int)c->p.k_ggsw_addr);
    if (rc != FHERAM_OK) return rc;
    HIPCHK(c, hipSetDevice(c->device));
    DigitPlan pl;
    unsigned bits = 0;
    for (auto& base1d : c->base2d) {
        unsigned tot = 0, lsh = 0;
        for (int b : base1d) tot += (unsigned)b;
        for (int b : base1d) {
            if (pl.n_digits >= 32) return fail(c, FHERAM_ERR_UNSUPPORTED, "digit plans of more than 32 digits");
            const int d = pl.n_digits++;
            pl.rsh[d] = (unsigned char)(bits + lsh); pl.width[d] = (unsigned char)b; pl.lsh[d] = (unsigned char)lsh;
            pl.coord_rsh[d] = (unsigned char)bits; pl.coord_bits[d] = (unsigned char)tot;
            lsh += (unsigned)b;
        }
        bits += tot;
    }
    if (bits < 32 && ((uint64_t)value >> bits) != 0)
        return fail(c, FHERAM_ERR_INVALID_ARG, "self.base2d.max() > value (address.rs:98): address does not fit the digit plan");
    fheram_addr* a = new fheram_addr{c, nullptr, c->n_digits, c->device};
    hipError_t e = hipMalloc(&a->d_ggsw, (size_t)c->n_digits * fheram_ctx::GGSW * sizeof(int32_t));
    if (e != hipSuccess) { delete a; return fail(c, FHERAM_ERR_DEVICE, std::string("hipMalloc: ") + hipGetErrorString(e)); }
    rc = digits_encrypt_body(c, sk, value, pl, mask, noise, a->d_ggsw);
    if (rc != FHERAM_OK) { fheram_address_destroy(a); return rc; }
    *out = a;
    return FHERAM_OK;
}
int fheram_address_download(fheram_ctx* c, const fheram_addr* a, int64_t* out) {
    if (!c || !out) return FHERAM_ERR_INVALID_ARG;
    if (!a || a->ctx != c) return fail(c, FHERAM_ERR_INVALID_ARG, "address belongs to another context");
    if (a->empty) return fail(c, FHERAM_ERR_INVALID_ARG, "empty address: fheram_address_alloc without fheram_address_derive");
    HIPCHK(c, hipSetDevice(c->device));
    return download_i64(c, out, a->d_ggsw, (size_t)a->n_digits * fheram_ctx::GGSW);
}

int fheram_keys_encrypt_sk(fheram_ctx* c, const fheram_secret* sk, const int64_t* mask, const int64_t* noise, int64_t* std_out) {
    if (!c) return FHERAM_ERR_INVALID_ARG;
    if (!mask || !noise) return fail(c, FHERAM_ERR_INVALID_ARG, "null argument");
    int rc = check_setup_args(c, sk, c->s_evk, (int)c->p.k_evk_trace);
    if (rc == FHERAM_OK) rc = check_setup_args(c, sk, fheram_ctx::S_INV, (int)c->p.k_evk_ggsw_inv);
    if (rc != FHERAM_OK) return rc;
    HIPCHK(c, hipSetDevice(c->device));
    HIPCHK(c, hipStreamSynchronize(c->stream));
    HIPCHK(c, hipStreamSynchronize(c->stream2));
    c->cur = c->stream;
    int32_t *d_stage = nullptr, *d_small = nullptr;
    double* d_hat = nullptr;
    const size_t stage_n = std::max(c->atk, fheram_ctx::EVK5);
    HIPCHK(c, hipMalloc(&d_stage, stage_n * sizeof(int32_t)));
    hipError_t e = hipMalloc(&d_small, 2 * N * sizeof(int32_t));
    if (e == hipSuccess) e = hipMalloc(&d_hat, N * sizeof(double));
    if (e != hipSuccess) { hipFree(d_stage); if (d_small) hipFree(d_small); return fail(c, FHERAM_ERR_DEVICE, std::string("hipMalloc: ") + hipGetErrorString(e)); }
    std::vector<int32_t> sk_out(N), ss(2 * N, 0), pre;
    auto gglwe = [&](const int32_t* scalar, const double* hat, int rows, int S, int k, double* d_prepared, int64_t* std_dst, int64_t gal) -> int {
        const size_t glen = (size_t)S * 2 * N;
        pre.assign((size_t)rows * glen, 0);
        for (int r = 0; r < rows; r++) {
            int32_t* pg = pre.data() + (size_t)r * glen;
            if (r < S) std::copy(scalar, scalar + N, pg + (size_t)(r * 2) * N);
            if (!stage_random(pg, S, k, mask + (size_t)r * S * N, noise + (size_t)r * N))
                return fail(c, FHERAM_ERR_RANGE, "mask limb outside [-2^16, 2^16) or |noise| >= 2^30");
        }
        mask += (size_t)rows * S * N; noise += (size_t)rows * N;
        int rc2 = encrypt_staged(c, hat, d_stage, pre, nullptr, rows, S);
        if (rc2 == FHERAM_OK && std_dst) rc2 = download_i64(c, std_dst, d_stage, (size_t)rows * glen);
        if (rc2 == FHERAM_OK) { launch_prepare(c, d_stage, d_prepared, (int)((size_t)rows * glen / N), gal); hipStreamSynchronize(c->stream); }
        return rc2;
    };
    auto automorphism_key = [&](int64_t p, int rows, int S, int k, double* d_prepared, int64_t* std_dst) -> int {
        host_automorphism(galois_inv_mod(galois_mod(p)), sk->sk.data(), sk_out.data());
        hipMemcpyAsync(d_small, sk_out.data(), N * sizeof(int32_t), hipMemcpyHostToDevice, c->stream);
        launch_prepare(c, d_small, d_hat, 1);
        hipStreamSynchronize(c->stream);
        return gglwe(sk->sk.data(), d_hat, rows, S, k, d_prepared, std_dst, p);
    };
    for (int i = 0; i < LOGN && rc == FHERAM_OK; i++)
        rc = automorphism_key(c->gal[i], fheram_ctx::DNUM_CT, c->s_evk, (int)c->p.k_evk_trace,
                              c->d_atk + (size_t)i * c->atk, std_out ? std_out + (size_t)i * c->atk : nullptr);
    if (rc == FHERAM_OK) {
        std::copy(sk->sk.begin(), sk->sk.end(), ss.begin() + N);
        hipMemcpyAsync(d_small, ss.data(), 2 * N * sizeof(int32_t), hipMemcpyHostToDevice, c->stream);
        launch_enc_dyn(c, 1, 1, d_small, sk->d_hat, nullptr, 1);
        hipMemcpyAsync(ss.data(), d_small, N * sizeof(int32_t), hipMemcpyDeviceToHost, c->stream);
        if (hipStreamSynchronize(c->stream) != hipSuccess) rc = fail(c, FHERAM_ERR_DEVICE, "tensor key: s*s failed");
    }
    if (rc == FHERAM_OK)
        rc = gglwe(ss.data(), sk->d_hat, fheram_ctx::DNUM_GGSW, fheram_ctx::S_INV, (int)c->p.k_evk_ggsw_inv, c->d_tsk,
                   std_out ? std_out + (size_t)LOGN * c->atk : nullptr, 0);
    if (rc == FHERAM_OK)
        rc = automorphism_key(-1, fheram_ctx::DNUM_GGSW, fheram_ctx::S_INV, (int)c->p.k_evk_ggsw_inv, c->d_atk_inv,
                              std_out ? std_out + (size_t)LOGN * c->atk + fheram_ctx::EVK5 : nullptr);
    hipFree(d_stage);
    wipe_free(c->stream, d_small, 2 * N * sizeof(int32_t));
    wipe_free(c->stream, d_hat, N * sizeof(double));
    wipe_host(sk_out.data(), sk_out.size() * sizeof(sk_out[0])); wipe_host(ss.data(), ss.size() * sizeof(ss[0]));
    if (rc != FHERAM_OK) return rc;
    HIPCHK(c, hipGetLastError());
    c->keys_loaded = true;
    c->inv_id[0] = c->inv_id[1] = 0;
    c->inv_pending[0] = c->inv_pending[1] = false;
    c->ram.memo_top = false; c->ram.memo_alone = 0;
    return FHERAM_OK;
}

size_t fheram_fheuint_ggsw_len(const fheram_ctx*) { return fheram_ctx::GGSW5; }
namespace {
int fheuint_alloc(fheram_ctx* c, int n_bits, fheram_fheuint** out) {
    fheram_fheuint* f = new fheram_fheuint{c, c->device, n_bits, nullptr, nullptr};
    hipError_t e = hipMalloc(&f->d_std, (size_t)n_bits * fheram_ctx::GGSW5 * sizeof(int32_t));
    if (e == hipSuccess) e = hipMalloc(&f->d_prep, (size_t)n_bits * fheram_ctx::GGSW5 * sizeof(double));
    if (e != hipSuccess) { fheram_fheuint_destroy(f); return fail(c, FHERAM_ERR_DEVICE, std::string("hipMalloc: ") + hipGetErrorString(e)); }
    *out = f;
    return FHERAM_OK;
}
int fheuint_prepare(fheram_ctx* c, fheram_fheuint* f) {
    c->cur = c->stream;
    launch_prepare(c, f->d_std, f->d_prep, f->n_bits * (int)(fheram_ctx::GGSW5 / N));
    HIPCHK(c, hipStreamSynchronize(c->stream));
    HIPCHK(c, hipGetLastError());
    return FHERAM_OK;
}
}
int fheram_fheuint_create(fheram_ctx* c, const int64_t* bits, int n_bits, fheram_fheuint** out) {
    if (!c || !out) return FHERAM_ERR_INVALID_ARG;
    *out = nullptr;
    if (!bits || n_bits <= 0 || n_bits > 64) return fail(c, FHERAM_ERR_INVALID_ARG, "bad argument");
    HIPCHK(c, hipSetDevice(c->device));
    fheram_fheuint* f = nullptr;
    int rc = fheuint_alloc(c, n_bits, &f);
    if (rc == FHERAM_OK) rc = upload_i64(c, f->d_std, bits, (size_t)n_bits * fheram_ctx::GGSW5);
    if (rc == FHERAM_OK) rc = fheuint_prepare(c, f);
    if (rc != FHERAM_OK) { fheram_fheuint_destroy(f); return rc; }
    *out = f;
    return FHERAM_OK;
}
int fheram_fheuint_encrypt_sk(fheram_ctx* c, const fheram_secret* sk, uint32_t value, int n_bits, const int64_t* mask,
                              const int64_t* noise, fheram_fheuint** out) {
    if (!c || !out) return FHERAM_ERR_INVALID_ARG;
    *out = nullptr;
    if (!mask || !noise || n_bits <= 0 || n_bits > 32) return fail(c, FHERAM_ERR_INVALID_ARG, "bad argument");
    const int S = fheram_ctx::S_INV, k = (int)c->p.k_evk_ggsw_inv, D = fheram_ctx::DNUM_GGSW;
    int rc = check_setup_args(c, sk, S, k);
    if (rc != FHERAM_OK) return rc;
    HIPCHK(c, hipSetDevice(c->device));
    const size_t glen = (size_t)S * 2 * N;
    const int n = n_bits * D * 2;
    std::vector<int32_t> pre((size_t)n * glen, 0), pt1((size_t)n * S * N, 0);
    int gi = 0;
    for (int i = 0; i < n_bits; i++) {
        const int32_t bit = (int32_t)((value >> i) & 1);
        for (int r = 0; r < D; r++)
            for (int ci = 0; ci < 2; ci++, gi++) {
                int32_t* pg = pre.data() + (size_t)gi * glen;
                if (ci == 0) pg[(size_t)(r * 2) * N] = bit;
                else pt1[((size_t)gi * S + r) * N] = bit;
                if (!stage_random(pg, S, k, mask + (size_t)gi * S * N, noise + (size_t)gi * N))
                    return fail(c, FHERAM_ERR_RANGE, "mask limb outside [-2^16, 2^16) or |noise| >= 2^30");
            }
    }
    fheram_fheuint* f = nullptr;
    rc = fheuint_alloc(c, n_bits, &f);
    if (rc == FHERAM_OK) rc = encrypt_staged(c, sk->d_hat, f->d_std, pre, &pt1, n, S);
    if (rc == FHERAM_OK) rc = fheuint_prepare(c, f);
    wipe_host(pre.data(), pre.size() * sizeof(int32_t)); wipe_host(pt1.data(), pt1.size() * sizeof(int32_t));
    if (rc != FHERAM_OK) { fheram_fheuint_destroy(f); return rc; }
    *out = f;
    return FHERAM_OK;
}
int fheram_fheuint_download(fheram_ctx* c, const fheram_fheuint* f, int64_t* out) {
    if (!c || !out) return FHERAM_ERR_INVALID_ARG;
    if (!f || f->ctx != c) return fail(c, FHERAM_ERR_INVALID_ARG, "integer belongs to another context");
    HIPCHK(c, hipSetDevice(c->device));
    return download_i64(c, out, f->d_std, (size_t)f->n_bits * fheram_ctx::GGSW5);
}
void fheram_fheuint_destroy(fheram_fheuint* f) {
    if (!f) return;
    hipSetDevice(f->device);
    if (f->d_std) hipFree(f->d_std);
    if (f->d_prep) hipFree(f->d_prep);
    delete f;
}
int fheram_address_set_from_fheuint(fheram_ctx* c, const fheram_fheuint* f, int sign, fheram_addr** out) {
    if (!c || !out) return FHERAM_ERR_INVALID_ARG;
    *out = nullptr;
    if (!f || f->ctx != c) return fail(c, FHERAM_ERR_INVALID_ARG, "integer belongs to another context");
    unsigned bits = 0;
    for (auto& b1 : c->base2d) for (int b : b1) bits += (unsigned)b;
    if ((int)bits > f->n_bits) return fail(c, FHERAM_ERR_INVALID_ARG, "the address plan is wider than the encrypted integer");
    HIPCHK(c, hipSetDevice(c->device));
    constexpr int S = fheram_ctx::S_ADDR, SG = fheram_ctx::S_INV, D = fheram_ctx::DNUM_CT;
    const long g4 = (long)fheram_ctx::GLWE4;
    const int rows = D * 2;
    fheram_addr* a = new fheram_addr{c, nullptr, c->n_digits, c->device};
    DevBuf tbuf, ebuf;
    double* big = nullptr;
    hipError_t e = hipMalloc(&a->d_ggsw, (size_t)c->n_digits * fheram_ctx::GGSW * sizeof(int32_t));
    if (e == hipSuccess) e = hipMalloc(&tbuf.p, (size_t)rows * g4 * sizeof(int32_t));
    if (e == hipSuccess) e = hipMalloc(&ebuf.p, (size_t)rows * g4 * sizeof(int32_t));
    if (e == hipSuccess) e = hipMalloc(&big, (size_t)rows * 2 * SG * 2 * S * N * sizeof(double));
    if (e != hipSuccess) { if (big) hipFree(big); fheram_address_destroy(a); return fail(c, FHERAM_ERR_DEVICE, std::string("hipMalloc: ") + hipGetErrorString(e)); }
    {
        std::vector<int32_t> h((size_t)c->n_digits * fheram_ctx::GGSW, 0);
        for (int d = 0; d < c->n_digits; d++)
            for (int r = 0; r < D; r++)
                for (int ci = 0; ci < 2; ci++) h[((size_t)(d * D + r) * 2 + ci) * g4 + (size_t)(r * 2 + ci) * N] = 1;
        e = hipMemcpy(a->d_ggsw, h.data(), h.size() * sizeof(int32_t), hipMemcpyHostToDevice);
    }
    c->cur = c->stream;
    int digit = 0;
    unsigned bit_rsh = 0;
    for (auto& base1d : c->base2d) {
        unsigned bit_lsh = 0;
        for (int bit_mask : base1d) {
            GlweRef acc = ref(a->d_ggsw + (size_t)digit * fheram_ctx::GGSW, 0, g4);
            GlweRef t = ref(tbuf.p, 0, g4), ev = ref(ebuf.p, 0, g4);
            for (int i = 0; i < bit_mask; i++) {
                const int step = 1 << (i + bit_lsh);
                const double* gb = f->d_prep + (size_t)(bit_rsh + i) * fheram_ctx::GGSW5;
                ProfScope ps(c, "set_from_fheuint", rows);
                hipLaunchKernelGGL((k_cmux_pre<S>), dim3(rows, 1, EW_SLICES), dim3(256), 0, c->cur, acc, t, sign ? step : -step);
                hipLaunchKernelGGL((k_ext_product_fine<S, SG>), dim3(rows, 1, 2 * SG * 2 * S), dim3(T), LDS_BYTES, c->cur, t, gb, c->d_tw, big);
                hipLaunchKernelGGL((k_ext_product_fine_norm<S, SG>), dim3(rows, 1, 2 * (N / 256)), dim3(256), 0, c->cur, ev, big);
                hipLaunchKernelGGL((k_add_norm<S>), dim3(rows, 1, EW_SLICES), dim3(256), 0, c->cur, acc, ev, acc);
            }
            bit_lsh += (unsigned)bit_mask;
            bit_rsh += (unsigned)bit_mask;
            digit++;
        }
    }
    if (e == hipSuccess) e = hipStreamSynchronize(c->stream);
    if (e == hipSuccess) e = hipGetLastError();
    hipFree(big);
    if (e != hipSuccess) { fheram_address_destroy(a); return fail(c, FHERAM_ERR_DEVICE, std::string("set_from_fheuint: ") + hipGetErrorString(e)); }
    *out = a;
    return FHERAM_OK;
}

int fheram_address_alloc(fheram_ctx* c, fheram_addr** out) {
    if (!c || !out) return FHERAM_ERR_INVALID_ARG;
    *out = nullptr;
    HIPCHK(c, hipSetDevice(c->device));
    fheram_addr* a = new fheram_addr{c, nullptr, c->n_digits, c->device};
    a->empty = true;
    const hipError_t e = hipMalloc(&a->d_ggsw, (size_t)c->n_digits * fheram_ctx::GGSW * sizeof(int32_t));
    if (e != hipSuccess) { delete a; return fail(c, FHERAM_ERR_DEVICE, std::string("hipMalloc: ") + hipGetErrorString(e)); }
    *out = a;
    return FHERAM_OK;
}
}
namespace {
void address_plan(const fheram_ctx* c, unsigned char* rsh, unsigned char* bits, unsigned char* lsh) {
    int digit = 0;
    unsigned bit_rsh = 0;
    for (auto& base1d : c->base2d) {
        unsigned bit_lsh = 0;
        for (int bit_mask : base1d) {
            rsh[digit] = (unsigned char)bit_rsh; bits[digit] = (unsigned char)bit_mask; lsh[digit] = (unsigned char)bit_lsh;
            bit_lsh += (unsigned)bit_mask;
            bit_rsh += (unsigned)bit_mask;
            digit++;
        }
    }
}
int derive_wait_readers(fheram_ctx* c, fheram_addr* const* addrs, int n) {
    bool wait_inv[2] = {false, false};
    for (int k = 0; k < n; k++)
        for (int ci = 0; ci < 2; ci++) if (c->inv_pending[ci] && c->inv_id[ci] == addrs[k]->id) wait_inv[ci] = true;
    for (int ci = 0; ci < 2; ci++) if (wait_inv[ci]) HIPCHK(c, hipStreamWaitEvent(c->stream, c->ev_inv[ci], 0));
    if (c->side_begun) HIPCHK(c, hipStreamWaitEvent(c->stream, c->ev_join, 0));
    return FHERAM_OK;
}
void derive_addresses_written(fheram_ctx* c, fheram_addr* const* addrs, int n) {
    for (int k = 0; k < n; k++) { addrs[k]->id = next_addr_id(); addrs[k]->empty = false; }
    c->derive_unsynced = true;
    main_enqueued(c);
}
int address_derive_body(fheram_ctx* c, const fheram_fheuint* const* fus, const int* first_bit, int n, int sign, fheram_addr* const* addrs) {
    if (n < 1 || n > FHERAM_DERIVE_MAX)
        return fail(c, FHERAM_ERR_INVALID_ARG, "n = " + std::to_string(n) + " is outside [1, FHERAM_DERIVE_MAX = " + std::to_string(FHERAM_DERIVE_MAX) + "]");
    static_assert(FHERAM_DERIVE_MAX == DERIVE_K_MAX, "the argument struct of k_cmux_chain holds FHERAM_DERIVE_MAX integers and addresses");
    unsigned bits = 0;
    for (auto& b1 : c->base2d) for (int b : b1) bits += (unsigned)b;
    for (int k = 0; k < n; k++) {
        if (!fus[k] || fus[k]->ctx != c) return fail(c, FHERAM_ERR_INVALID_ARG, "integer " + std::to_string(k) + " is null or belongs to another context");
        if (!addrs[k] || addrs[k]->ctx != c) return fail(c, FHERAM_ERR_INVALID_ARG, "address " + std::to_string(k) + " is null or belongs to another context");
        if ((int)bits > fus[k]->n_bits) return fail(c, FHERAM_ERR_INVALID_ARG, "the address plan is wider than the encrypted integer");
        if (first_bit && (first_bit[k] < 0 || first_bit[k] > fus[k]->n_bits - (int)bits))
            return fail(c, FHERAM_ERR_INVALID_ARG, "bits [" + std::to_string(first_bit[k]) + ", " + std::to_string(first_bit[k]) + " + " + std::to_string(bits) + ") of integer " + std::to_string(k) + " are beyond its " + std::to_string(fus[k]->n_bits) + " bits");
        for (int q = 0; q < k; q++)
            if (addrs[q] == addrs[k]) return fail(c, FHERAM_ERR_INVALID_ARG, "address " + std::to_string(k) + " appears twice in the list");
    }
    if (c->n_digits > DERIVE_DIGITS_MAX)
        return fail(c, FHERAM_ERR_UNSUPPORTED, "fheram_address_derive takes digit plans of at most " + std::to_string(DERIVE_DIGITS_MAX) + " digits");
    HIPCHK(c, hipSetDevice(c->device));
    CmuxChainArgs ca{};
    ca.tw = c->d_tw;
    ca.sign = sign ? 1 : 0;
    unsigned char rsh0[DERIVE_DIGITS_MAX] = {};
    address_plan(c, rsh0, ca.bits, ca.lsh);
    const int rcw = derive_wait_readers(c, addrs, n);
    if (rcw != FHERAM_OK) return rcw;
    c->cur = c->stream;
    bool done[DERIVE_K_MAX] = {};
    for (int k = 0; k < n; k++) {
        if (done[k]) continue;
        const int f0 = first_bit ? first_bit[k] : 0;
        for (int d = 0; d < c->n_digits; d++) ca.first[d] = (unsigned char)(rsh0[d] + f0);
        int K = 0;
        for (int q = k; q < n; q++)
            if ((first_bit ? first_bit[q] : 0) == f0) { ca.fu[K] = fus[q]->d_prep; ca.out[K] = addrs[q]->d_ggsw; K++; done[q] = true; }
        const int rows = fheram_ctx::DNUM_CT * 2;
        ProfScope ps(c, "derive", (uint64_t)K * c->n_digits * rows);
        cmux_chain_launch(dim3(rows, c->n_digits, K), c->cur, ca);
    }
    HIPCHK(c, hipGetLastError());
    derive_addresses_written(c, addrs, n);
    return FHERAM_OK;
}
}
extern "C" {
int fheram_address_derive(fheram_ctx* c, const fheram_fheuint* const* fus, int n, int sign, fheram_addr* const* addrs) {
    if (!c) return FHERAM_ERR_INVALID_ARG;
    if (!fus || !addrs) return fail(c, FHERAM_ERR_INVALID_ARG, "null integer or address list");
    return address_derive_body(c, fus, nullptr, n, sign, addrs);
}
int fheram_address_derive_at(fheram_ctx* c, const fheram_fheuint* const* fus, const int* first_bit, int n, int sign, fheram_addr* const* addrs) {
    if (!c) return FHERAM_ERR_INVALID_ARG;
    if (!fus || !addrs || !first_bit) return fail(c, FHERAM_ERR_INVALID_ARG, "null integer, bit or address list");
    return address_derive_body(c, fus, first_bit, n, sign, addrs);
}

}
```

Baseline: 1341.

## Precompute head rows of write trace on a third stream during read tail

Adds a third low-priority stream that, after a read preparing a write, runs the trace keyswitch chain for the first few rows into a dedicated buffer, overlapping with the read's inverse precompute. The following write on the same address copies those rows in and traces only the remaining rows, with the external products forced to a non-split form when this head split is active. The aim is to hide part of the write's serial trace latency behind the read's tail. In exchange it adds cross-stream events, extra state, a new buffer and narrow eligibility conditions, and it competes for CUs with the concurrent work.

```diff
diff --git a/fhe-ram_amd/csrc/bank.hpp b/fhe-ram_amd/csrc/bank.hpp
--- a/fhe-ram_amd/csrc/bank.hpp
+++ b/fhe-ram_amd/csrc/bank.hpp
@@ -293,7 +293,7 @@
 }
 void fheram_bank_destroy(fheram_bank* b) {
     if (!b) return;
-    if (b->c) { hipSetDevice(b->c->device); for (hipStream_t s : {b->c->stream, b->c->stream2}) if (s) hipStreamSynchronize(s); }
+    if (b->c) { hipSetDevice(b->c->device); for (hipStream_t s : {b->c->stream, b->c->stream2, b->c->stream3}) if (s) hipStreamSynchronize(s); }
     dense_free(b->list);
     dense_free(b->wl);
     select_free(b->sel);
diff --git a/fhe-ram_amd/csrc/ctx.hpp b/fhe-ram_amd/csrc/ctx.hpp
--- a/fhe-ram_amd/csrc/ctx.hpp
+++ b/fhe-ram_amd/csrc/ctx.hpp
@@ -37,6 +37,7 @@
     bool memo_top = false;
     int memo_alone = 0;
     bool res_in_trtop = false;
+    uint64_t early_id = 0;
 };
 
 struct DenseBufs {
@@ -106,6 +107,7 @@
     CtxResources res;
     hipStream_t stream = nullptr;
     hipStream_t stream2 = nullptr;
+    hipStream_t stream3 = nullptr;
     hipStream_t cur = nullptr;
     hipEvent_t ev_fork = nullptr, ev_join = nullptr;
     hipEvent_t ev_xout = nullptr, ev_xin = nullptr;
@@ -172,6 +174,15 @@
     bool wide_unsynced = false;
     bool derive_unsynced = false;
     bool main_idle = false;
+    int write_head = 0;
+    int32_t* d_early = nullptr;
+    int early_n = 0;
+    hipEvent_t ev_rows = nullptr;
+    hipEvent_t ev_gate = nullptr;
+    hipEvent_t ev_early = nullptr;
+    bool early_wanted = false;
+    bool early_pending = false;
+    bool head_split = false;
     int32_t* h_pin[2] = {nullptr, nullptr};
     hipEvent_t ev_pin[2] = {nullptr, nullptr};
     int64_t* h_res = nullptr;
diff --git a/fhe-ram_amd/csrc/fheram.hip b/fhe-ram_amd/csrc/fheram.hip
--- a/fhe-ram_amd/csrc/fheram.hip
+++ b/fhe-ram_amd/csrc/fheram.hip
@@ -109,9 +109,10 @@
         int lo = 0, hi = 0;
         CCHK(hipDeviceGetStreamPriorityRange(&lo, &hi));
         CCHK(hipStreamCreateWithPriority(&c->stream2, hipStreamNonBlocking, lo));
+        CCHK(hipStreamCreateWithPriority(&c->stream3, hipStreamNonBlocking, lo));
     }
     c->cur = c->stream;
-    for (hipEvent_t* ev : {&c->ev_fork, &c->ev_join, &c->ev_xout, &c->ev_xin}) CCHK(c->res.event(ev));
+    for (hipEvent_t* ev : {&c->ev_fork, &c->ev_join, &c->ev_xout, &c->ev_xin, &c->ev_rows, &c->ev_gate, &c->ev_early}) CCHK(c->res.event(ev));
     for (hipEvent_t* ev : {&c->t0, &c->t1}) CCHK(c->res.event(ev, true));
     fheram_config asked;
     if (user_cfg) asked = *user_cfg; else fheram_config_default(&asked);
@@ -211,6 +212,11 @@
     CCHK(hipHostGetDevicePointer((void**)&c->d_h_tail_done, c->h_tail_done, 0));
     c->tail_wait.done = c->h_tail_done; c->tail_wait.gave_up = c->h_tail_done + 16;
     if (const char* e = std::getenv("FHERAM_TAIL_POLL_US")) c->tail_wait.bound_us = std::atol(e);
+    {
+        const char* e = std::getenv("FHERAM_WRITE_HEAD");
+        c->write_head = (e && e[0] == '0') ? 0 : ((e && e[0] == '2') ? 2 : 1);
+        if (c->write_head && c->n2 == 2 && n_shards == 1) CCHK(c->res.device(&c->d_early, (size_t)2 * std::max(8, c->ws) * G * sizeof(int32_t)));
+    }
     CCHK(c->res.host(&c->h_mid_fb, 128, hipHostMallocDefault));
     memset(c->h_mid_fb, 0, 128);
     CCHK(c->res.host(&c->h_res, ((size_t)c->ws * G + 1) * sizeof(int64_t), hipHostMallocMapped));
@@ -225,11 +231,11 @@
 void fheram_ctx_destroy(fheram_ctx* c) {
     if (!c) return;
     hipSetDevice(c->device);
-    for (hipStream_t s : {c->stream, c->stream2}) if (s) hipStreamSynchronize(s);
+    for (hipStream_t s : {c->stream, c->stream2, c->stream3}) if (s) hipStreamSynchronize(s);
     prof_collect(c);
     dense_free(c->batch);
     c->res.release();
-    for (hipStream_t s : {c->stream2, c->stream}) if (s) hipStreamDestroy(s);
+    for (hipStream_t s : {c->stream3, c->stream2, c->stream}) if (s) hipStreamDestroy(s);
     delete c;
 }
 
@@ -257,6 +263,7 @@
     HIPCHK(c, hipSetDevice(c->device));
     HIPCHK(c, hipStreamSynchronize(c->stream));
     HIPCHK(c, hipStreamSynchronize(c->stream2));
+    HIPCHK(c, hipStreamSynchronize(c->stream3));
     int order[LOGN];
     for (int i = 0; i < LOGN; i++) {
         order[i] = -1;
@@ -282,7 +289,7 @@
     c->keys_loaded = true;
     c->inv_id[0] = c->inv_id[1] = 0;
     c->inv_pending[0] = c->inv_pending[1] = false;
-    c->ram.memo_top = false; c->ram.memo_alone = 0;
+    c->ram.memo_top = false; c->ram.memo_alone = 0; c->ram.early_id = 0; c->early_pending = false;
     return FHERAM_OK;
 }
 
@@ -292,7 +299,7 @@
     HIPCHK(c, hipSetDevice(c->device));
     int rc = upload_i64(c, c->d_data, rows, (size_t)c->ws * c->rows * fheram_ctx::GLWE);
     if (rc != FHERAM_OK) return rc;
-    c->ram.initialized = true; c->ram.state = false; c->ram.memo_top = false; c->ram.memo_alone = 0;
+    c->ram.initialized = true; c->ram.state = false; c->ram.memo_top = false; c->ram.memo_alone = 0; c->ram.early_id = 0;
     return FHERAM_OK;
 }
 int fheram_ram_download(fheram_ctx* c, int64_t* rows) {
@@ -363,6 +370,7 @@
     HIPCHK(c, hipSetDevice(c->device));
     HIPCHK(c, hipStreamSynchronize(c->stream));
     HIPCHK(c, hipStreamSynchronize(c->stream2));
+    HIPCHK(c, hipStreamSynchronize(c->stream3));
     double m = 0.0;
     HIPCHK(c, hipMemcpy(&m, c->d_tw + N, sizeof(double), hipMemcpyDeviceToHost));
     *max_out = m;
@@ -374,6 +382,7 @@
     HIPCHK(c, hipSetDevice(c->device));
     HIPCHK(c, hipStreamSynchronize(c->stream));
     HIPCHK(c, hipStreamSynchronize(c->stream2));
+    HIPCHK(c, hipStreamSynchronize(c->stream3));
     HIPCHK(c, hipMemset(c->d_tw + N, 0, sizeof(double)));
     __atomic_store_n(c->h_ro_flag, 0u, __ATOMIC_RELAXED);
     return FHERAM_OK;
diff --git a/fhe-ram_amd/csrc/launch.hpp b/fhe-ram_amd/csrc/launch.hpp
--- a/fhe-ram_amd/csrc/launch.hpp
+++ b/fhe-ram_amd/csrc/launch.hpp
@@ -34,20 +34,20 @@
 bool use_fine_split(const fheram_ctx* c, int gx, int gy, int wgs) {
     return c->cfg.limb_split && c->cfg.fine_split && (long)gx * gy * wgs <= c->cus && (long)gx * gy * wgs * N * 8 <= (long)LIMB_SPLIT_MAX * BIG_STRIDE * 8;
 }
-void launch_ep(fheram_ctx* c, GlweRef a, GlweRef res, const double* ggsw, int gx, int gy) {
+void launch_ep(fheram_ctx* c, GlweRef a, GlweRef res, const double* ggsw, int gx, int gy, bool beside = false) {
     if (gx <= 0 || gy <= 0) return;
     ProfScope ps(c, "ext_product", (uint64_t)gx * gy);
-    if (use_fine_split(c, gx, gy, 2 * 4 * 2 * 3)) {
+    if (!beside && use_fine_split(c, gx, gy, 2 * 4 * 2 * 3)) {
         hipLaunchKernelGGL((k_ext_product_fine<3, 4>), dim3(gx, gy, 2 * 4 * 2 * 3), dim3(T), LDS_BYTES, c->cur, a, ggsw, c->d_tw, big_of(c));
         hipLaunchKernelGGL((k_ext_product_fine_norm<3, 4>), dim3(gx, gy, 2 * (N / 256)), dim3(256), 0, c->cur, res, big_of(c));
         return;
     }
-    if (use_limb_split(c, gx, gy, 4)) {
+    if (!beside && use_limb_split(c, gx, gy, 4)) {
         hipLaunchKernelGGL((k_ext_product<3, 4, 1, 1>), dim3(gx, gy, 8), dim3(T), LDS_BYTES, c->cur, a, res, ggsw, c->d_tw, big_of(c));
         hipLaunchKernelGGL((k_ext_product<3, 4, 1, 2>), dim3(gx, gy, 2), dim3(T), 0, c->cur, a, res, ggsw, c->d_tw, big_of(c));
         return;
     }
-    if (pick_nco(c, gx, gy) == 1) hipLaunchKernelGGL((k_ext_product<3, 4, 1>), dim3(gx, gy, 2), dim3(T), LDS_BYTES, c->cur, a, res, ggsw, c->d_tw, big_of(c));
+    if (!beside && pick_nco(c, gx, gy) == 1) hipLaunchKernelGGL((k_ext_product<3, 4, 1>), dim3(gx, gy, 2), dim3(T), LDS_BYTES, c->cur, a, res, ggsw, c->d_tw, big_of(c));
     else {
         ProfScope pf(c, "ext_product_fused", (uint64_t)gx * gy);
         hipLaunchKernelGGL((k_ext_product<3, 4, 2>), dim3(gx, gy, 1), dim3(T), LDS_BYTES, c->cur, a, res, ggsw, c->d_tw, big_of(c));
@@ -129,11 +129,13 @@
     bool rotated = false;
     bool one_wg = false;
     bool handoff = true;
+    bool beside = false;
 };
 ChainPlan chain_form(const fheram_ctx* c, const ChainQuery& q) {
     const long batch = (long)q.gx * q.gy;
     const int sk = q.ep ? 4 : c->s_evk;
     const bool len = q.n >= 2 && q.n <= CHAIN_MAX;
+    if (q.ep && q.beside) return {len && c->cfg.chain ? ChainForm::Chain : ChainForm::Steps, 0};
     const bool handoff = q.handoff && len && c->cfg.limb_split &&
                          c->cus >= TAIL_GROUPS * 32 &&
                          !capturing(c);
@@ -233,11 +235,13 @@
     if (d >= 2) hipLaunchKernelGGL((k_ext_product_chain_r<4>), dim3(gx, gy, 1), dim3(T), LDS_BYTES, c->cur, ca);
     else hipLaunchKernelGGL((k_ext_product_chain<3, 4>), dim3(gx, gy, 1), dim3(T), LDS_BYTES, c->cur, ca);
 }
-void ep_chain(fheram_ctx* c, GlweRef src, GlweRef dst, GlweRef tmp, const double* prep, int d, int gx, int gy) {
+void ep_chain(fheram_ctx* c, GlweRef src, GlweRef dst, GlweRef tmp, const double* prep, int d, int gx, int gy, bool beside = false) {
     if (gx <= 0 || gy <= 0) return;
     GlweRef b[2];
     bool fits;
-    switch (plan_chain(c, ChainQuery{true, d, gx, gy}, src, dst, tmp, b, fits).form) {
+    ChainQuery q{true, d, gx, gy};
+    q.beside = beside;
+    switch (plan_chain(c, q, src, dst, tmp, b, fits).form) {
     case ChainForm::Mid: launch_mid_ep(c, src, b, prep, d, gx, gy); return;
     case ChainForm::Chain:
         if (!fits && !chain_bufs(d, src, tmp, dst, b)) break;
@@ -246,7 +250,7 @@
         return;
     default: break;
     }
-    run_chain(c, d, src, dst, tmp, gx, gy, [&](int i, GlweRef in, GlweRef out) { launch_ep(c, in, out, prep + (size_t)i * fheram_ctx::GGSW, gx, gy); });
+    run_chain(c, d, src, dst, tmp, gx, gy, [&](int i, GlweRef in, GlweRef out) { launch_ep(c, in, out, prep + (size_t)i * fheram_ctx::GGSW, gx, gy, beside); });
 }
 void launch_trace_chain(fheram_ctx* c, GlweRef src, const GlweRef (&b)[2], int start, int n, int gx, int gy, int rot_mul, int rot_base) {
     ProfScope ps(c, "keyswitch", (uint64_t)gx * gy, n);
@@ -403,6 +407,10 @@
         launch_ks_tr<KS_TRACE>(c, ka, gx, gy);
     });
 }
+GlweRef from_row(GlweRef r, int first) { r.p += (long)first * r.sx; return r; }
+void trace_steps_rows(fheram_ctx* c, GlweRef src, GlweRef dst, GlweRef tmp, int start, int end, int first, int count, int gy) {
+    trace_steps(c, from_row(src, first), from_row(dst, first), from_row(tmp, first), start, end, count, gy);
+}
 int32_t* pack_levels(fheram_ctx* c, int32_t* src, int32_t* A, int32_t* B, long sy, long sx, size_t count, int gy,
                      int n_alone, int first_pair, bool keep_alone = false, int32_t* P0 = nullptr, int32_t* P1 = nullptr) {
     const int k = ilog2_ceil(count);
@@ -472,6 +480,7 @@
         hipEventRecord(c->ev_fork, c->stream);
         hipStreamWaitEvent(c->stream2, c->ev_fork, 0);
     }
+    if (fork && c->early_wanted) hipEventRecord(c->ev_gate, c->stream2);
     hipStream_t keep = c->cur;
     c->cur = c->stream2;
     coordinate_prepare_inv(c, addr, ci, c->d_ggsw_inv + (size_t)coord_first_digit(c, ci) * fheram_ctx::GGSW, digits_of(c, c->d_prep_inv, ci), true);
diff --git a/fhe-ram_amd/csrc/path.hpp b/fhe-ram_amd/csrc/path.hpp
--- a/fhe-ram_amd/csrc/path.hpp
+++ b/fhe-ram_amd/csrc/path.hpp
@@ -38,13 +38,44 @@
 
 void read_local_done(const fheram_ctx* c, RamState* st, bool prepare_write) {
     if (c->n2 == 2) st->memo_alone = (prepare_write && c->cfg.memo) ? LOGN - ilog2_ceil(c->rows_glob) : 0;
+    st->early_id = 0;
 }
 void read_top_done(fheram_ctx* c, RamState* st, bool prepare_write) {
     st->memo_top = prepare_write && c->cfg.memo;
     st->res_in_trtop = st->memo_top;
     c->prep1_ready = false;
 }
-void write_done(fheram_ctx* c, RamState* st) { st->memo_top = false; st->memo_alone = 0; c->side_begun = false; c->tree_rotate_pending = false; }
+void write_done(fheram_ctx* c, RamState* st) { st->memo_top = false; st->memo_alone = 0; st->early_id = 0; c->side_begun = false; c->tree_rotate_pending = false; c->head_split = false; }
+
+int head_rows(const fheram_ctx* c, int ws) {
+    const int d = (ws <= 8 && 8 % ws == 0) ? 8 / ws : 1;
+    return std::max(1, std::min(d, (int)c->rows - 1));
+}
+bool early_rows_form(const Opnds& o, const RamView& a, bool prepare_write) {
+    const fheram_ctx* c = o.c;
+    if (!c->write_head || !prepare_write || o.n != 1 || o.bank || o.st != &c->ram || a.rows != c->d_data || !c->d_early) return false;
+    if (c->n_shards != 1 || c->n2 != 2 || capturing(c)) return false;
+    if (!c->cfg.memo || c->cfg.pre_inv != 1 || !c->cfg.fuse || !c->cfg.chain || c->cfg.chain_y != 3) return false;
+    const long fill = (long)c->rows * o.ws;
+    return c->write_head == 2 ? fill <= c->cus : (fill == c->cus && head_rows(c, o.ws) * o.ws % 8 == 0);
+}
+void early_rows(const Opnds& o, const RamView& a) {
+    fheram_ctx* c = o.c;
+    const long G = (long)fheram_ctx::GLWE;
+    const int kept = o.st->memo_alone, d = head_rows(c, o.ws);
+    hipStreamWaitEvent(c->stream3, c->ev_rows, 0);
+    hipStreamWaitEvent(c->stream3, c->ev_gate, 0);
+    hipStream_t keep = c->cur;
+    c->cur = c->stream3;
+    GlweRef b[2];
+    chain_bufs(LOGN - kept, ref(a.A, (long)c->rows * G, G), ref(c->d_early, d * G, G), ref(c->d_early + (long)o.ws * d * G, d * G, G), b);
+    launch_trace_chain(c, ref(a.A, (long)c->rows * G, G), b, kept, LOGN - kept, d, o.ws, 0, 0);
+    hipEventRecord(c->ev_early, c->stream3);
+    c->cur = keep;
+    c->early_pending = true;
+    c->early_n = d;
+    o.st->early_id = o.addrs[0]->id;
+}
 
 template <typename F>
 int run_op(fheram_ctx* c, const fheram_addr* addr, int which, F&& enqueue) {
@@ -117,8 +148,10 @@
     const int L0 = LOGN - ilog2_ceil(c->rows_glob);
     const bool keep = o.st->memo_alone > 0;
     int32_t* packed;
+    const bool early = early_rows_form(o, a, prepare_write);
     if (o.row_fuse(d0, L0, R) && !(prepare_write && (d0 & 1))) {
         launch_read_chain(c, data, prepare_write ? &data : nullptr, A, o.prep(0, 0), d0, L0, R, Y, o.table());
+        if (early) hipEventRecord(c->ev_rows, c->stream);
         packed = pack_levels(c, a.A, a.A, a.B, sy, G, (size_t)R, Y, 0, L0, keep, a.C, a.D);
     } else {
         for (int k = 0; k < n; k++)
@@ -130,6 +163,7 @@
             leaves = a.D;
         }
         packed = pack_levels(c, leaves, a.A, a.B, sy, G, (size_t)R, Y, L0, L0, keep, a.C, a.D);
+        if (early) hipEventRecord(c->ev_rows, c->stream);
     }
     *packed_out = ref(packed, sy, 0);
     if (to_part) launch_copy(c, *packed_out, part, 1, Y);
@@ -162,6 +196,8 @@
     }
     const bool pre = n == 1 && prepare_write && c->cfg.pre_inv && (long)c->rows * Y <= c->cus;
     const bool gated = pre && c->cfg.pre_inv == 1 && !capturing(c) && tail_top();
+    const bool early = pre && o.st->memo_alone > 0 && early_rows_form(o, a, prepare_write);
+    c->early_wanted = early;
     if (pre && !gated)
         for (int ci = c->n2 - 1; ci >= 0; ci--) precompute_inverse(c, o.addrs[0], ci, ci == c->n2 - 1);
     read_top_done(c, o.st, prepare_write);
@@ -182,6 +218,8 @@
         const unsigned seq = c->tail_launches != tl0 ? c->tail_seq : 0;
         for (int ci = c->n2 - 1; ci >= 0; ci--) precompute_inverse(c, o.addrs[0], ci, ci == c->n2 - 1, seq);
     }
+    if (early) early_rows(o, a);
+    c->early_wanted = false;
     c->tail_wait.note_top(c->tail_launches != tl0 ? c->tail_seq : 0);
     return FHERAM_OK;
 }
@@ -399,6 +437,12 @@
     GlweRef top = (c->n2 != 1) ? tree : ref(v.rows, sy, 0);
     GlweRef tr = tmp;
     const bool by_member = c->n2 == 1 && !o.rows_dense();
+    if (c->head_split) {
+        hipStreamWaitEvent(c->stream, c->ev_early, 0);
+        c->early_pending = false;
+        launch_copy(c, ref(c->d_early, c->early_n * G, G), ref(c->trhi_in_C ? v.C : v.A, sy, G), c->early_n, Y);
+    }
+    const bool beside = c->head_split;
     if (o.st->memo_top) tr = ref(v.trtop, G, 0);
     else if (by_member) for (int k = 0; k < n; k++) trace_steps(c, o.rows(top, k), o.slice(tmp, k), o.slice(tmp2, k), 0, LOGN, 1, ws);
     else trace_steps(c, top, tmp, tmp2, 0, LOGN, 1, Y);
@@ -419,7 +463,7 @@
         }
         if (n == 1) { c->inv_pending[1] = false; c->inv_id[1] = 0; }
         for (int k = 0; k < n; k++)
-            ep_chain(c, o.slice(tree, k), o.slice(ref(v.part, G, 0), k), o.slice(tmp, k), o.inv(k, 1), (int)c->base2d[1].size(), 1, ws);
+            ep_chain(c, o.slice(tree, k), o.slice(ref(v.part, G, 0), k), o.slice(tmp, k), o.inv(k, 1), (int)c->base2d[1].size(), 1, ws, beside);
         c->tree_rotate_pending = true;
     }
     return FHERAM_OK;
@@ -434,11 +478,20 @@
         hipStreamWaitEvent(c->stream2, c->ev_fork, 0);
     }
     main_enqueued(c);
+    c->head_split = c->write_head && o.n == 1 && o.st == &c->ram && c->n2 == 2 && c->n_shards == 1 && !capturing(c) && o.st->memo_alone > 0 && o.st->memo_top &&
+                    o.st->early_id != 0 && o.st->early_id == o.addrs[0]->id && c->inv_id[0] == o.addrs[0]->id && c->inv_id[1] == o.addrs[0]->id;
+    if (c->early_pending && !c->head_split) {
+        hipStreamWaitEvent(c->stream, c->ev_early, 0);
+        hipStreamWaitEvent(c->stream2, c->ev_early, 0);
+        c->early_pending = false;
+    }
+    o.st->early_id = 0;
     c->cur = c->stream2;
     if (c->n2 == 2) {
         const int kept = o.st->memo_alone;
         c->trhi_in_C = kept > 0 && (LOGN - kept) % 2 == 1;
-        if (kept > 0) trace_steps(c, ref(v.A, sy, G), ref(c->trhi_in_C ? v.C : v.A, sy, G), ref(c->trhi_in_C ? v.A : v.C, sy, G), kept, LOGN, (int)c->rows, o.Y());
+        if (c->head_split) trace_steps_rows(c, ref(v.A, sy, G), ref(c->trhi_in_C ? v.C : v.A, sy, G), ref(c->trhi_in_C ? v.A : v.C, sy, G), kept, LOGN, c->early_n, (int)c->rows - c->early_n, o.Y());
+        else if (kept > 0) trace_steps(c, ref(v.A, sy, G), ref(c->trhi_in_C ? v.C : v.A, sy, G), ref(c->trhi_in_C ? v.A : v.C, sy, G), kept, LOGN, (int)c->rows, o.Y());
         else if (!o.rows_dense())
             for (int k = 0; k < o.n; k++) trace_steps(c, o.rows(ref(v.rows, sy, G), k), o.slice(ref(v.A, sy, G), k), o.slice(ref(v.C, sy, G), k), 0, LOGN, (int)c->rows, o.ws);
         else trace_steps(c, ref(v.rows, sy, G), ref(v.A, sy, G), ref(v.C, sy, G), 0, LOGN, (int)c->rows, o.Y());
diff --git a/fhe-ram_amd/csrc/setup.hpp b/fhe-ram_amd/csrc/setup.hpp
--- a/fhe-ram_amd/csrc/setup.hpp
+++ b/fhe-ram_amd/csrc/setup.hpp
@@ -318,6 +318,7 @@
     HIPCHK(c, hipSetDevice(c->device));
     HIPCHK(c, hipStreamSynchronize(c->stream));
     HIPCHK(c, hipStreamSynchronize(c->stream2));
+    HIPCHK(c, hipStreamSynchronize(c->stream3));
     c->cur = c->stream;
     int32_t *d_stage = nullptr, *d_small = nullptr;
     double* d_hat = nullptr;
@@ -374,7 +375,7 @@
     c->keys_loaded = true;
     c->inv_id[0] = c->inv_id[1] = 0;
     c->inv_pending[0] = c->inv_pending[1] = false;
-    c->ram.memo_top = false; c->ram.memo_alone = 0;
+    c->ram.memo_top = false; c->ram.memo_alone = 0; c->ram.early_id = 0; c->early_pending = false;
     return FHERAM_OK;
 }
 
```

New measurement: 1299. 3.1% lower.
